# kalj/dealii-cuda

Hardware: AMD Instinct MI355X
Metric: DoFs/s on 1305x Laplace vmult (bmop), p=4 3D uniform (higher is better)
Workload: dtype f64; 1 GPU; bmop: DEGREE_FE=4, DIMENSION=3, MATRIX_FREE_UNIFORM_MESH, hyper_cube(-1,1), 54^3 cells, 10218313 DoFs, 1 z-slab(s); cells_per_dir=54, n_dofs=10218313, n_cells=157464, parallelism=slab1, dof_numbering=caller's (lexicographic), finite=True, clock_ramp_steps=2000

## Files before the change

dealii-cuda_amd/csrc/mfgpu_api.hip:

```cpp
#include <hip/hip_runtime.h>

#include <type_traits>

#include <algorithm>
#include <cmath>
#include <cstdlib>
#include <cstring>
#include <memory>
#include <string>
#include <vector>

#include "mfgpu_kernels.h"

using namespace mfgpu;

struct EventTimer {
  std::vector<Event> ev;
  size_t used = 0;
  double ms = 0.0;
  int begin(hipStream_t st) {
    if (used + 2 > ev.size()) {
      Event e0, e1;
      int rc;
      if ((rc = e0.create(hipEventDefault)) || (rc = e1.create(hipEventDefault))) return rc;
      ev.push_back(std::move(e0));
      ev.push_back(std::move(e1));
    }
    HIP_TRY(hipEventRecord(ev[used].get(), st));
    return 0;
  }
  int end(hipStream_t st) {
    HIP_TRY(hipEventRecord(ev[used + 1].get(), st));
    used += 2;
    return 0;
  }
  int drain(double *total) {
    for (size_t i = 0; i + 1 < used; i += 2) {
      float t = 0.f;
      HIP_TRY(hipEventElapsedTime(&t, ev[i].get(), ev[i + 1].get()));
      ms += t;
    }
    used = 0;
    *total = ms;
    return 0;
  }
  void reset() {
    used = 0;
    ms = 0.0;
  }
};

struct mfgpu_handle {
  Plan plan;
  int dim = 0, n = 0, nd = 0, number_type = MFGPU_F64;
  bool hn = false;
  std::vector<double> S, Dt;
  std::vector<double> sv, sg;
  DeviceArray<uint32_t> d_batch_cell_off, d_batch_dof_off, d_bdofs;
  DeviceArray<uint8_t> d_bflags;
  DeviceArray<uint16_t> d_lmap;
  DeviceArray<uint16_t> d_lmapx;
  DeviceArray<uint16_t> d_perm;
  DeviceArray<uint32_t> d_bdofsp, d_idxp;
  DeviceArray<uint32_t> d_hnrec;
  DeviceArray<uint32_t> d_hn_slot;
  DeviceArray<void> d_coefp;
  DeviceArray<void> d_coef;
  DeviceArray<uint32_t> d_cmask, d_orphans;
  DeviceArray<void> d_hnw;
  DeviceArray<uint32_t> d_constrained;
  uint32_t n_constrained = 0;
  DeviceArray<void> d_tabsd;
  DeviceArray<void> d_tab2;
  bool twopass = true;
  DeviceArray<uint32_t> d_batch_nint, d_halo_off;
  std::vector<uint32_t> seg_end;
  std::vector<DeviceArray<uint32_t>> d_p2arr, d_p2tiles;
  std::vector<uint32_t> n_p2tiles;
  Stream side;
  std::vector<Event> ev_seg;
  Event ev_side;
  bool side_pending = false;
  DeviceArray<void> d_halo;
  DeviceArray<unsigned long long> d_stamps;
  size_t lds = 0, device_bytes = 0;
  PlaneKernel planes = PlaneKernel::none;
  BatchKernel batches = BatchKernel::none;
  uint32_t max_grid = 0;
  uint32_t max_grid_p = 0;
  uint32_t max_grid_ph = 0;
  bool prof = false;
  EventTimer t_cells;
  EventTimer t_pass2;
  uint64_t prof_vmults = 0;
};

namespace {

template <typename T>
hipError_t family_configure(const mfgpu_handle *h, PlaneKernel k, bool hn, size_t *lds, int *blocks) {
  const Plan &P = h->plan;
  switch (k) {
    case PlaneKernel::planes3: return p_configure<T>(P.dim, P.n, hn, h->twopass, P.max_batch_dofs, lds, blocks);
    case PlaneKernel::planes4: return q_configure<T>(P.dim, P.n, hn, h->twopass, P.max_batch_dofs, lds, blocks);
    default: return hipErrorInvalidValue;
  }
}
template <typename T>
hipError_t family_configure(const mfgpu_handle *h, BatchKernel k, bool hn, size_t *lds, int *blocks) {
  const Plan &P = h->plan;
  switch (k) {
    case BatchKernel::batches: return apply_configure<T>(P.dim, P.n, hn, h->twopass, P.max_batch_dofs, lds, blocks);
    case BatchKernel::x: return x_configure<T>(P.dim, P.n, hn, h->twopass, P.max_batch_dofs, lds, blocks);
    case BatchKernel::g: return g_configure<T>(P.dim, P.n, hn, h->twopass, P.max_batch_dofs, lds, blocks);
    case BatchKernel::g2: return g2_configure<T>(P.dim, P.n, hn, h->twopass, P.max_batch_dofs, lds, blocks);
    default: return hipErrorInvalidValue;
  }
}
template <typename T>
hipError_t family_launch(const mfgpu_handle *h, PlaneKernel k, const ApplyArgs<T> &a, bool hn, uint32_t grid,
                         hipStream_t st) {
  const Plan &P = h->plan;
  const double *S = h->S.data(), *Dt = h->Dt.data();
  switch (k) {
    case PlaneKernel::planes3: return p_launch<T>(P.dim, P.n, hn, h->twopass, a, S, Dt, grid, st);
    case PlaneKernel::planes4: return q_launch<T>(P.dim, P.n, hn, h->twopass, a, S, Dt, grid, st);
    default: return hipErrorInvalidValue;
  }
}
template <typename T>
hipError_t family_launch(const mfgpu_handle *h, BatchKernel k, const ApplyArgs<T> &a, bool hn, uint32_t grid,
                         hipStream_t st) {
  const Plan &P = h->plan;
  const double *S = h->S.data(), *Dt = h->Dt.data();
  switch (k) {
    case BatchKernel::batches: return apply_launch<T>(P.dim, P.n, hn, h->twopass, a, S, Dt, grid, st);
    case BatchKernel::x: return x_launch<T>(P.dim, P.n, hn, h->twopass, a, S, Dt, grid, st);
    case BatchKernel::g: return g_launch<T>(P.dim, P.n, hn, h->twopass, a, S, Dt, grid, st);
    case BatchKernel::g2: return g2_launch<T>(P.dim, P.n, hn, h->twopass, a, S, Dt, grid, st);
    default: return hipErrorInvalidValue;
  }
}

int check_symmetrize(int n, std::vector<double> &S, std::vector<double> &Dt) {
  const int p = n - 1;
  double err = 0, mag = 0;
  for (int r = 0; r < n; ++r)
    for (int c = 0; c < n; ++c) {
      const double s1 = S[r * n + c], s2 = S[(p - r) * n + (p - c)];
      const double d1 = Dt[r * n + c], d2 = -Dt[(p - r) * n + (p - c)];
      err = std::fmax(err, std::fmax(std::fabs(s1 - s2), std::fabs(d1 - d2)));
      mag = std::fmax(mag, std::fmax(std::fabs(s1), std::fabs(d1)));
    }
  if (err > 1e-10 * mag) {
    set_error("shape tables are not symmetric about the cell midpoint (unsupported)");
    return MFGPU_EUNSUPPORTED;
  }
  for (int r = 0; r < n; ++r)
    for (int c = 0; c < n; ++c) {
      const int r2 = p - r, c2 = p - c;
      if (r * n + c < r2 * n + c2) {
        const double s = 0.5 * (S[r * n + c] + S[r2 * n + c2]);
        S[r * n + c] = S[r2 * n + c2] = s;
        const double d = 0.5 * (Dt[r * n + c] - Dt[r2 * n + c2]);
        Dt[r * n + c] = d;
        Dt[r2 * n + c2] = -d;
      } else if (r == r2 && c == c2) {
        Dt[r * n + c] = 0.0;
      }
    }
  return 0;
}

int upload_pass2(mfgpu_handle *h, const uint32_t *priority, uint32_t n_priority) {
  const Plan &P = h->plan;
  std::vector<uint8_t> prio(P.n_dofs, 0);
  for (uint32_t i = 0; i < n_priority; ++i) {
    if (priority[i] >= P.n_dofs) {
      set_error("priority dof out of range");
      return MFGPU_EINVAL;
    }
    prio[priority[i]] = 1;
  }
  const size_t ng = 1 + h->seg_end.size();
  std::vector<std::vector<uint32_t>> sd(ng), so(ng, std::vector<uint32_t>(1, 0u)), si(ng);
  auto add = [&](uint32_t dof, const uint32_t *slots, uint32_t k, size_t seg) {
    const size_t g = prio[dof & 0x7fffffffu] ? 0 : 1 + seg;
    sd[g].push_back(dof);
    si[g].insert(si[g].end(), slots, slots + k);
    so[g].push_back((uint32_t)si[g].size());
  };
  for (size_t i = 0; i < P.sdofs.size(); ++i) {
    size_t seg = 0;
    if (P.s_off[i + 1] > P.s_off[i]) {
      const uint32_t slot = P.s_idx[P.s_off[i + 1] - 1];
      const uint32_t batch = (uint32_t)(std::upper_bound(P.halo_off.begin(), P.halo_off.end(), slot) - P.halo_off.begin()) - 1;
      seg = (size_t)(std::upper_bound(h->seg_end.begin(), h->seg_end.end(), batch) - h->seg_end.begin());
      if (seg >= h->seg_end.size()) seg = h->seg_end.size() - 1;
    }
    add(P.sdofs[i], P.s_idx.data() + P.s_off[i], P.s_off[i + 1] - P.s_off[i], seg);
  }
  const uint32_t zero_slot = P.halo_off.empty() ? 0u : P.halo_off.back();
  for (uint32_t orph : P.orphans) add(orph, &zero_slot, 1, 0);
  std::vector<DeviceArray<uint32_t>> d_arr(ng), d_tiles(ng);
  std::vector<uint32_t> n_tiles(ng, 0u);
  for (size_t g = 0; g < ng; ++g) {
    std::vector<uint32_t> arr, tiles;
    build_pass2_classes(sd[g], so[g], si[g], arr, tiles);
    n_tiles[g] = (uint32_t)(tiles.size() / 4);
    if ((size_t)P.halo_off.back() * esize(h->number_type) <= ((size_t)256 << 20)) {
      const size_t nt = tiles.size() / 4;
      for (size_t a = 0, b = nt ? nt - 1 : 0; a < b; ++a, --b)
        for (int w = 0; w < 4; ++w) std::swap(tiles[4 * a + w], tiles[4 * b + w]);
    }
    int rc;
    if ((rc = d_arr[g].upload(arr.data(), arr.size()))) return rc;
    if ((rc = d_tiles[g].upload(tiles.data(), tiles.size()))) return rc;
  }
  h->d_p2arr = std::move(d_arr);
  h->d_p2tiles = std::move(d_tiles);
  h->n_p2tiles = std::move(n_tiles);
  return 0;
}

template <typename T>
int create_arrays(mfgpu_handle *h, const mfgpu_desc &d) {
  const Plan &P = h->plan;
  const size_t ncell = P.n_cells, nd = (size_t)P.nd;
  size_t &acct = h->device_bytes;
  auto up = [&](auto &arr, const void *src, size_t n) {
    const int rc = arr.upload(src, n);
    acct += arr.bytes();
    return rc;
  };
  int rc;
  if ((rc = up(h->d_batch_cell_off, P.batch_cell_off.data(), P.batch_cell_off.size()))) return rc;
  if ((rc = up(h->d_batch_dof_off, P.batch_dof_off.data(), P.batch_dof_off.size()))) return rc;
  if ((rc = up(h->d_bdofs, P.bdofs.data(), P.bdofs.size()))) return rc;
  if ((rc = up(h->d_bflags, P.bflags.data(), P.bflags.size()))) return rc;
  if ((rc = up(h->d_lmap, P.lmap.data(), P.lmap.size()))) return rc;
  const bool general = h->batches == BatchKernel::g || h->batches == BatchKernel::g2;
  if (h->batches == BatchKernel::x && !h->hn) {
    const int n = P.n, n2 = n * n, PP = n2, CH = 256 / PP, ndl = n2 * n;
    std::vector<uint16_t> perm(512, 0xffff);
    for (int layout = 0; layout < 2; ++layout) {
      uint16_t *lanes = perm.data() + 256 * layout;
      std::vector<int> fill(32, 0), overflow;
      for (int q = 0; q < CH * PP; ++q) {
        const int cell = q / PP, pen = q % PP, a = pen % n, b = pen / n;
        const int base = cell * ndl + (layout == 0 ? a + n2 * b : a + n * b);
        const int r = base & 31;
        if (fill[r] < 8) lanes[32 * fill[r]++ + r] = (uint16_t)q;
        else overflow.push_back(q);
      }
      for (int l = 255; l >= 0 && !overflow.empty(); --l)
        if (lanes[l] == 0xffff) {
          lanes[l] = (uint16_t)overflow.back();
          overflow.pop_back();
        }
    }
    if ((rc = up(h->d_perm, perm.data(), perm.size()))) return rc;
  }
  if (h->batches == BatchKernel::x || general) {
    const size_t n = (size_t)P.n, np = (n + 1) & ~(size_t)1, runs = P.lmap.size() / n;
    std::vector<uint16_t> lx(runs * np, 0);
    for (size_t r = 0; r < runs; ++r)
      for (size_t i = 0; i < n; ++i) lx[r * np + i] = P.lmap[r * n + i];
    if ((rc = up(h->d_lmapx, lx.data(), lx.size()))) return rc;
  }
  if (h->batches == BatchKernel::g2) {
    std::vector<T> sd(2 * (size_t)P.n * P.n);
    for (int i = 0; i < P.n * P.n; ++i) {
      sd[i] = (T)h->S[i];
      sd[P.n * P.n + i] = (T)h->Dt[i];
    }
    if ((rc = up(h->d_tabsd, sd.data(), sd.size() * sizeof(T)))) return rc;
  }
  if (h->planes != PlaneKernel::none) {
    if ((rc = build_plane_records(h->plan, d.constraint_mask))) return rc;
    if (!P.pr_hn.empty()) {
      if ((rc = up(h->d_hnrec, P.pr_hn.data(), P.pr_hn.size()))) return rc;
      if ((rc = up(h->d_hn_slot, P.pr_hn_slot.data(), P.pr_hn_slot.size()))) return rc;
    }
    if ((rc = up(h->d_bdofsp, P.pr_dofs.data(), P.pr_dofs.size()))) return rc;
    if ((rc = up(h->d_idxp, P.pr_idx.data(), P.pr_idx.size()))) return rc;
  }
  if ((rc = up(h->d_orphans, P.orphans.data(), P.orphans.size()))) return rc;
  if (h->twopass) {
    if ((rc = up(h->d_batch_nint, P.batch_nint.data(), P.batch_nint.size()))) return rc;
    if ((rc = up(h->d_halo_off, P.halo_off.data(), P.halo_off.size()))) return rc;
    if (h->planes != PlaneKernel::none && (uint64_t)P.halo_off.back() >= (1ull << 29)) {
      set_error("halo buffer too large for 32-bit byte offsets");
      return MFGPU_EUNSUPPORTED;
    }
    const size_t hb = ((size_t)P.halo_off.back() + 1) * sizeof(T);
    if ((rc = h->d_halo.alloc(hb, true))) return rc;
    acct += hb;
  }
  if (h->hn) {
    std::vector<uint32_t> cm(ncell);
    for (size_t i = 0; i < ncell; ++i) cm[i] = d.constraint_mask[P.cell_order[i]];
    if ((rc = up(h->d_cmask, cm.data(), ncell))) return rc;
    std::vector<T> w((size_t)h->n * h->n);
    for (size_t i = 0; i < w.size(); ++i) w[i] = (T)d.constraint_weights[i];
    if ((rc = up(h->d_hnw, w.data(), w.size() * sizeof(T)))) return rc;
  }
  DeviceArray<T> metric;
  if ((rc = fold_coefficient<T>(metric, d.coefficient, d.quadrature_points, d.JxW, d.inv_jac, P.cell_order.data(), P.dim,
                                (uint32_t)ncell, (uint32_t)nd, general)))
    return rc;
  h->d_coef = std::move(metric);
  acct += h->d_coef.bytes();
  if (h->planes != PlaneKernel::none) {
    const int n = P.n, NT = p_cells_per_wave(n) * n;
    const size_t nbat = P.n_plane_batches, total = nbat * (size_t)(n * n) * NT;
    const size_t ncell_p = P.batch_cell_off[nbat];
    std::vector<uint32_t> cb(ncell_p), cp(ncell_p);
    for (size_t b = 0; b < nbat; ++b)
      for (uint32_t c = P.batch_cell_off[b]; c < P.batch_cell_off[b + 1]; ++c) {
        cb[c] = (uint32_t)b;
        cp[c] = c - P.batch_cell_off[b];
      }
    DeviceArray<uint32_t> t_cb, t_cp;
    if ((rc = t_cb.upload(cb.data(), ncell_p))) return rc;
    if ((rc = t_cp.upload(cp.data(), ncell_p))) return rc;
    if ((rc = h->d_coefp.alloc(total * sizeof(T), true))) return rc;
    acct += h->d_coefp.bytes();
    HIP_TRY(relayout_coef_launch<T>(h->d_coefp.as<T>(), h->d_coef.as<const T>(), t_cb.get(), t_cp.get(), ncell_p * nd, n,
                                    nullptr));
    HIP_TRY(hipDeviceSynchronize());
  }
  int dev = 0, per_cu = 0;
  hipDeviceProp_t prop;
  HIP_TRY(hipGetDevice(&dev));
  HIP_TRY(hipGetDeviceProperties(&prop, dev));
  auto resident_grid = [&](int blocks_per_cu) {
    const uint32_t g = (uint32_t)(blocks_per_cu < 1 ? 1 : blocks_per_cu) * (uint32_t)prop.multiProcessorCount;
    return d.max_workgroups && d.max_workgroups < g ? d.max_workgroups : g;
  };
  if (h->planes != PlaneKernel::none) {
    HIP_TRY(family_configure<T>(h, h->planes, false, &h->lds, &per_cu));
    h->max_grid_p = resident_grid(per_cu);
    if (P.n_plain_plane_batches < P.n_plane_batches) {
      size_t lds_h = 0;
      HIP_TRY(family_configure<T>(h, h->planes, true, &lds_h, &per_cu));
      h->max_grid_ph = resident_grid(per_cu);
      h->lds = std::max(h->lds, lds_h);
    }
  }
  if (h->batches == BatchKernel::none) return 0;
  const hipError_t configure_batch_family = family_configure<T>(h, h->batches, h->hn, &h->lds, &per_cu);
  if (h->lds > 160 * 1024) {
    set_error("batch needs more than 160 KiB of LDS; lower max_dofs_per_batch");
    return MFGPU_EINVAL;
  }
  HIP_TRY(configure_batch_family);
  h->max_grid = resident_grid(per_cu);
  return 0;
}

void choose_segments(mfgpu_handle *h, uint32_t request) {
  const Plan &P = h->plan;
  const uint32_t nb = (uint32_t)(P.batch_cell_off.size() - 1);
  h->seg_end.assign(1, nb);
  if (!h->twopass || nb < 2 || request == 1) return;
  const uint32_t npl = P.n_plane_batches, nplain = P.n_plain_plane_batches;
  std::vector<uint32_t> cuts;
  if (npl > 0 && npl < nb) cuts.push_back(npl);
  if (nplain > 0 && nplain < npl) cuts.push_back(nplain);
  if (request > 1) {
    for (uint32_t i = 1; i < request; ++i) cuts.push_back((uint32_t)((uint64_t)nb * i / request));
  }
  if (request == 0 && !P.pr_hn.empty() && nplain == 0 && P.n == 5) cuts.push_back(nb / 2);
  std::sort(cuts.begin(), cuts.end());
  h->seg_end.clear();
  for (uint32_t c : cuts)
    if (c > 0 && c < nb && (h->seg_end.empty() || h->seg_end.back() != c)) h->seg_end.push_back(c);
  h->seg_end.push_back(nb);
}

template <typename T>
int create_typed(mfgpu_handle *h, const mfgpu_desc &d) {
  int rc = create_arrays<T>(h, d);
  if (rc) return rc;
  choose_segments(h, d.cell_loop_segments);
  if (!h->twopass) return 0;
  if (h->seg_end.size() > 1) {
    int prio_least = 0, prio_greatest = 0;
    HIP_TRY(hipDeviceGetStreamPriorityRange(&prio_least, &prio_greatest));
    if ((rc = h->side.create(hipStreamNonBlocking, prio_least))) return rc;
    if ((rc = h->ev_side.create(hipEventDisableTiming))) return rc;
    h->ev_seg.resize(h->seg_end.size() - 1);
    for (Event &e : h->ev_seg)
      if ((rc = e.create(hipEventDisableTiming))) return rc;
  }
  return upload_pass2(h, nullptr, 0);
}

template <typename T>
int launch_pass2_group(mfgpu_handle *h, size_t group, void *dst, const void *src, hipStream_t st, int add) {
  HIP_TRY(reduce_classes_launch<T>((T *)dst, (const T *)src, h->d_halo.as<const T>(), h->d_p2arr[group].get(),
                                   h->d_p2tiles[group].get(), h->n_p2tiles[group], add, st));
  return 0;
}

template <typename T>
int vmult_pass2(mfgpu_handle *h, int phase, void *dst, const void *src, hipStream_t st, int add) {
  if (!h->twopass) return 0;
  if (phase == 0) return launch_pass2_group<T>(h, 0, dst, src, st, add);
  int rc = launch_pass2_group<T>(h, h->seg_end.size(), dst, src, st, add);
  if (!rc && h->side_pending) {
    HIP_TRY(hipStreamWaitEvent(st, h->ev_side.get(), 0));
    h->side_pending = false;
  }
  return rc;
}

template <typename T>
int launch_cells(mfgpu_handle *h, ApplyArgs<T> a, uint32_t b0, uint32_t b1, hipStream_t st) {
  const Plan &P = h->plan;
  const uint32_t npl = P.n_plane_batches, nplain = P.n_plain_plane_batches;
  if (b0 < nplain) {
    a.batch0 = b0;
    a.batch_end = b1 < nplain ? b1 : nplain;
    const uint32_t nbat = a.batch_end - a.batch0;
    HIP_TRY(family_launch<T>(h, h->planes, a, false, nbat < h->max_grid_p ? nbat : h->max_grid_p, st));
    b0 = a.batch_end;
  }
  if (b0 < npl && b0 < b1) {
    a.batch0 = b0;
    a.batch_end = b1 < npl ? b1 : npl;
    const uint32_t nbat = a.batch_end - a.batch0;
    HIP_TRY(family_launch<T>(h, h->planes, a, true, nbat < h->max_grid_ph ? nbat : h->max_grid_ph, st));
    b0 = a.batch_end;
  }
  if (b0 >= b1) return 0;
  a.batch0 = b0;
  a.batch_end = b1;
  const uint32_t nrest = b1 - b0, grid = nrest < h->max_grid ? nrest : h->max_grid;
  HIP_TRY(family_launch<T>(h, h->batches, a, h->hn, grid, st));
  return 0;
}

template <typename T>
ApplyArgs<T> make_args(mfgpu_handle *h, void *dst, const void *src, int add) {
  const Plan &P = h->plan;
  ApplyArgs<T> a;
  a.batch_cell_off = h->d_batch_cell_off.get();
  a.batch_dof_off = h->d_batch_dof_off.get();
  a.bdofs = h->d_bdofs.get();
  a.bflags = h->d_bflags.get();
  a.lmap = h->d_lmap.get();
  a.lmapx = h->d_lmapx.get();
  a.perm = h->d_perm.get();
  a.bdofsp = h->d_bdofsp.get();
  a.idxp = h->d_idxp.get();
  a.hnrec = h->d_hnrec.get();
  a.hn_slot = h->d_hn_slot.get();
  a.coefp = h->d_coefp.as<const T>();
  a.coef = h->d_coef.as<const T>();
  a.cmask = h->d_cmask.get();
  a.hn_weights = h->d_hnw.as<const T>();
  a.tabS = h->d_tabsd.as<const T>();
  a.tabDt = a.tabS ? a.tabS + (size_t)P.n * P.n : nullptr;
  a.batch_nint = h->d_batch_nint.get();
  a.halo_off = h->d_halo_off.get();
  a.halo = h->d_halo.as<T>();
  a.dst = (T *)dst;
  a.src = (const T *)src;
  a.nb_max = P.max_batch_dofs;
  a.add = add;
  a.stamps = h->d_stamps.get();
  a.dbg = 0;
  return a;
}

template <typename T>
int vmult_main(mfgpu_handle *h, void *dst, const void *src, hipStream_t st, int add) {
  const Plan &P = h->plan;
  ApplyArgs<T> a = make_args<T>(h, dst, src, add);
  int rc;
  if (h->prof && (rc = h->t_cells.begin(st))) return rc;
  if (h->twopass) {
    const size_t nseg = h->seg_end.size();
    if (h->side_pending) {
      HIP_TRY(hipStreamWaitEvent(st, h->ev_side.get(), 0));
      h->side_pending = false;
    }
    for (size_t s = 0; s < nseg; ++s) {
      if ((rc = launch_cells<T>(h, a, s ? h->seg_end[s - 1] : 0u, h->seg_end[s], st))) return rc;
      if (s + 1 < nseg) {
        HIP_TRY(hipEventRecord(h->ev_seg[s].get(), st));
        HIP_TRY(hipStreamWaitEvent(h->side.get(), h->ev_seg[s].get(), 0));
        if ((rc = launch_pass2_group<T>(h, 1 + s, dst, src, h->side.get(), add))) return rc;
      }
    }
    if (nseg > 1) {
      HIP_TRY(hipEventRecord(h->ev_side.get(), h->side.get()));
      h->side_pending = true;
    }
  } else {
    for (size_t c = 0; c + 1 < P.color_batch_off.size(); ++c) {
      if (P.color_batch_off[c + 1] == P.color_batch_off[c]) continue;
      if ((rc = launch_cells<T>(h, a, P.color_batch_off[c], P.color_batch_off[c + 1], st))) return rc;
    }
  }
  if (h->prof && (rc = h->t_cells.end(st))) return rc;
  if (!h->twopass)
    HIP_TRY(orphan_launch<T>((T *)dst, (const T *)src, h->d_orphans.get(), (uint32_t)P.orphans.size(), add, st));
  if (h->prof) h->prof_vmults++;
  return 0;
}

template <typename T>
int vmult_typed(mfgpu_handle *h, void *dst, const void *src, hipStream_t st, int add) {
  int rc = vmult_main<T>(h, dst, src, st, add);
  if (rc) return rc;
  const bool timed = h->prof && h->twopass;
  if (timed && (rc = h->t_pass2.begin(st))) return rc;
  rc = vmult_pass2<T>(h, 0, dst, src, st, add);
  if (!rc) rc = vmult_pass2<T>(h, 1, dst, src, st, add);
  if (!rc && timed) rc = h->t_pass2.end(st);
  return rc;
}

}

namespace {
template <typename T>
int inverse_diagonal_typed(mfgpu_handle *h, void *diag, hipStream_t st) {
  const Plan &P = h->plan;
  const bool general = h->batches == BatchKernel::g || h->batches == BatchKernel::g2;
  if (!h->d_tab2.get()) {
    const int nn = h->n * h->n;
    std::vector<T> t2(2 * (size_t)nn);
    for (int i = 0; i < nn; ++i) {
      t2[i] = (T)(general ? h->sv[i] : h->sv[i] * h->sv[i]);
      t2[nn + i] = (T)(general ? h->sg[i] : h->sg[i] * h->sg[i]);
    }
    if (const int rc = h->d_tab2.upload(t2.data(), t2.size() * sizeof(T))) return rc;
    h->device_bytes += h->d_tab2.bytes();
  }
  HIP_TRY(fill_launch<T>((T *)diag, P.n_dofs, T(0), st));
  const uint32_t nb = (uint32_t)(P.batch_cell_off.size() - 1), *cell_off = h->d_batch_cell_off.get();
  const uint32_t *dof_off = h->d_batch_dof_off.get(), *bdofs = h->d_bdofs.get(), *cmask = h->d_cmask.get();
  const uint16_t *lmap = h->d_lmap.get();
  const T *coef = h->d_coef.as<const T>(), *hnw = h->d_hnw.as<const T>(), *tab2 = h->d_tab2.as<const T>();
  if (h->batches == BatchKernel::g2)
    HIP_TRY(diag_general2_launch<T>(P.n, (T *)diag, nb, cell_off, dof_off, bdofs, lmap, coef, cmask, hnw, tab2, st));
  else if (h->batches == BatchKernel::g)
    HIP_TRY(diag_general_launch<T>(P.n, (T *)diag, nb, cell_off, dof_off, bdofs, lmap, coef, cmask, hnw, tab2, st));
  else
    HIP_TRY(diag_launch<T>(P.dim, P.n, (T *)diag, nb, cell_off, dof_off, bdofs, lmap, coef, cmask, hnw, tab2, st));
  HIP_TRY(set_values_launch<T>((T *)diag, h->d_constrained.get(), h->n_constrained, T(1), st));
  HIP_TRY(vec_map_launch<T>(4, (T *)diag, nullptr, T(0), T(0), P.n_dofs, st));
  return 0;
}
}


namespace {
int vec_map(int op, void *v, const void *w, double s, double a, size_t n, int nt, void *stream) {
  if ((!v && n) || (!w && n && op <= 3)) {
    set_error("null vector");
    return MFGPU_EINVAL;
  }
  if (nt == MFGPU_F32)
    HIP_TRY(vec_map_launch<float>(op, (float *)v, (const float *)w, (float)s, (float)a, n, (hipStream_t)stream));
  else if (nt == MFGPU_F64)
    HIP_TRY(vec_map_launch<double>(op, (double *)v, (const double *)w, s, a, n, (hipStream_t)stream));
  else
    return MFGPU_EINVAL;
  return 0;
}
int vec_reduce(int op, void *v, const void *x, const void *w, double a, size_t n, int nt, void *stream, double *out) {
  if (!out || (n && (!v || (op != 2 && !w) || (op == 1 && !x)))) {
    set_error("null argument");
    return MFGPU_EINVAL;
  }
  if (nt == MFGPU_F32)
    HIP_TRY(vec_reduce_launch<float>(op, (float *)v, (const float *)x, (const float *)w, (float)a, n, (hipStream_t)stream, out));
  else if (nt == MFGPU_F64)
    HIP_TRY(vec_reduce_launch<double>(op, (double *)v, (const double *)x, (const double *)w, a, n, (hipStream_t)stream, out));
  else
    return MFGPU_EINVAL;
  return 0;
}
}


namespace mfgpu {
int handle_number_type(const mfgpu_handle *h) { return h->number_type; }
int handle_set_priority_dofs(mfgpu_handle *h, const uint32_t *ids, uint32_t n) {
  return h->twopass ? upload_pass2(h, ids, n) : 0;
}
int handle_n_batches(const mfgpu_handle *h) { return (int)h->plan.batch_cell_off.size() - 1; }
bool handle_ranged_ok(const mfgpu_handle *h) { return h->twopass && h->seg_end.size() == 1; }
int handle_batches_touching(const mfgpu_handle *h, const uint32_t *ids, uint32_t n, std::vector<uint8_t> &flags) {
  const Plan &P = h->plan;
  std::vector<uint8_t> mark(P.n_dofs, 0);
  for (uint32_t i = 0; i < n; ++i) {
    if (ids[i] >= P.n_dofs) {
      set_error("interface dof out of range");
      return MFGPU_EINVAL;
    }
    mark[ids[i]] = 1;
  }
  const size_t nb = P.batch_cell_off.size() - 1;
  flags.assign(nb, 0);
  for (size_t b = 0; b < nb; ++b)
    for (uint32_t t = P.batch_dof_off[b]; t < P.batch_dof_off[b + 1]; ++t)
      if (mark[P.bdofs[t] & 0x7fffffffu]) {
        flags[b] = 1;
        break;
      }
  return 0;
}
int handle_cells_range(mfgpu_handle *h, uint32_t b0, uint32_t b1, void *dst, const void *src, void *stream, int add) {
  if (b0 >= b1) return 0;
  hipStream_t st = (hipStream_t)stream;
  if (h->number_type == MFGPU_F64) return launch_cells<double>(h, make_args<double>(h, dst, src, add), b0, b1, st);
  return launch_cells<float>(h, make_args<float>(h, dst, src, add), b0, b1, st);
}
int handle_cells_two_ranges(mfgpu_handle *h, uint32_t b0, uint32_t b1, uint32_t c0, uint32_t c1, void *dst,
                            const void *src, void *stream, int add) {
  const uint32_t nplain = h->plan.n_plain_plane_batches, npl = h->plan.n_plane_batches;
  const bool plain = c1 <= nplain, masked = b0 >= nplain && c1 <= npl;
  if (b0 >= b1 || c0 >= c1 || b1 > c0 || !(plain || masked)) {
    const int rc = handle_cells_range(h, b0, b1, dst, src, stream, add);
    return rc ? rc : handle_cells_range(h, c0, c1, dst, src, stream, add);
  }
  hipStream_t st = (hipStream_t)stream;
  auto run = [&](auto a) -> int {
    a.batch0 = b0;
    a.batch_end = c1;
    a.hole0 = b1;
    a.hole_len = c0 - b1;
    const uint32_t nbat = (b1 - b0) + (c1 - c0);
    using T = typename std::remove_const<typename std::remove_pointer<decltype(a.src)>::type>::type;
    const uint32_t cap = plain ? h->max_grid_p : h->max_grid_ph;
    HIP_TRY(family_launch<T>(h, h->planes, a, !plain, nbat < cap ? nbat : cap, st));
    return 0;
  };
  return h->number_type == MFGPU_F64 ? run(make_args<double>(h, dst, src, add)) : run(make_args<float>(h, dst, src, add));
}
int handle_pass2_group(mfgpu_handle *h, int group, void *dst, const void *src, void *stream, int add) {
  if (!h->twopass) return 0;
  hipStream_t st = (hipStream_t)stream;
  return h->number_type == MFGPU_F64 ? launch_pass2_group<double>(h, (size_t)group, dst, src, st, add)
                                     : launch_pass2_group<float>(h, (size_t)group, dst, src, st, add);
}
int handle_vmult_phase(mfgpu_handle *h, int phase, void *dst, const void *src, void *stream, int add) {
  hipStream_t st = (hipStream_t)stream;
  if (h->number_type == MFGPU_F64)
    return phase == 0 ? vmult_main<double>(h, dst, src, st, add) : vmult_pass2<double>(h, phase - 1, dst, src, st, add);
  return phase == 0 ? vmult_main<float>(h, dst, src, st, add) : vmult_pass2<float>(h, phase - 1, dst, src, st, add);
}
}

extern "C" {

int mfgpu_create(const mfgpu_desc *desc, mfgpu_handle **out) {
  if (!desc || !out) {
    set_error("null argument");
    return MFGPU_EINVAL;
  }
  const mfgpu_desc &d = *desc;
  if (!valid_number_type(d.number_type)) {
    set_error("number_type must be MFGPU_F64 or MFGPU_F32");
    return MFGPU_EINVAL;
  }
  const bool general = !(d.flags & MFGPU_UNIFORM_J0);
  if (general && (d.flags & MFGPU_COLORED_SCATTER)) {
    set_error("the general-Jacobian path (no MFGPU_UNIFORM_J0) is implemented in two-pass scatter mode only");
    return MFGPU_EUNSUPPORTED;
  }
  if (!d.JxW || !d.inv_jac || !d.shape_values || !d.shape_gradients ||
      (!d.coefficient && !d.quadrature_points)) {
    set_error("JxW, inv_jac, shape tables and coefficient (or quadrature_points) are required");
    return MFGPU_EINVAL;
  }
  const bool hn = (d.flags & MFGPU_HANGING_NODES) != 0;
  if (hn && (!d.constraint_mask || !d.constraint_weights)) {
    set_error("MFGPU_HANGING_NODES needs constraint_mask and constraint_weights");
    return MFGPU_EINVAL;
  }
  std::unique_ptr<mfgpu_handle, decltype(&mfgpu_destroy)> h(new mfgpu_handle(), mfgpu_destroy);
  int rc = choose_kernel_and_plan(d, h->planes, h->batches, h->plan);
  if (rc) return rc;
  h->dim = d.dim;
  h->n = d.degree + 1;
  h->nd = h->plan.nd;
  h->number_type = d.number_type;
  h->hn = hn;
  h->twopass = !(d.flags & MFGPU_COLORED_SCATTER);
  const int nn = h->n * h->n;
  std::vector<double> sv(nn), sg(nn);
  for (int i = 0; i < nn; ++i) {
    sv[i] = d.number_type == MFGPU_F64 ? ((const double *)d.shape_values)[i] : ((const float *)d.shape_values)[i];
    sg[i] = d.number_type == MFGPU_F64 ? ((const double *)d.shape_gradients)[i] : ((const float *)d.shape_gradients)[i];
  }
  h->sv = sv;
  h->sg = sg;
  rc = derive_tables(h->n, sv.data(), sg.data(), h->S, h->Dt);
  if (!rc) rc = check_symmetrize(h->n, h->S, h->Dt);
  if (!rc) rc = d.number_type == MFGPU_F64 ? create_typed<double>(h.get(), d) : create_typed<float>(h.get(), d);
  if (!rc && d.n_constrained) {
    h->n_constrained = d.n_constrained;
    rc = h->d_constrained.upload(d.constrained_dofs, d.n_constrained);
    h->device_bytes += h->d_constrained.bytes();
  }
  if (rc) return rc;
  *out = h.release();
  return 0;
}

void mfgpu_destroy(mfgpu_handle *h) {
  if (!h) return;
  if (h->side.get()) hipStreamSynchronize(h->side.get());
  delete h;
}

int mfgpu_vmult(mfgpu_handle *h, void *dst, const void *src, void *stream) {
  if (!h || !dst || !src) {
    set_error("null argument");
    return MFGPU_EINVAL;
  }
  if (dst == src) {
    set_error("vmult: dst and src must not alias");
    return MFGPU_EINVAL;
  }
  return h->number_type == MFGPU_F64 ? vmult_typed<double>(h, dst, src, (hipStream_t)stream, 0)
                                     : vmult_typed<float>(h, dst, src, (hipStream_t)stream, 0);
}

int mfgpu_vmult_add(mfgpu_handle *h, void *dst, const void *src, void *stream) {
  if (!h || !dst || !src) {
    set_error("null argument");
    return MFGPU_EINVAL;
  }
  if (dst == src) {
    set_error("vmult_add: dst and src must not alias");
    return MFGPU_EINVAL;
  }
  return h->number_type == MFGPU_F64 ? vmult_typed<double>(h, dst, src, (hipStream_t)stream, 1)
                                     : vmult_typed<float>(h, dst, src, (hipStream_t)stream, 1);
}

uint32_t mfgpu_n_dofs(const mfgpu_handle *h) { return h ? h->plan.n_dofs : 0; }

size_t mfgpu_memory_consumption(const mfgpu_handle *h) { return h ? h->device_bytes : 0; }

int mfgpu_plan_stats(const mfgpu_handle *h, uint64_t s[8]) {
  if (!h || !s) return MFGPU_EINVAL;
  const Plan &P = h->plan;
  s[0] = P.batch_cell_off.size() - 1;
  s[1] = P.color_batch_off.size() - 1;
  s[2] = P.bdofs.size();
  s[3] = P.max_batch_dofs;
  s[4] = P.max_batch_cells;
  s[5] = P.orphans.size();
  s[6] = P.n_first;
  s[7] = P.n_add;
  if (h->twopass) {
    const uint32_t nb = (uint32_t)s[0], npl = P.n_plane_batches, nplain = P.n_plain_plane_batches;
    const uint32_t edge[4] = {0u, nplain, npl, nb};
    s[1] = 0;
    for (size_t g = 0; g < h->seg_end.size(); ++g) {
      const uint32_t s0 = g ? h->seg_end[g - 1] : 0u, s1 = h->seg_end[g];
      for (int f = 0; f < 3; ++f)
        if (std::max(s0, edge[f]) < std::min(s1, edge[f + 1])) ++s[1];
    }
    s[6] = P.sdofs.size();
    s[7] = P.halo_off.back();
  }
  return 0;
}

const char *mfgpu_kernel_name(const mfgpu_handle *h) {
  if (!h) return "";
  const bool x = h->batches == BatchKernel::x;
  switch (h->planes) {
    case PlaneKernel::planes3: return x ? "apply_planes3+apply_batches_x" : "apply_planes3";
    case PlaneKernel::planes4: return x ? "apply_planes4+apply_batches_x" : "apply_planes4";
    default: break;
  }
  switch (h->batches) {
    case BatchKernel::x: return "apply_batches_x";
    case BatchKernel::g: return "apply_batches_g";
    case BatchKernel::g2: return "apply_batches_g2";
    default: return "apply_batches";
  }
}

int mfgpu_profile_enable(mfgpu_handle *h, int on) {
  if (!h) return MFGPU_EINVAL;
  h->prof = on != 0;
  h->t_cells.reset();
  h->t_pass2.reset();
  h->prof_vmults = 0;
  return 0;
}

int mfgpu_profile_read_pass2(mfgpu_handle *h, double *ms) {
  if (!h || !ms) return MFGPU_EINVAL;
  HIP_TRY(hipDeviceSynchronize());
  return h->t_pass2.drain(ms);
}

int mfgpu_profile_read(mfgpu_handle *h, double *ms, uint64_t *nv) {
  if (!h || !ms || !nv) return MFGPU_EINVAL;
  HIP_TRY(hipDeviceSynchronize());
  if (const int rc = h->t_cells.drain(ms)) return rc;
  *nv = h->prof_vmults;
  return 0;
}

#ifdef MFGPU_STAMPS
int mfgpu_debug_stamps(mfgpu_handle *h, unsigned long long *out, size_t n_batches) {
  if (!h) return MFGPU_EINVAL;
  const size_t nbt = h->plan.batch_cell_off.size() - 1;
  if (!h->d_stamps.get()) return h->d_stamps.alloc(2 * nbt * 16, true);
  if (out && n_batches == nbt) {
    HIP_TRY(hipDeviceSynchronize());
    HIP_TRY(hipMemcpy(out, h->d_stamps.get(), 2 * nbt * 16 * sizeof(unsigned long long), hipMemcpyDeviceToHost));
  }
  return 0;
}
#endif


int mfgpu_compute_inverse_diagonal(mfgpu_handle *h, void *inv_diag, void *stream) {
  if (!h || !inv_diag) {
    set_error("null argument");
    return MFGPU_EINVAL;
  }
  return h->number_type == MFGPU_F64 ? inverse_diagonal_typed<double>(h, inv_diag, (hipStream_t)stream)
                                     : inverse_diagonal_typed<float>(h, inv_diag, (hipStream_t)stream);
}

int mfgpu_set_constrained_values(mfgpu_handle *h, void *vec, double value, void *stream) {
  if (!h || !vec) {
    set_error("null argument");
    return MFGPU_EINVAL;
  }
  if (h->number_type == MFGPU_F64)
    HIP_TRY(set_values_launch<double>((double *)vec, h->d_constrained.get(), h->n_constrained, value, (hipStream_t)stream));
  else
    HIP_TRY(set_values_launch<float>((float *)vec, h->d_constrained.get(), h->n_constrained, (float)value,
                                     (hipStream_t)stream));
  return 0;
}

int mfgpu_vec_sadd(void *v, double s, double a, const void *w, size_t n, int nt, void *stream) {
  return vec_map(0, v, w, s, a, n, nt, stream);
}
int mfgpu_vec_equ(void *v, double a, const void *w, size_t n, int nt, void *stream) {
  return vec_map(1, v, w, 0.0, a, n, nt, stream);
}
int mfgpu_vec_scale(void *v, const void *w, size_t n, int nt, void *stream) {
  return vec_map(2, v, w, 0.0, 0.0, n, nt, stream);
}
int mfgpu_vec_divide(void *v, const void *w, size_t n, int nt, void *stream) {
  return vec_map(3, v, w, 0.0, 0.0, n, nt, stream);
}
int mfgpu_vec_invert(void *v, size_t n, int nt, void *stream) { return vec_map(4, v, nullptr, 0.0, 0.0, n, nt, stream); }
int mfgpu_vec_mul(void *v, double a, size_t n, int nt, void *stream) {
  return vec_map(5, v, nullptr, 0.0, a, n, nt, stream);
}
int mfgpu_vec_dot(const void *v, const void *w, size_t n, int nt, void *stream, double *result) {
  return vec_reduce(0, const_cast<void *>(v), nullptr, w, 0.0, n, nt, stream, result);
}
int mfgpu_vec_l2_norm(const void *v, size_t n, int nt, void *stream, double *result) {
  int rc = vec_reduce(0, const_cast<void *>(v), nullptr, v, 0.0, n, nt, stream, result);
  if (!rc) *result = std::sqrt(*result);
  return rc;
}
int mfgpu_vec_add_and_dot(void *v, double a, const void *x, const void *w, size_t n, int nt, void *stream,
                          double *result) {
  return vec_reduce(1, v, x, w, a, n, nt, stream, result);
}
int mfgpu_vec_all_zero(const void *v, size_t n, int nt, void *stream, int *result) {
  if (!result) return MFGPU_EINVAL;
  double cnt = 0.0;
  int rc = vec_reduce(2, const_cast<void *>(v), nullptr, nullptr, 0.0, n, nt, stream, &cnt);
  if (!rc) *result = cnt == 0.0;
  return rc;
}

int mfgpu_vec_alloc(void **dev, size_t n, int nt) {
  if (!dev) return MFGPU_EINVAL;
  *dev = nullptr;
  if (n == 0) return 0;
  HIP_TRY(hipMalloc(dev, n * esize(nt)));
  HIP_TRY(hipMemset(*dev, 0, n * esize(nt)));
  return 0;
}
int mfgpu_vec_free(void *dev) {
  if (dev) HIP_TRY(hipFree(dev));
  return 0;
}
int mfgpu_vec_fill(void *dev, size_t n, int nt, double value, void *stream) {
  if (!dev && n) return MFGPU_EINVAL;
  if (nt == MFGPU_F32)
    HIP_TRY(fill_launch<float>((float *)dev, n, (float)value, (hipStream_t)stream));
  else
    HIP_TRY(fill_launch<double>((double *)dev, n, value, (hipStream_t)stream));
  return 0;
}
int mfgpu_vec_from_host(void *dev, const void *host, size_t n, int nt) {
  if (n) HIP_TRY(hipMemcpy(dev, host, n * esize(nt), hipMemcpyHostToDevice));
  return 0;
}
int mfgpu_vec_to_host(void *host, const void *dev, size_t n, int nt) {
  if (n) HIP_TRY(hipMemcpy(host, dev, n * esize(nt), hipMemcpyDeviceToHost));
  return 0;
}
int mfgpu_device_synchronize(void) {
  HIP_TRY(hipDeviceSynchronize());
  return 0;
}
int mfgpu_device_memory_info(size_t *free_bytes, size_t *total_bytes) {
  if (!free_bytes || !total_bytes) return MFGPU_EINVAL;
  HIP_TRY(hipMemGetInfo(free_bytes, total_bytes));
  return 0;
}

}
```

dealii-cuda_amd/csrc/mfgpu_internal.h:

```cpp
#ifndef MFGPU_INTERNAL_H
#define MFGPU_INTERNAL_H

#include <cstdint>
#include <string>
#include <vector>

#include "../../include/mfgpu.h"

namespace mfgpu {

void set_error(const std::string &msg);

inline int ipow(int a, int e) {
  int r = 1;
  for (int i = 0; i < e; ++i) r *= a;
  return r;
}

constexpr int p_cells_per_wave(int n) { return 64 / n; }
constexpr int p_ji(int n) { return n == 3 ? 2 : n == 4 ? 5 : n == 5 ? 9 : n == 6 ? 14 : 23; }
constexpr int p_hs(int n) { return n == 3 ? 3 : n == 4 ? 6 : n == 5 ? 9 : n == 6 ? 14 : 18; }
constexpr int p_kgu(int n) { return p_ji(n) + p_hs(n); }
constexpr int p_cell_stride(int n) {
  int s = n * n * n;
  while ((s & 31) != (n & 31)) ++s;
  return s;
}

constexpr int q_plane_stride(int n) { return n >= 6 ? 65 : n == 5 ? 33 : n == 4 ? 17 : 33; }
constexpr int q_cell_stride(int n) { return n * q_plane_stride(n); }
constexpr int p_priv_max(int n) { return n >= 5 ? 384 : n == 4 ? 256 : 192; }
constexpr int kHnOpRounds = 2;
constexpr int p_hn_rows(int n) { return p_priv_max(n) / 64 + 3 * kHnOpRounds * 3 + 2; }

template <typename T>
constexpr size_t q_region_doubles(int n) {
  const size_t t = ((size_t)(p_cells_per_wave(n) + 1) * q_cell_stride(n) * sizeof(T) + 7) / 8;
  const size_t u = (size_t)p_kgu(n) * 64 + p_priv_max(n);
  return t > u ? t : u;
}
template <typename T>
constexpr size_t q_lds_bytes(int n, bool hn) {
  return (q_region_doubles<T>(n) + (hn ? (size_t)n * n : 0)) * 8;
}

constexpr uint8_t kFlagConstrained = 1;
constexpr uint8_t kFlagAdd = 2;

struct Plan {
  int dim = 0, degree = 0, n = 0, nd = 0;
  uint32_t n_dofs = 0, n_cells = 0;
  std::vector<uint32_t> cell_order;
  std::vector<uint32_t> batch_cell_off;
  std::vector<uint32_t> batch_dof_off;
  std::vector<uint32_t> color_batch_off;
  std::vector<uint32_t> bdofs;
  std::vector<uint8_t> bflags;
  std::vector<uint16_t> lmap;
  std::vector<uint32_t> orphans;
  std::vector<uint32_t> batch_nint;
  std::vector<uint32_t> halo_off;
  std::vector<uint32_t> sdofs;
  std::vector<uint32_t> s_off;
  std::vector<uint32_t> s_idx;
  std::vector<uint32_t> chunks;
  std::vector<uint32_t> gstarts;
  uint32_t max_batch_dofs = 0, max_batch_cells = 0;
  uint32_t n_plane_batches = 0;
  uint32_t n_plain_plane_batches = 0;
  std::vector<uint32_t> pr_dofs, pr_idx, pr_hn, pr_hn_slot;
  uint64_t n_first = 0, n_add = 0;
};

struct PlanLimits {
  uint32_t max_cells = 0, max_dofs = 0;
  uint32_t interior_max = 0, shared_max = 0, halo_stride = 0;
  bool segregate_masked = false;
  bool masked_planes = false;
  uint32_t private_max = 0;
};

int build_plan(const mfgpu_desc &d, Plan &plan, uint32_t max_chunks = 3, const PlanLimits *limits = nullptr);

struct HnLine {
  uint16_t node[8];
};
void hn_cell_lines(unsigned mask, int n, std::vector<HnLine> (&lines)[3], std::vector<uint16_t> &nodes);

enum class PlaneKernel : uint8_t { none, planes3, planes4 };
enum class BatchKernel : uint8_t { none, batches, x, g, g2 };
int choose_kernel_and_plan(const mfgpu_desc &d, PlaneKernel &pk, BatchKernel &bk, Plan &plan);
int build_plane_records(Plan &plan, const uint32_t *constraint_mask);

int derive_tables(int n, const double *shape_values, const double *shape_gradients,
                  std::vector<double> &S, std::vector<double> &Dt);

int handle_number_type(const mfgpu_handle *h);
int handle_set_priority_dofs(mfgpu_handle *h, const uint32_t *ids, uint32_t n);
int handle_vmult_phase(mfgpu_handle *h, int phase, void *dst, const void *src, void *stream, int add);
int handle_n_batches(const mfgpu_handle *h);
bool handle_ranged_ok(const mfgpu_handle *h);
int handle_batches_touching(const mfgpu_handle *h, const uint32_t *ids, uint32_t n, std::vector<uint8_t> &flags);
int handle_cells_range(mfgpu_handle *h, uint32_t b0, uint32_t b1, void *dst, const void *src, void *stream, int add);
int handle_cells_two_ranges(mfgpu_handle *h, uint32_t b0, uint32_t b1, uint32_t c0, uint32_t c1, void *dst,
                            const void *src, void *stream, int add);
int handle_pass2_group(mfgpu_handle *h, int group, void *dst, const void *src, void *stream, int add);

}

struct mfgpu_plan {
  mfgpu::Plan plan;
};

#endif
```

dealii-cuda_amd/csrc/mfgpu_kernels.h:

```cpp
#ifndef MFGPU_KERNELS_H
#define MFGPU_KERNELS_H

#include <hip/hip_runtime.h>

#include "mfgpu_device.h"
#include "mfgpu_internal.h"

namespace mfgpu {

template <typename T>
struct ApplyArgs {
  const uint32_t *batch_cell_off;
  const uint32_t *batch_dof_off;
  const uint32_t *bdofs;
  const uint8_t *bflags;
  const uint16_t *lmap;
  const uint16_t *lmapx;
  const uint16_t *perm;
  const uint32_t *bdofsp;
  const uint32_t *idxp;
  const T *coefp;
  const uint32_t *hnrec;
  const uint32_t *hn_slot;
  const T *coef;
  const uint32_t *cmask;
  const T *hn_weights;
  const T *tabS, *tabDt;
  const uint32_t *batch_nint;
  const uint32_t *halo_off;
  T *halo;
  T *dst;
  const T *src;
  uint32_t batch0;
  uint32_t batch_end;
  uint32_t hole0 = 0xffffffffu, hole_len = 0;
  uint32_t nb_max;
  int add;
  unsigned long long *stamps;
  int dbg;
};

template <typename T, int n>
struct Tables {
  T S[((n + 1) / 2) * n];
  T Dt[((n + 1) / 2) * n];
};

template <typename T, int n>
inline Tables<T, n> make_tables(const double *S, const double *Dt) {
  Tables<T, n> tab;
  for (int i = 0; i < ((n + 1) / 2) * n; ++i) {
    tab.S[i] = (T)S[i];
    tab.Dt[i] = (T)Dt[i];
  }
  return tab;
}

inline hipError_t configure_kernel(const void *kernel, size_t lds, int block, int *blocks) {
  const hipError_t e = hipFuncSetAttribute(kernel, hipFuncAttributeMaxDynamicSharedMemorySize, (int)lds);
  return e == hipSuccess ? hipOccupancyMaxActiveBlocksPerMultiprocessor(blocks, kernel, block, lds) : e;
}

#define MFGPU_CELL_LOOP_LAUNCHERS(F)                                                                               \
  template <typename T>                                                                                            \
  hipError_t F##_configure(int dim, int n, bool hn, bool twopass, uint32_t nb_max, size_t *lds, int *blocks);     \
  template <typename T>                                                                                            \
  hipError_t F##_launch(int dim, int n, bool hn, bool twopass, const ApplyArgs<T> &a, const double *S,            \
                        const double *Dt, uint32_t grid, hipStream_t st);
MFGPU_CELL_LOOP_LAUNCHERS(apply)
MFGPU_CELL_LOOP_LAUNCHERS(x)
MFGPU_CELL_LOOP_LAUNCHERS(g)
MFGPU_CELL_LOOP_LAUNCHERS(g2)
MFGPU_CELL_LOOP_LAUNCHERS(p)
MFGPU_CELL_LOOP_LAUNCHERS(q)
#undef MFGPU_CELL_LOOP_LAUNCHERS
#define MFGPU_SWITCH_N_HN(FN, ...)                                                                \
  switch (n) {                                                                                    \
    case 2: return hn ? FN<2, T, true>(__VA_ARGS__) : FN<2, T, false>(__VA_ARGS__);               \
    case 3: return hn ? FN<3, T, true>(__VA_ARGS__) : FN<3, T, false>(__VA_ARGS__);               \
    case 4: return hn ? FN<4, T, true>(__VA_ARGS__) : FN<4, T, false>(__VA_ARGS__);               \
    case 5: return hn ? FN<5, T, true>(__VA_ARGS__) : FN<5, T, false>(__VA_ARGS__);               \
    case 6: return hn ? FN<6, T, true>(__VA_ARGS__) : FN<6, T, false>(__VA_ARGS__);               \
    case 7: return hn ? FN<7, T, true>(__VA_ARGS__) : FN<7, T, false>(__VA_ARGS__);               \
    default: return hipErrorInvalidValue;                                                         \
  }

void build_pass2_classes(const std::vector<uint32_t> &sdofs, const std::vector<uint32_t> &s_off,
                         const std::vector<uint32_t> &s_idx, std::vector<uint32_t> &arr, std::vector<uint32_t> &tiles);
template <typename T>
hipError_t reduce_classes_launch(T *dst, const T *src, const T *halo, const uint32_t *arr, const uint32_t *tiles,
                                 uint32_t n_tiles, int add, hipStream_t st);
template <typename T>
hipError_t relayout_coef_launch(T *out, const T *in, const uint32_t *cell_batch, const uint32_t *cell_pos,
                                size_t total, int n, hipStream_t st);
template <typename T>
hipError_t fold_general_launch(T *M, const T *coef, const T *jxw, const T *jinv, const uint32_t *order,
                               uint32_t n_cells, uint32_t nd, hipStream_t st);
template <typename T>
hipError_t fold_general2_launch(T *M, const T *coef, const T *jxw, const T *jinv, const uint32_t *order,
                                uint32_t n_cells, uint32_t nd, hipStream_t st);
template <typename T>
hipError_t orphan_launch(T *dst, const T *src, const uint32_t *orph, uint32_t n, int add, hipStream_t st);
template <typename T>
hipError_t coefficient_launch(T *coef, const T *qpts, size_t nq, int dim, hipStream_t st);
template <typename T>
hipError_t fold_launch(T *c, const T *coef, const T *jxw, const T *j0, const uint32_t *order,
                       uint32_t n_cells, uint32_t nd, hipStream_t st);
template <typename T>
hipError_t fill_launch(T *v, size_t n, T a, hipStream_t st);
template <typename T>
int fold_coefficient(DeviceArray<T> &out, const void *coefficient, const void *quadrature_points, const void *JxW,
                     const void *inv_jac, const uint32_t *cell_order, int dim, uint32_t n_cells, uint32_t nd,
                     bool general);

template <typename T>
hipError_t diag_launch(int dim, int n, T *diag, uint32_t n_batches, const uint32_t *batch_cell_off,
                       const uint32_t *batch_dof_off, const uint32_t *bdofs, const uint16_t *lmap, const T *coef,
                       const uint32_t *cmask, const T *hn_weights, const T *tab2, hipStream_t st);
template <typename T>
hipError_t diag_general_launch(int n, T *diag, uint32_t n_batches, const uint32_t *batch_cell_off,
                               const uint32_t *batch_dof_off, const uint32_t *bdofs, const uint16_t *lmap,
                               const T *metric, const uint32_t *cmask, const T *hn_weights, const T *tab,
                               hipStream_t st);
template <typename T>
hipError_t diag_general2_launch(int n, T *diag, uint32_t n_batches, const uint32_t *batch_cell_off,
                                const uint32_t *batch_dof_off, const uint32_t *bdofs, const uint16_t *lmap,
                                const T *metric, const uint32_t *cmask, const T *hn_weights, const T *tab,
                                hipStream_t st);
template <typename T>
hipError_t set_values_launch(T *v, const uint32_t *idx, uint32_t n, T value, hipStream_t st);
template <typename T>
hipError_t vec_map_launch(int op, T *v, const T *w, T s, T a, size_t n, hipStream_t st);
template <typename T>
hipError_t vec_reduce_launch(int op, T *v, const T *x, const T *w, T a, size_t n, hipStream_t st, double *out);

}
#endif
```

dealii-cuda_amd/csrc/mfgpu_kernels_p.hip:

```cpp
#include <hip/hip_runtime.h>

#include "mfgpu_cell.h"
#include "mfgpu_kernels.h"
#include "mfgpu_planes.h"

namespace mfgpu {

#define MFGPU_PIN_VMEM() __builtin_amdgcn_sched_barrier(0x380)

template <int n, typename T, bool ADD, bool HN>
__global__ void __launch_bounds__(64) __attribute__((amdgpu_waves_per_eu(1, 1)))
apply_planes3(const ApplyArgs<T> A, const TablesEO<T, n> tab) {
  constexpr int n2 = n * n;
  constexpr int CW = p_cells_per_wave(n);
  constexpr int NT = CW * n;
  constexpr int KGU = p_kgu(n);
  constexpr int JI = p_ji(n);
  constexpr int HS = KGU - JI;
  constexpr int SA = p_cell_stride(n);
  constexpr int NIW = (n2 + 1) / 2;
  extern __shared__ __attribute__((aligned(16))) unsigned char smem_raw[];
  constexpr int PRIV = HN ? p_priv_max(n) : 0;
  double *ua = reinterpret_cast<double *>(smem_raw);
  T *Aw = reinterpret_cast<T *>(ua + KGU * 64 + PRIV + (HN ? n2 : 0));
  T *Bw = Aw + (CW + 1) * SA;
  double *Wl = ua + KGU * 64 + PRIV;

  const int lane = threadIdx.x;
  if (HN) {
    if (lane < n2) Wl[lane] = (double)A.hn_weights[lane];
  }
  const int lc = lane / n, k = lane - lc * n;
  const bool lane_on = lane < NT;
  const int tk = lane_on ? lane : NT - 1;

  uint32_t b, bstride, bend;
  {
    const uint32_t nbt = A.batch_end - A.batch0 - A.hole_len, G = gridDim.x;
    if (G >= 8 && nbt >= G) {
      const uint32_t xcd = blockIdx.x & 7u, slot = blockIdx.x >> 3;
      const uint32_t q = G >> 3, rem = G & 7u;
      const uint32_t wlo = xcd * q + (xcd < rem ? xcd : rem);
      const uint32_t w = q + (xcd < rem ? 1u : 0u);
      b = A.batch0 + (uint32_t)((uint64_t)nbt * wlo / G) + slot;
      bend = A.batch0 + (uint32_t)((uint64_t)nbt * (wlo + w) / G);
      bstride = w;
    } else {
      b = A.batch0 + blockIdx.x;
      bend = A.batch_end - A.hole_len;
      bstride = G;
    }
  }
  if (b >= bend) return;
  const uint32_t hole0 = A.hole0, hole_len = A.hole_len;
  auto next_of = [&](uint32_t x) {
    const uint32_t l = (x >= hole0 ? x - hole_len : x) + bstride;
    return l < bend ? (l >= hole0 ? l + hole_len : l) : x;
  };
  if (b >= hole0) b += hole_len;

  auto load_dofs = [&](uint32_t bb, uint32_t (&g)[KGU]) {
    const uint32_t *p = A.bdofsp + (size_t)bb * (KGU * 64) + lane;
#pragma unroll
    for (int j = 0; j < KGU; ++j) g[j] = nt_load(p + j * 64);
  };
  auto src_at = [&](uint32_t g) -> T {
    return *reinterpret_cast<const T *>(reinterpret_cast<const char *>(A.src) + (uint32_t)(g * (uint32_t)sizeof(T)));
  };
  auto dst_at = [&](uint32_t g) -> T * {
    return reinterpret_cast<T *>(reinterpret_cast<char *>(A.dst) + (uint32_t)(g * (uint32_t)sizeof(T)));
  };
  auto load_ix = [&](uint32_t bb, uint32_t (&ix)[NIW]) {
    const uint32_t *p = A.idxp + (size_t)bb * (NIW * NT) + tk;
#pragma unroll
    for (int w = 0; w < NIW; ++w) ix[w] = nt_load(p + w * NT);
  };
  auto stage_src = [&](const uint32_t (&g)[KGU], const T (&sv)[KGU]) {
#pragma unroll
    for (int j = 0; j < KGU; ++j) {
      double v = (double)sv[j];
      if (j >= JI) {
        const unsigned long long keep = (unsigned long long)(long long)~((int)g[j] >> 31);
        v = __longlong_as_double((long long)((unsigned long long)__double_as_longlong(v) & keep));
      }
      ua[lane + j * 64] = v;
    }
  };
  auto ixb = [&](const uint32_t (&ix)[NIW], int i) -> uint32_t {
    return (i & 1) ? (ix[i >> 1] >> 16) : (ix[i >> 1] & 0xffffu);
  };
  auto scatter_slot = [&](int j, uint32_t bb, uint32_t g, T r, T oldv) {
    if (j < JI) {
      *dst_at(g) = ADD ? oldv + r : r;
    } else {
      T *const hp = A.halo + (size_t)bb * (HS * 64) + lane;
      hp[(j - JI) * 64] = r;
    }
  };

  uint32_t b1 = next_of(b), b2 = next_of(b1);
  uint32_t Gp[KGU], Gc[KGU], Gn[KGU], Gnn[KGU];
  uint32_t IXc[NIW], IXn[NIW];
  constexpr int CR = PRIV / 64, HROWS = HN ? p_hn_rows(n) : 1;
  uint32_t Hc[HROWS], Hn[HROWS];
  auto load_hn = [&](uint32_t bb, uint32_t (&H)[HROWS]) {
    const uint32_t slot = A.hn_slot[bb];
    if (slot != 0xffffffffu) {
      const uint32_t *p = A.hnrec + (size_t)slot * (HROWS * 64) + lane;
#pragma unroll
      for (int w = 0; w < HROWS; ++w) H[w] = nt_load(p + w * 64);
    } else {
#pragma unroll
      for (int w = 0; w < HROWS; ++w) H[w] = 0u;
    }
  };
  T Cc[n2];
  T SVn[KGU], R[KGU], old[KGU];
  load_dofs(b, Gc);
  load_dofs(b1, Gn);
  load_ix(b, IXc);
  if (HN) load_hn(b, Hc);
  constexpr uint32_t kDummyIx = 8u * (uint32_t)(KGU * 64 - 1) * 0x10001u;
#pragma unroll
  for (int w = 0; w < NIW; ++w) IXc[w] = lane_on ? IXc[w] : kDummyIx;
  {
    const T *p = A.coefp + (size_t)b * (n2 * NT) + tk;
#pragma unroll
    for (int r = 0; r < n2; ++r) Cc[r] = nt_load(p + r * NT);
  }
#pragma unroll
  for (int j = 0; j < KGU; ++j) {
    SVn[j] = src_at(Gc[j]);
    Gp[j] = Gc[j];
    R[j] = T(0);
    old[j] = T(0);
  }
  stage_src(Gc, SVn);
  WaveSync::sync();

  const int pxy = lc * SA + n2 * k;
  const int pyz = lc * SA + k;
  uint32_t bp = b;

  while (true) {
    const bool has_next = b1 != b;
    constexpr int kH2 = HN ? HROWS - 2 : 0, kH1 = HN ? HROWS - 1 : 0;
    const uint32_t hn_ncopy = HN ? (uint32_t)__builtin_amdgcn_readfirstlane(Hc[kH2] & 0xffffu) : 0u;
    auto hn_count = [&](int dir) -> uint32_t {
      const uint32_t w = dir == 0 ? Hc[kH2] >> 16 : dir == 1 ? Hc[kH1] & 0xffffu : Hc[kH1] >> 16;
      return (uint32_t)__builtin_amdgcn_readfirstlane(w);
    };
    auto hn_pass = [&](int dir, bool transposed, const double (&Wr)[n2]) {
      const uint32_t count = hn_count(dir);
#pragma unroll
      for (int r = 0; r < kHnOpRounds; ++r) {
        if ((uint32_t)(r * 64) >= count) break;
        const bool on = (uint32_t)(r * 64 + lane) < count;
        const uint32_t *ww = &Hc[CR + (dir * kHnOpRounds + r) * 3];
        double v[n], o[n];
        uint32_t pos[n];
#pragma unroll
        for (int t = 0; t < n; ++t) {
          pos[t] = on ? (ww[t >> 1] >> (16 * (t & 1))) & 0xffffu : (uint32_t)(KGU * 64 + PRIV - 1);
          v[t] = ua[pos[t]];
        }
#pragma unroll
        for (int i = 0; i < n; ++i) {
          double acc = 0.0;
#pragma unroll
          for (int k2 = 0; k2 < n; ++k2) acc = fma(transposed ? Wr[k2 * n + i] : Wr[i * n + k2], v[k2], acc);
          o[i] = acc;
        }
        if (on) {
#pragma unroll
          for (int i = 0; i < n; ++i) ua[pos[i]] = o[i];
        }
      }
    };
    if (HN && hn_ncopy) {
      double Wr[n2];
#pragma unroll
      for (int i = 0; i < n2; ++i) Wr[i] = Wl[i];
      double cv[CR > 0 ? CR : 1];
#pragma unroll
      for (int r = 0; r < CR; ++r) cv[r] = (uint32_t)(r * 64 + lane) < hn_ncopy ? ua[Hc[r] & 0xffffu] : 0.0;
#pragma unroll
      for (int r = 0; r < CR; ++r)
        if ((uint32_t)(r * 64 + lane) < hn_ncopy) ua[Hc[r] >> 16] = cv[r];
      WaveSync::sync();
      hn_pass(0, false, Wr);
      WaveSync::sync();
      hn_pass(1, false, Wr);
      WaveSync::sync();
      hn_pass(2, false, Wr);
      WaveSync::sync();
    }
    STAMP(0);
    RSTAMP(8);
    WGSTAMP(10);
    load_dofs(b2, Gnn);
    load_ix(b1, IXn);
    if (HN) load_hn(b1, Hn);
    if (ADD) {
#pragma unroll
      for (int j = 0; j < JI; ++j) old[j] = *dst_at(Gp[j]);
    }
    STAMP(1);
    auto hookA = [&](int) {};
    auto hookB = [&](int s) {
      MFGPU_PIN_VMEM();
#pragma unroll
      for (int j = (KGU * s) / (5 * n); j < (KGU * (s + 1)) / (5 * n); ++j)
        scatter_slot(j, bp, Gp[j], R[j], old[j]);
#pragma unroll
      for (int j = (KGU * s) / (5 * n); j < (KGU * (s + 1)) / (5 * n); ++j)
        SVn[j] = src_at(Gn[j]);
      MFGPU_PIN_VMEM();
    };
    const T *const cnext = A.coefp + (size_t)b1 * (n2 * NT) + tk;
    auto hookC = [&](int s) {
      MFGPU_PIN_VMEM();
#pragma unroll
      for (int r = (n2 * s) / (2 * n); r < (n2 * (s + 1)) / (2 * n); ++r)
        Cc[r] = nt_load(cnext + r * NT);
      MFGPU_PIN_VMEM();
    };

    {
      T u[n2];
#pragma unroll
      for (int x = 0; x < n; ++x)
#pragma unroll
        for (int y = 0; y < n; ++y)
          u[x + n * y] = (T) * reinterpret_cast<const double *>(reinterpret_cast<const char *>(ua) + ixb(IXc, x + n * y));
#pragma unroll
      for (int x = 0; x < n; ++x) {
        T in[n], out[n];
        get_line<n, 1>(u, x, in);
        eo_apply<n, 0>(tab, in, out);
        set_line<n, 1>(u, x, out);
        hookA(x);
      }
#pragma unroll
      for (int y = 0; y < n; ++y) {
        T in[n], a[n], bb[n];
        get_line<n, 0>(u, y, in);
        eo_apply<n, 0>(tab, in, a);
        eo_apply<n, 2>(tab, a, bb);
#pragma unroll
        for (int x = 0; x < n; ++x) {
          Aw[pxy + x + n * y] = a[x];
          Bw[pxy + x + n * y] = bb[x];
        }
        hookA(n + y);
      }
    }
    WaveSync::sync();
    STAMP(2);
#pragma unroll
    for (int j = 0; j < KGU + PRIV / 64; ++j) ua[lane + j * 64] = 0.0;

    {
      T nx[n];
#pragma unroll
      for (int z = 0; z < n; ++z) nx[z] = Bw[pyz + n2 * z];
#pragma unroll
      for (int y = 0; y < n; ++y) {
        T in[n], g[n], o[n];
#pragma unroll
        for (int z = 0; z < n; ++z) in[z] = nx[z];
#pragma unroll
        for (int z = 0; z < n; ++z) nx[z] = y + 1 < n ? Bw[pyz + n * (y + 1) + n2 * z] : Aw[pyz + n2 * z];
        eo_apply<n, 0>(tab, in, g);
#pragma unroll
        for (int z = 0; z < n; ++z) g[z] *= Cc[y + n * z];
        eo_apply<n, 1>(tab, g, o);
#pragma unroll
        for (int z = 0; z < n; ++z) Bw[pyz + n * y + n2 * z] = o[z];
        hookB(y);
      }
      T v[n2], r[n2];
#pragma unroll
      for (int y = 0; y < n; ++y) {
        T in[n], o[n];
#pragma unroll
        for (int z = 0; z < n; ++z) in[z] = nx[z];
        if (y + 1 < n) {
#pragma unroll
          for (int z = 0; z < n; ++z) nx[z] = Aw[pyz + n * (y + 1) + n2 * z];
        }
        eo_apply<n, 0>(tab, in, o);
        set_line<n, 1>(v, y, o);
        hookB(n + y);
      }
#pragma unroll
      for (int y = 0; y < n; ++y) {
        T in[n], g[n], o[n];
        get_line<n, 1>(v, y, in);
        eo_apply<n, 2>(tab, in, g);
#pragma unroll
        for (int z = 0; z < n; ++z) g[z] *= Cc[y + n * z];
        eo_apply<n, 3>(tab, g, o);
        set_line<n, 1>(r, y, o);
        hookB(2 * n + y);
      }
#pragma unroll
      for (int z = 0; z < n; ++z) {
        T in[n], g[n], o[n];
        get_line<n, 0>(v, z, in);
        eo_apply<n, 2>(tab, in, g);
#pragma unroll
        for (int y = 0; y < n; ++y) g[y] *= Cc[y + n * z];
        eo_apply<n, 3>(tab, g, o);
#pragma unroll
        for (int y = 0; y < n; ++y) r[y + n * z] += o[y];
        hookB(3 * n + z);
      }
#pragma unroll
      for (int y = 0; y < n; ++y) {
        T in[n], o[n];
        get_line<n, 1>(r, y, in);
        eo_apply<n, 1>(tab, in, o);
#pragma unroll
        for (int z = 0; z < n; ++z) Aw[pyz + n * y + n2 * z] = o[z];
        hookB(4 * n + y);
      }
    }
    WaveSync::sync();
    STAMP(3);

    {
      T o[n2];
      T nr[n], nt[n];
#pragma unroll
      for (int x = 0; x < n; ++x) {
        nr[x] = Aw[pxy + x];
        nt[x] = Bw[pxy + x];
      }
#pragma unroll
      for (int y = 0; y < n; ++y) {
        T rp[n], tp[n], w[n], ol[n];
#pragma unroll
        for (int x = 0; x < n; ++x) {
          rp[x] = nr[x];
          tp[x] = nt[x];
        }
        if (y + 1 < n) {
#pragma unroll
          for (int x = 0; x < n; ++x) {
            nr[x] = Aw[pxy + x + n * (y + 1)];
            nt[x] = Bw[pxy + x + n * (y + 1)];
          }
        }
        eo_apply<n, 3>(tab, tp, w);
#pragma unroll
        for (int x = 0; x < n; ++x) w[x] += rp[x];
        eo_apply<n, 1>(tab, w, ol);
        set_line<n, 0>(o, y, ol);
        hookC(y);
      }
#pragma unroll
      for (int x = 0; x < n; ++x) {
        T in[n], out[n];
        get_line<n, 1>(o, x, in);
        eo_apply<n, 1>(tab, in, out);
#pragma unroll
        for (int y = 0; y < n; ++y)
          lds_add(reinterpret_cast<double *>(reinterpret_cast<char *>(ua) + ixb(IXc, x + n * y)), (double)out[y]);
        hookC(n + x);
      }
    }
    WaveSync::sync();
    STAMP(4);

    if (HN && hn_ncopy) {
      double Wr[n2];
#pragma unroll
      for (int i = 0; i < n2; ++i) Wr[i] = Wl[i];
      hn_pass(2, true, Wr);
      WaveSync::sync();
      hn_pass(1, true, Wr);
      WaveSync::sync();
      hn_pass(0, true, Wr);
      WaveSync::sync();
      double cv[CR > 0 ? CR : 1];
#pragma unroll
      for (int r = 0; r < CR; ++r) cv[r] = (uint32_t)(r * 64 + lane) < hn_ncopy ? ua[Hc[r] >> 16] : 0.0;
#pragma unroll
      for (int r = 0; r < CR; ++r)
        if ((uint32_t)(r * 64 + lane) < hn_ncopy) lds_add(ua + (Hc[r] & 0xffffu), cv[r]);
      WaveSync::sync();
    }
#pragma unroll
    for (int j = 0; j < KGU; ++j) R[j] = (T)ua[lane + j * 64];
    WaveSync::sync();
    STAMP(5);
    stage_src(Gn, SVn);
    STAMP(6);
    bp = b;
#pragma unroll
    for (int j = 0; j < KGU; ++j) Gp[j] = Gc[j];
    STAMP(7);
    RSTAMP(9);
    if (!has_next) break;
    WaveSync::sync();
    b = b1;
    b1 = b2;
    b2 = next_of(b2);
#pragma unroll
    for (int j = 0; j < KGU; ++j) {
      Gc[j] = Gn[j];
      Gn[j] = Gnn[j];
    }
#pragma unroll
    for (int w = 0; w < NIW; ++w) IXc[w] = lane_on ? IXn[w] : kDummyIx;
    if (HN) {
#pragma unroll
      for (int w = 0; w < HROWS; ++w) Hc[w] = Hn[w];
    }
  }
  if (ADD) {
#pragma unroll
    for (int j = 0; j < JI; ++j) old[j] = *dst_at(Gp[j]);
  }
#pragma unroll
  for (int j = 0; j < KGU; ++j) scatter_slot(j, bp, Gp[j], R[j], old[j]);
}

template <int n, typename T>
static size_t p_lds_bytes(bool hn) {
  return ((size_t)p_kgu(n) * 64 + (hn ? (size_t)p_priv_max(n) + n * n : 0)) * sizeof(double) +
         (size_t)2 * (p_cells_per_wave(n) + 1) * p_cell_stride(n) * sizeof(T);
}

template <int n, typename T>
static hipError_t p_configure_t(bool hn, size_t *lds, int *blocks) {
  *lds = p_lds_bytes<n, T>(hn);
  const void *f0 = hn ? (const void *)apply_planes3<n, T, false, true> : (const void *)apply_planes3<n, T, false, false>;
  const void *f1 = hn ? (const void *)apply_planes3<n, T, true, true> : (const void *)apply_planes3<n, T, true, false>;
  const hipError_t e = hipFuncSetAttribute(f1, hipFuncAttributeMaxDynamicSharedMemorySize, (int)*lds);
  return e == hipSuccess ? configure_kernel(f0, *lds, 64, blocks) : e;
}

template <int n, typename T>
static hipError_t p_launch_t(const ApplyArgs<T> &a, const double *S, const double *Dt, bool hn, uint32_t grid,
                             hipStream_t st) {
  const size_t lds = p_lds_bytes<n, T>(hn);
  const TablesEO<T, n> tab = make_tables_eo<T, n>(S, Dt);
  if (hn) {
    if (a.add)
      hipLaunchKernelGGL((apply_planes3<n, T, true, true>), dim3(grid), dim3(64), lds, st, a, tab);
    else
      hipLaunchKernelGGL((apply_planes3<n, T, false, true>), dim3(grid), dim3(64), lds, st, a, tab);
  } else {
    if (a.add)
      hipLaunchKernelGGL((apply_planes3<n, T, true, false>), dim3(grid), dim3(64), lds, st, a, tab);
    else
      hipLaunchKernelGGL((apply_planes3<n, T, false, false>), dim3(grid), dim3(64), lds, st, a, tab);
  }
  return hipGetLastError();
}

#define P_SWITCH(FN, ...)                 \
  switch (n) {                            \
    case 3: return FN<3, T>(__VA_ARGS__); \
    case 4: return FN<4, T>(__VA_ARGS__); \
    case 5: return FN<5, T>(__VA_ARGS__); \
    default: return hipErrorInvalidValue; \
  }
template <typename T>
hipError_t p_configure(int, int n, bool hn, bool, uint32_t, size_t *lds, int *blocks) {
  P_SWITCH(p_configure_t, hn, lds, blocks)
}
template <typename T>
hipError_t p_launch(int, int n, bool hn, bool, const ApplyArgs<T> &a, const double *S, const double *Dt, uint32_t grid,
                    hipStream_t st) {
  P_SWITCH(p_launch_t, a, S, Dt, hn, grid, st)
}
#undef P_SWITCH

template hipError_t p_configure<double>(int, int, bool, bool, uint32_t, size_t *, int *);
template hipError_t p_configure<float>(int, int, bool, bool, uint32_t, size_t *, int *);
template hipError_t p_launch<double>(int, int, bool, bool, const ApplyArgs<double> &, const double *, const double *,
                                     uint32_t, hipStream_t);
template hipError_t p_launch<float>(int, int, bool, bool, const ApplyArgs<float> &, const double *, const double *,
                                    uint32_t, hipStream_t);

template <typename T>
__global__ void relayout_coef_kernel(T *out, const T *in, const uint32_t *cell_batch, const uint32_t *cell_pos,
                                     size_t total, int n) {
  const size_t i = (size_t)blockIdx.x * blockDim.x + threadIdx.x;
  if (i >= total) return;
  const int n2 = n * n, nd = n2 * n, NT = (64 / n) * n;
  const size_t cell = i / nd;
  const int q = (int)(i - cell * nd);
  const int x = q % n, r = q / n;
  out[((size_t)cell_batch[cell] * n2 + r) * NT + cell_pos[cell] * n + x] = in[i];
}

template <typename T>
hipError_t relayout_coef_launch(T *out, const T *in, const uint32_t *cell_batch, const uint32_t *cell_pos,
                                size_t total, int n, hipStream_t st) {
  if (total == 0) return hipSuccess;
  hipLaunchKernelGGL(relayout_coef_kernel<T>, dim3((unsigned)((total + 255) / 256)), dim3(256), 0, st, out, in,
                     cell_batch, cell_pos, total, n);
  return hipGetLastError();
}
template hipError_t relayout_coef_launch<double>(double *, const double *, const uint32_t *, const uint32_t *, size_t,
                                                 int, hipStream_t);
template hipError_t relayout_coef_launch<float>(float *, const float *, const uint32_t *, const uint32_t *, size_t, int,
                                                hipStream_t);

}
```

dealii-cuda_amd/csrc/mfgpu_pass2.hip:

```cpp
#include <hip/hip_runtime.h>

#include <algorithm>

#include "mfgpu_kernels.h"

namespace mfgpu {

namespace {

template <typename T, int K>
__device__ __forceinline__ void reduce_two(T *__restrict__ dst, const T *__restrict__ src, const T *__restrict__ halo,
                                           const uint32_t *__restrict__ p, uint32_t cnt, uint32_t i0, uint32_t k,
                                           int add) {
  const uint32_t i1 = i0 + 256u;
  const uint32_t d0 = p[i0], d1 = p[i1];
  constexpr int KU = K > 0 ? K : 1;
  uint32_t s0[KU], s1[KU];
#pragma unroll
  for (int t = 0; t < KU; ++t) {
    s0[t] = p[(size_t)(1 + t) * cnt + i0];
    s1[t] = p[(size_t)(1 + t) * cnt + i1];
  }
  const bool on0 = d0 != 0xffffffffu, on1 = d1 != 0xffffffffu;
  const uint32_t g0 = d0 & 0x7fffffffu, g1 = d1 & 0x7fffffffu;
  T v0 = T(0), v1 = T(0), o0 = T(0), o1 = T(0);
  if (on0) {
    if (d0 >> 31) {
      v0 = src[g0];
    } else {
      T q[KU];
#pragma unroll
      for (int t = 0; t < KU; ++t) q[t] = halo[s0[t]];
      v0 = q[0];
#pragma unroll
      for (int t = 1; t < KU; ++t) v0 += q[t];
      if (K == 0)
        for (uint32_t t = 1; t < k; ++t) v0 += halo[p[(size_t)(1 + t) * cnt + i0]];
    }
    if (add) o0 = dst[g0];
  }
  if (on1) {
    if (d1 >> 31) {
      v1 = src[g1];
    } else {
      T q[KU];
#pragma unroll
      for (int t = 0; t < KU; ++t) q[t] = halo[s1[t]];
      v1 = q[0];
#pragma unroll
      for (int t = 1; t < KU; ++t) v1 += q[t];
      if (K == 0)
        for (uint32_t t = 1; t < k; ++t) v1 += halo[p[(size_t)(1 + t) * cnt + i1]];
    }
    if (add) o1 = dst[g1];
  }
  if (on0) dst[g0] = add ? o0 + v0 : v0;
  if (on1) dst[g1] = add ? o1 + v1 : v1;
}

template <typename T>
__global__ void __launch_bounds__(256)
reduce_classes(T *__restrict__ dst, const T *__restrict__ src, const T *__restrict__ halo,
               const uint32_t *__restrict__ arr, const uint4 *__restrict__ tiles, int add) {
  const uint4 td = tiles[blockIdx.x];
  const uint32_t *p = arr + td.x;
  const uint32_t i0 = td.w + threadIdx.x;
  switch (td.y) {
    case 1: reduce_two<T, 1>(dst, src, halo, p, td.z, i0, 1, add); break;
    case 2: reduce_two<T, 2>(dst, src, halo, p, td.z, i0, 2, add); break;
    case 3: reduce_two<T, 3>(dst, src, halo, p, td.z, i0, 3, add); break;
    case 4: reduce_two<T, 4>(dst, src, halo, p, td.z, i0, 4, add); break;
    case 8: reduce_two<T, 8>(dst, src, halo, p, td.z, i0, 8, add); break;
    default: reduce_two<T, 0>(dst, src, halo, p, td.z, i0, td.y, add); break;
  }
}

}

void build_pass2_classes(const std::vector<uint32_t> &sdofs, const std::vector<uint32_t> &s_off,
                         const std::vector<uint32_t> &s_idx, std::vector<uint32_t> &arr, std::vector<uint32_t> &tiles) {
  arr.clear();
  tiles.clear();
  const size_t ns = sdofs.size();
  uint32_t kmax = 0;
  for (size_t i = 0; i < ns; ++i) kmax = std::max(kmax, s_off[i + 1] - s_off[i]);
  std::vector<std::vector<uint32_t>> members(kmax + 1);
  for (size_t i = 0; i < ns; ++i) {
    uint32_t k = s_off[i + 1] - s_off[i];
    if (k == 0) k = 1;
    members[k].push_back((uint32_t)i);
  }
  for (uint32_t k = 1; k <= kmax; ++k) {
    const std::vector<uint32_t> &m = members[k];
    if (m.empty()) continue;
    const uint32_t entries = (uint32_t)((m.size() + 511) / 512 * 512);
    const uint32_t base = (uint32_t)arr.size();
    arr.resize(arr.size() + (size_t)(1 + k) * entries, 0u);
    for (uint32_t e = 0; e < entries; ++e) arr[base + e] = e < m.size() ? sdofs[m[e]] : 0xffffffffu;
    for (size_t e = 0; e < m.size(); ++e) {
      const uint32_t i = m[e], cnt = s_off[i + 1] - s_off[i];
      for (uint32_t t = 0; t < k; ++t) arr[base + (size_t)(1 + t) * entries + e] = t < cnt ? s_idx[s_off[i] + t] : 0u;
    }
    for (uint32_t first = 0; first < entries; first += 512) {
      tiles.push_back(base);
      tiles.push_back(k);
      tiles.push_back(entries);
      tiles.push_back(first);
    }
  }
}

template <typename T>
hipError_t reduce_classes_launch(T *dst, const T *src, const T *halo, const uint32_t *arr, const uint32_t *tiles,
                                 uint32_t n_tiles, int add, hipStream_t st) {
  if (n_tiles == 0) return hipSuccess;
  hipLaunchKernelGGL(reduce_classes<T>, dim3(n_tiles), dim3(256), 0, st, dst, src, halo, arr,
                     reinterpret_cast<const uint4 *>(tiles), add);
  return hipGetLastError();
}
template hipError_t reduce_classes_launch<double>(double *, const double *, const double *, const uint32_t *,
                                                  const uint32_t *, uint32_t, int, hipStream_t);
template hipError_t reduce_classes_launch<float>(float *, const float *, const float *, const uint32_t *,
                                                 const uint32_t *, uint32_t, int, hipStream_t);

}
```

dealii-cuda_amd/csrc/mfgpu_plan.cpp:

```cpp
#include <algorithm>
#include <cassert>
#include <cmath>
#include <cstring>
#include <numeric>

#include "mfgpu_internal.h"

namespace mfgpu {

static thread_local std::string g_err;
void set_error(const std::string &msg) { g_err = msg; }
const char *last_error() { return g_err.c_str(); }

int derive_tables(int n, const double *sv, const double *sg, std::vector<double> &S,
                  std::vector<double> &Dt) {
  std::vector<long double> A(n * n), B(n * n);
  for (int i = 0; i < n * n; ++i) {
    A[i] = sv[i];
    B[i] = sg[i];
  }
  for (int c = 0; c < n; ++c) {
    int piv = c;
    for (int r = c + 1; r < n; ++r)
      if (fabsl(A[r * n + c]) > fabsl(A[piv * n + c])) piv = r;
    if (fabsl(A[piv * n + c]) < 1e-30L) {
      set_error("shape_values table is singular");
      return MFGPU_EINVAL;
    }
    if (piv != c)
      for (int k = 0; k < n; ++k) {
        std::swap(A[c * n + k], A[piv * n + k]);
        std::swap(B[c * n + k], B[piv * n + k]);
      }
    for (int r = 0; r < n; ++r) {
      if (r == c) continue;
      long double f = A[r * n + c] / A[c * n + c];
      for (int k = 0; k < n; ++k) {
        A[r * n + k] -= f * A[c * n + k];
        B[r * n + k] -= f * B[c * n + k];
      }
    }
  }
  S.assign(sv, sv + n * n);
  Dt.resize(n * n);
  for (int t = 0; t < n; ++t)
    for (int q = 0; q < n; ++q) Dt[q * n + t] = (double)(B[t * n + q] / A[t * n + t]);
  return 0;
}

static void default_batch_limits(const mfgpu_desc &d, uint32_t max_chunks, uint32_t &max_cells, uint32_t &max_dofs) {
  const int p = d.degree, dim = d.dim;
  max_dofs = d.max_dofs_per_batch ? d.max_dofs_per_batch : 2304u;
  if (max_dofs > 2304u) max_dofs = 2304u;
  const uint32_t nd = (uint32_t)ipow(p + 1, dim);
  if (max_dofs < nd) max_dofs = nd;
  if (d.max_cells_per_batch) {
    max_cells = d.max_cells_per_batch;
  } else {
    int m = 1;
    while ((uint64_t)ipow((m + 1) * p + 1, dim) <= max_dofs) ++m;
    uint64_t best = (uint64_t)ipow(m, dim);
    for (int k = 1; k < dim; ++k) {
      const uint64_t dofs = (uint64_t)ipow((m + 1) * p + 1, k) * (uint64_t)ipow(m * p + 1, dim - k);
      if (dofs <= max_dofs) best = (uint64_t)ipow(m + 1, k) * (uint64_t)ipow(m, dim - k);
    }
    max_cells = (uint32_t)best;
    const uint32_t cap = std::max<uint32_t>(1u, d.n_cells / 4096u);
    max_cells = std::min(max_cells, cap);
  }
  const uint32_t threads = d.max_dofs_per_batch && d.max_dofs_per_batch <= 768 ? 64u : 256u;
  const uint32_t ch = std::max<uint32_t>(1u, threads / (uint32_t)ipow(p + 1, dim - 1));
  max_cells = std::min(max_cells, max_chunks * ch);
  if (max_cells < 1) max_cells = 1;
}

void hn_cell_lines(unsigned mask, int n, std::vector<HnLine> (&lines)[3], std::vector<uint16_t> &nodes) {
  const int p = n - 1;
  const unsigned TYPE[3] = {1u << 0, 1u << 1, 1u << 2}, FACE[3] = {1u << 3, 1u << 4, 1u << 5};
  const unsigned EDGE[3] = {1u << 7, 1u << 8, 1u << 6};
  const int stride[3] = {1, n, n * n};
  std::vector<uint8_t> on(n * n * n, 0);
  for (int d = 0; d < 3; ++d) {
    lines[d].clear();
    const int d1 = (d + 1) % 3, d2 = (d + 2) % 3;
    if (!(mask & (FACE[d1] | FACE[d2] | EDGE[d]))) continue;
    const int i1 = (mask & TYPE[d1]) ? 0 : p, i2 = (mask & TYPE[d2]) ? 0 : p;
    const bool typ = (mask & TYPE[d]) != 0;
    for (int a = 0; a < n; ++a)
      for (int b = 0; b < n; ++b) {
        const bool flag = ((mask & FACE[d1]) && a == i1) || ((mask & FACE[d2]) && b == i2) ||
                          ((mask & EDGE[d]) && a == i1 && b == i2);
        if (!flag) continue;
        HnLine L{};
        for (int t = 0; t < n; ++t) {
          const int node = (typ ? t : p - t) * stride[d] + a * stride[d1] + b * stride[d2];
          L.node[t] = (uint16_t)node;
          on[node] = 1;
        }
        lines[d].push_back(L);
      }
  }
  nodes.clear();
  for (int i = 0; i < n * n * n; ++i)
    if (on[i]) nodes.push_back((uint16_t)i);
}

int build_plan(const mfgpu_desc &d, Plan &P, uint32_t max_chunks, const PlanLimits *limits) {
  if (d.dim != 2 && d.dim != 3) {
    set_error("dim must be 2 or 3");
    return MFGPU_EINVAL;
  }
  if (d.degree < 1 || d.degree > 6) {
    set_error("degree must be in 1..6");
    return MFGPU_EUNSUPPORTED;
  }
  if (!d.loc2glob || d.n_cells == 0 || d.n_dofs == 0) {
    set_error("empty description (n_cells, n_dofs and loc2glob are required)");
    return MFGPU_EINVAL;
  }
  if (d.n_constrained && !d.constrained_dofs) {
    set_error("n_constrained > 0 but constrained_dofs is NULL");
    return MFGPU_EINVAL;
  }
  P.dim = d.dim;
  P.degree = d.degree;
  P.n = d.degree + 1;
  P.nd = ipow(P.n, d.dim);
  P.n_dofs = d.n_dofs;
  P.n_cells = d.n_cells;
  const uint32_t nd = (uint32_t)P.nd, nc = d.n_cells, N = d.n_dofs;
  const uint32_t *l2g = d.loc2glob;

  for (uint64_t i = 0; i < (uint64_t)nc * nd; ++i)
    if (l2g[i] >= N) {
      set_error("loc2glob entry out of range");
      return MFGPU_EINVAL;
    }
  std::vector<uint8_t> constrained(N, 0);
  for (uint32_t i = 0; i < d.n_constrained; ++i) {
    if (d.constrained_dofs[i] >= N) {
      set_error("constrained_dofs entry out of range");
      return MFGPU_EINVAL;
    }
    constrained[d.constrained_dofs[i]] = 1;
  }

  if (N >= 0x80000000u) {
    set_error("n_dofs >= 2^31 is not supported (bit 31 of the dof lists carries the constrained flag)");
    return MFGPU_EUNSUPPORTED;
  }
  const bool segregate = limits && limits->segregate_masked && (d.flags & MFGPU_HANGING_NODES) && d.constraint_mask;
  uint32_t Bmax1 = 0, NBmax1 = 0;
  if (segregate) default_batch_limits(d, max_chunks, Bmax1, NBmax1);
  const bool masked_planes = segregate && limits->masked_planes && limits->max_cells && limits->max_dofs;
  std::vector<uint32_t> priv_of_mask;
  if (masked_planes) {
    priv_of_mask.assign(512, 0u);
    std::vector<HnLine> ln[3];
    std::vector<uint16_t> nodes;
    for (unsigned m = 1; m < 512; ++m) {
      hn_cell_lines(m, P.n, ln, nodes);
      priv_of_mask[m] = (uint32_t)nodes.size();
    }
    for (uint32_t c = 0; c < nc; ++c)
      if (d.constraint_mask[c] >= 512) {
        set_error("constraint_mask has bits beyond the nine of hanging_nodes.cuh:38-50");
        return MFGPU_EINVAL;
      }
  }
  auto priv_of = [&](uint32_t c) { return masked_planes ? priv_of_mask[d.constraint_mask[c]] : 0u; };
  uint32_t Bmax, NBmax;
  if (limits && limits->max_cells && limits->max_dofs) {
    Bmax = d.max_cells_per_batch ? std::min(d.max_cells_per_batch, limits->max_cells) : limits->max_cells;
    NBmax = d.max_dofs_per_batch ? std::min(d.max_dofs_per_batch, limits->max_dofs) : limits->max_dofs;
    if (NBmax < (uint32_t)P.nd) {
      set_error("max_dofs_per_batch is smaller than one cell");
      return MFGPU_EINVAL;
    }
  } else {
    default_batch_limits(d, max_chunks, Bmax, NBmax);
  }

  std::vector<uint32_t> dc_off(N + 1, 0);
  for (uint64_t i = 0; i < (uint64_t)nc * nd; ++i) dc_off[l2g[i] + 1]++;
  for (uint32_t g = 0; g < N; ++g) dc_off[g + 1] += dc_off[g];
  std::vector<uint32_t> dc(dc_off[N]);
  {
    std::vector<uint32_t> pos(dc_off.begin(), dc_off.end() - 1);
    for (uint32_t c = 0; c < nc; ++c)
      for (uint32_t i = 0; i < nd; ++i) dc[pos[l2g[(uint64_t)c * nd + i]]++] = c;
    uint32_t w = 0;
    for (uint32_t g = 0; g < N; ++g) {
      const uint32_t beg = dc_off[g], end = dc_off[g + 1];
      dc_off[g] = w;
      for (uint32_t k = beg; k < end; ++k)
        if (k == beg || dc[k] != dc[k - 1]) dc[w++] = dc[k];
    }
    dc_off[N] = w;
    dc.resize(w);
  }

  constexpr uint32_t NONE = 0xffffffffu;
  const bool bound_surface_any = limits && limits->interior_max;
  auto masked = [&](uint32_t c) { return segregate && d.constraint_mask[c] != 0; };

  std::vector<uint32_t> nbr;
  const bool use_boxes = bound_surface_any && !segregate && P.dim == 3 && P.n >= 3 && Bmax >= 4;
  if (use_boxes) {
    nbr.assign((size_t)nc * 6, NONE);
    const uint32_t n_ = (uint32_t)P.n, mid = 1;
    for (uint32_t c = 0; c < nc; ++c)
      for (uint32_t axis = 0; axis < 3; ++axis)
        for (uint32_t side = 0; side < 2; ++side) {
          uint32_t ijk[3] = {mid, mid, mid}, opp[3] = {mid, mid, mid};
          ijk[axis] = side ? n_ - 1 : 0;
          opp[axis] = side ? 0 : n_ - 1;
          const uint32_t li = ijk[0] + n_ * ijk[1] + n_ * n_ * ijk[2], lo = opp[0] + n_ * opp[1] + n_ * n_ * opp[2];
          const uint32_t g = l2g[(uint64_t)c * nd + li];
          if (dc_off[g + 1] - dc_off[g] != 2) continue;
          const uint32_t c2 = dc[dc_off[g]] == c ? dc[dc_off[g] + 1] : dc[dc_off[g]];
          if (c2 != c && l2g[(uint64_t)c2 * nd + lo] == g) nbr[(size_t)c * 6 + 2 * axis + side] = c2;
        }
  }
  struct Shape {
    uint32_t a, b, c;
  };
  std::vector<Shape> shapes;
  if (use_boxes) {
    for (uint32_t a = 1; a <= Bmax; ++a)
      for (uint32_t b2 = 1; a * b2 <= Bmax; ++b2)
        for (uint32_t c2 = 1; a * b2 * c2 <= Bmax; ++c2)
          if (a * b2 * c2 == Bmax) shapes.push_back({a, b2, c2});
    auto spread = [](const Shape &s2) { return std::max(s2.a, std::max(s2.b, s2.c)) * 4 + s2.a + s2.b + s2.c; };
    std::stable_sort(shapes.begin(), shapes.end(), [&](const Shape &x, const Shape &y) {
      const uint32_t vx = x.a * x.b * x.c, vy = y.a * y.b * y.c;
      if (vx != vy) return vx > vy;
      if (spread(x) != spread(y)) return spread(x) < spread(y);
      return x.a != y.a ? x.a > y.a : x.b > y.b;
    });
  }

  std::vector<uint8_t> batch_masked;
  std::vector<uint32_t> cell_batch(nc, NONE);
  std::vector<uint32_t> dof_stamp(N, NONE);
  std::vector<uint32_t> inc_cnt(bound_surface_any ? N : 0, 0);
  std::vector<uint32_t> gain(nc, 0), gain_stamp(nc, NONE);
  std::vector<uint32_t> cand, box;
  std::vector<std::vector<uint32_t>> batches;
  uint32_t stamp = 0;
  uint32_t seed = 0;
  while (true) {
    while (seed < nc && cell_batch[seed] != NONE) ++seed;
    if (seed >= nc) break;
    const uint32_t b = (uint32_t)batches.size();
    batches.emplace_back();
    std::vector<uint32_t> &cells = batches.back();
    const bool cls = masked(seed);
    batch_masked.push_back(cls);
    const bool bound_surface = bound_surface_any && (!cls || masked_planes);
    const uint32_t Bmax_b = cls && !masked_planes ? Bmax1 : Bmax, NBmax_b = cls && !masked_planes ? NBmax1 : NBmax;
    uint32_t ndofs = 0, n_enclosed = 0, npriv = 0;
    auto surface_ok = [&]() {
      return !bound_surface || ndofs - std::min(n_enclosed, limits->interior_max) <= limits->shared_max;
    };
    auto begin_build = [&]() {
      for (uint32_t c : cells) cell_batch[c] = NONE;
      cells.clear();
      cand.clear();
      ++stamp;
      ndofs = n_enclosed = npriv = 0;
    };
    auto add_cell = [&](uint32_t c) {
      cell_batch[c] = b;
      cells.push_back(c);
      npriv += priv_of(c);
      for (uint32_t i = 0; i < nd; ++i) {
        const uint32_t g = l2g[(uint64_t)c * nd + i];
        const bool first = dof_stamp[g] != stamp;
        if (bound_surface) {
          bool dup = false;
          for (uint32_t i2 = 0; i2 < i && !dup; ++i2) dup = l2g[(uint64_t)c * nd + i2] == g;
          if (!dup) {
            if (first) inc_cnt[g] = 0;
            if (++inc_cnt[g] == dc_off[g + 1] - dc_off[g] && !constrained[g]) ++n_enclosed;
          }
        }
        if (!first) continue;
        dof_stamp[g] = stamp;
        ++ndofs;
        if (Bmax_b == 1) continue;
        for (uint32_t k = dc_off[g]; k < dc_off[g + 1]; ++k) {
          const uint32_t c2 = dc[k];
          if (cell_batch[c2] != NONE || masked(c2) != cls) continue;
          if (gain_stamp[c2] != stamp) {
            gain_stamp[c2] = stamp;
            gain[c2] = 0;
            cand.push_back(c2);
          }
          gain[c2]++;
        }
      }
    };

    bool boxed = false;
    if (use_boxes && bound_surface && Bmax_b == Bmax) {
      for (const Shape &sh : shapes) {
        box.clear();
        bool ok = true;
        uint32_t cz = seed;
        for (uint32_t k = 0; k < sh.c && ok; ++k) {
          uint32_t cy = cz;
          for (uint32_t j = 0; j < sh.b && ok; ++j) {
            uint32_t cx = cy;
            for (uint32_t i = 0; i < sh.a && ok; ++i) {
              if (cx == NONE || cell_batch[cx] != NONE || masked(cx) != cls) {
                ok = false;
                break;
              }
              box.push_back(cx);
              cx = nbr[(size_t)cx * 6 + 1];
            }
            cy = cy == NONE ? NONE : nbr[(size_t)cy * 6 + 3];
            if (cy == NONE && j + 1 < sh.b) ok = false;
          }
          cz = cz == NONE ? NONE : nbr[(size_t)cz * 6 + 5];
          if (cz == NONE && k + 1 < sh.c) ok = false;
        }
        if (!ok) continue;
        begin_build();
        for (uint32_t c : box) add_cell(c);
        if (ndofs <= NBmax_b && surface_ok() && (!(cls && masked_planes) || npriv <= limits->private_max)) {
          boxed = true;
          break;
        }
      }
      if (!boxed) begin_build();
    } else {
      begin_build();
    }

    size_t last_ok = boxed ? cells.size() : 0;
    uint32_t next = boxed ? NONE : seed;
    while (true) {
      if (next != NONE) {
        add_cell(next);
        if (surface_ok()) last_ok = cells.size();
      }
      if (cells.size() >= Bmax_b) break;
      uint32_t best = NONE, best_gain = 0;
      size_t w = 0;
      for (size_t k = 0; k < cand.size(); ++k) {
        const uint32_t c2 = cand[k];
        if (cell_batch[c2] != NONE) continue;
        cand[w++] = c2;
        if (gain[c2] > best_gain) {
          best_gain = gain[c2];
          best = c2;
        }
      }
      cand.resize(w);
      if (best == NONE) break;
      if (ndofs + (nd - best_gain) > NBmax_b) break;
      if (cls && masked_planes && npriv + priv_of(best) > limits->private_max) break;
      next = best;
    }
    if (last_ok == 0) last_ok = 1;
    for (size_t k = last_ok; k < cells.size(); ++k) cell_batch[cells[k]] = NONE;
    cells.resize(last_ok);
    if (seed < nc && cell_batch[seed] != b) seed = 0;
  }
  if (segregate && !masked_planes) {
    std::vector<uint32_t> idx(batches.size());
    std::iota(idx.begin(), idx.end(), 0u);
    std::stable_sort(idx.begin(), idx.end(), [&](uint32_t a, uint32_t b2) { return batch_masked[a] < batch_masked[b2]; });
    std::vector<std::vector<uint32_t>> sorted_batches(batches.size());
    std::vector<uint8_t> sorted_masked(batches.size());
    for (size_t k = 0; k < idx.size(); ++k) {
      sorted_batches[k] = std::move(batches[idx[k]]);
      sorted_masked[k] = batch_masked[idx[k]];
    }
    batches.swap(sorted_batches);
    batch_masked.swap(sorted_masked);
  } else if (!segregate) {
    batch_masked.assign(batches.size(), 0);
  }
  uint32_t nb = (uint32_t)batches.size();
  if ((d.flags & MFGPU_HANGING_NODES) && d.constraint_mask)
    for (auto &cells : batches)
      std::stable_partition(cells.begin(), cells.end(), [&](uint32_t c) { return d.constraint_mask[c] != 0; });

  const uint32_t interior_max = limits ? limits->interior_max : 0u;
  std::vector<std::vector<uint32_t>> bd;
  std::vector<uint32_t> ntouch, nint;
  std::vector<uint8_t> shared_flag;
  for (;;) {
    nb = (uint32_t)batches.size();
    bd.assign(nb, {});
    ntouch.assign(N, 0);
    for (uint32_t b = 0; b < nb; ++b) {
      std::vector<uint32_t> &v = bd[b];
      v.reserve(batches[b].size() * nd);
      for (uint32_t c : batches[b])
        for (uint32_t i = 0; i < nd; ++i) v.push_back(l2g[(uint64_t)c * nd + i]);
      std::sort(v.begin(), v.end());
      v.erase(std::unique(v.begin(), v.end()), v.end());
      if (v.size() > (batch_masked[b] && !masked_planes ? NBmax1 : NBmax) || v.size() > 8191u) {
        set_error("internal: batch exceeds the kernel's dof slots (degenerate loc2glob?)");
        return MFGPU_EINVAL;
      }
      for (uint32_t g : v) ntouch[g]++;
    }
    shared_flag.assign(N, 0);
    for (uint32_t g = 0; g < N; ++g) shared_flag[g] = ntouch[g] >= 2;
    if (interior_max)
      for (uint32_t b = 0; b < nb; ++b)
        if (!batch_masked[b] || masked_planes)
          for (uint32_t g : bd[b])
            if (ntouch[g] == 1 && constrained[g]) shared_flag[g] = 1;
    nint.assign(nb, 0);
    std::vector<uint32_t> too_big;
    for (uint32_t b = 0; b < nb; ++b) {
      std::vector<uint32_t> &v = bd[b];
      std::stable_partition(v.begin(), v.end(), [&](uint32_t g) { return !shared_flag[g]; });
      uint32_t k = 0;
      while (k < v.size() && !shared_flag[v[k]]) ++k;
      if (interior_max && (!batch_masked[b] || masked_planes)) {
        uint32_t keep = std::min(k, interior_max);
        if (keep == v.size() && keep > 0) --keep;
        for (uint32_t t = keep; t < k; ++t) shared_flag[v[t]] = 1;
        k = keep;
        if (v.size() - k > limits->shared_max) too_big.push_back(b);
      }
      nint[b] = k;
    }
    if (too_big.empty()) break;
    for (size_t i = too_big.size(); i-- > 0;) {
      const uint32_t b = too_big[i];
      if (batches[b].size() < 2) {
        set_error("one cell has more pass-2 dofs than the plane kernel's dof-list slots hold");
        return MFGPU_EUNSUPPORTED;
      }
      const size_t half = batches[b].size() / 2;
      std::vector<uint32_t> second(batches[b].begin() + half, batches[b].end());
      batches[b].resize(half);
      batches.insert(batches.begin() + b + 1, std::move(second));
      batch_masked.insert(batch_masked.begin() + b + 1, batch_masked[b]);
    }
  }

  std::vector<uint64_t> dof_colors(N, 0);
  std::vector<uint32_t> bcolor(nb, 0);
  uint32_t ncolors = 0;
  for (uint32_t b = 0; b < nb; ++b) {
    uint64_t forbidden = 0;
    for (uint32_t g : bd[b]) forbidden |= dof_colors[g];
    uint32_t c = 0;
    while (c < 64 && (forbidden >> c) & 1) ++c;
    if (c >= 64) {
      set_error("more than 64 batch colours needed");
      return MFGPU_EUNSUPPORTED;
    }
    bcolor[b] = c;
    ncolors = std::max(ncolors, c + 1);
    for (uint32_t g : bd[b]) dof_colors[g] |= (1ull << c);
  }
  const bool colored = (d.flags & MFGPU_COLORED_SCATTER) != 0;
  std::vector<uint32_t> order(nb);
  std::iota(order.begin(), order.end(), 0u);
  if (colored) {
    std::stable_sort(order.begin(), order.end(),
                     [&](uint32_t a, uint32_t b2) { return bcolor[a] < bcolor[b2]; });
    P.color_batch_off.assign(ncolors + 1, 0);
    for (uint32_t b = 0; b < nb; ++b) P.color_batch_off[bcolor[b] + 1]++;
    for (uint32_t c = 0; c < ncolors; ++c) P.color_batch_off[c + 1] += P.color_batch_off[c];
  } else {
    P.color_batch_off.assign({0u, nb});
  }

  std::vector<uint32_t> rank_of(nb);
  for (uint32_t k = 0; k < nb; ++k) rank_of[order[k]] = k;
  std::vector<uint32_t> shared_ids;
  for (uint32_t g = 0; g < N; ++g)
    if (shared_flag[g]) shared_ids.push_back(g);
  const size_t ns = shared_ids.size();
  std::vector<uint32_t> sid(N, NONE), t_off(ns + 1, 0);
  for (size_t i = 0; i < ns; ++i) {
    sid[shared_ids[i]] = (uint32_t)i;
    t_off[i + 1] = t_off[i] + ntouch[shared_ids[i]];
  }
  std::vector<uint32_t> touchers(t_off[ns]);
  {
    std::vector<uint32_t> fill(t_off.begin(), t_off.end() - 1);
    for (uint32_t k = 0; k < nb; ++k)
      for (size_t t = nint[order[k]]; t < bd[order[k]].size(); ++t) touchers[fill[sid[bd[order[k]][t]]]++] = k;
  }
  auto seq_less = [&](uint32_t a, uint32_t b2) {
    const uint32_t la = t_off[a + 1] - t_off[a], lb = t_off[b2 + 1] - t_off[b2];
    const uint32_t *pa = &touchers[t_off[a]], *pb = &touchers[t_off[b2]];
    for (uint32_t i = 0; i < la && i < lb; ++i)
      if (pa[i] != pb[i]) return pa[i] < pb[i];
    if (la != lb) return la < lb;
    return a < b2;
  };
  auto same_group = [&](uint32_t a, uint32_t b2) {
    const uint32_t la = t_off[a + 1] - t_off[a], lb = t_off[b2 + 1] - t_off[b2];
    return la == lb && std::equal(&touchers[t_off[a]], &touchers[t_off[a]] + la, &touchers[t_off[b2]]);
  };
  std::vector<uint32_t> sorder(ns);
  std::iota(sorder.begin(), sorder.end(), 0u);
  std::sort(sorder.begin(), sorder.end(), seq_less);
  std::vector<uint32_t> spos(N, NONE);
  for (size_t i = 0; i < ns; ++i) spos[shared_ids[sorder[i]]] = (uint32_t)i;
  for (uint32_t b = 0; b < nb; ++b)
    std::sort(bd[b].begin() + nint[b], bd[b].end(), [&](uint32_t x, uint32_t y) { return spos[x] < spos[y]; });

  P.cell_order.clear();
  P.cell_order.reserve(nc);
  P.batch_cell_off.assign(1, 0);
  P.batch_dof_off.assign(1, 0);
  P.bdofs.clear();
  P.bflags.clear();
  P.lmap.assign((size_t)nc * nd, 0);
  std::vector<uint8_t> touched(N, 0);
  std::vector<uint16_t> pos_in_batch(N, 0);
  P.max_batch_dofs = P.max_batch_cells = 0;
  P.n_first = P.n_add = 0;
  P.batch_nint.clear();
  P.halo_off.assign(1, 0);
  for (uint32_t k = 0; k < nb; ++k) {
    const uint32_t b = order[k];
    const std::vector<uint32_t> &v = bd[b];
    P.batch_nint.push_back(nint[b]);
    P.halo_off.push_back(P.halo_off.back() +
                         (interior_max && (!batch_masked[b] || masked_planes) ? limits->halo_stride
                                                                              : (uint32_t)(v.size() - nint[b])));
    for (uint32_t g : v) {
      uint8_t f = 0;
      if (constrained[g]) f |= kFlagConstrained;
      if (touched[g]) {
        f |= kFlagAdd;
        ++P.n_add;
      } else {
        touched[g] = 1;
        ++P.n_first;
      }
      P.bdofs.push_back(g | (constrained[g] ? 0x80000000u : 0u));
      P.bflags.push_back(f);
    }
    for (size_t t = 0; t < v.size(); ++t) pos_in_batch[v[t]] = (uint16_t)t;
    for (uint32_t c : batches[b]) {
      const size_t pos = P.cell_order.size();
      P.cell_order.push_back(c);
      for (uint32_t i = 0; i < nd; ++i) P.lmap[pos * nd + i] = pos_in_batch[l2g[(uint64_t)c * nd + i]];
    }
    P.batch_cell_off.push_back((uint32_t)P.cell_order.size());
    P.batch_dof_off.push_back((uint32_t)P.bdofs.size());
    P.max_batch_dofs = std::max<uint32_t>(P.max_batch_dofs, (uint32_t)v.size());
    P.max_batch_cells = std::max<uint32_t>(P.max_batch_cells, (uint32_t)batches[b].size());
  }
  P.n_plane_batches = P.n_plain_plane_batches = 0;
  if (interior_max) {
    for (uint32_t k = 0; k < nb; ++k) {
      P.n_plain_plane_batches += batch_masked[order[k]] ? 0u : 1u;
      P.n_plane_batches += (batch_masked[order[k]] && !masked_planes) ? 0u : 1u;
    }
    if (masked_planes && P.n_plain_plane_batches < P.n_plane_batches) P.n_plain_plane_batches = 0;
  }
  P.orphans.clear();
  for (uint32_t g = 0; g < N; ++g)
    if (!touched[g]) P.orphans.push_back(g | (constrained[g] ? 0x80000000u : 0u));
  {
    P.sdofs.resize(ns);
    for (size_t i = 0; i < ns; ++i) {
      const uint32_t g = shared_ids[sorder[i]];
      P.sdofs[i] = g | (constrained[g] ? 0x80000000u : 0u);
    }
    P.s_off.assign(ns + 1, 0);
    for (size_t i = 0; i < ns; ++i) P.s_off[i + 1] = P.s_off[i] + ntouch[P.sdofs[i] & 0x7fffffffu];
    P.s_idx.assign(P.s_off[ns], 0);
    std::vector<uint32_t> fill(P.s_off.begin(), P.s_off.end() - 1);
    for (uint32_t k = 0; k < nb; ++k) {
      const uint32_t ni = P.batch_nint[k];
      const uint32_t d0 = P.batch_dof_off[k], d1 = P.batch_dof_off[k + 1];
      for (uint32_t t = d0 + ni; t < d1; ++t) {
        const uint32_t g = P.bdofs[t] & 0x7fffffffu;
        P.s_idx[fill[spos[g]]++] = P.halo_off[k] + (t - d0 - ni);
      }
    }
    P.chunks.clear();
    P.gstarts.clear();
    for (size_t i = 0; i < ns;) {
      size_t j = i + 1;
      while (j < ns && same_group(sorder[i], sorder[j])) ++j;
      const uint32_t k = P.s_off[i + 1] - P.s_off[i], tstart = (uint32_t)P.gstarts.size();
      for (uint32_t t = 0; t < k; ++t) P.gstarts.push_back(P.s_idx[P.s_off[i] + t]);
      for (size_t o = i; o < j; o += 64) {
        const uint32_t cnt = (uint32_t)std::min<size_t>(64, j - o);
        P.chunks.push_back((uint32_t)o);
        P.chunks.push_back(cnt | (k << 16));
        P.chunks.push_back(tstart);
        P.chunks.push_back((uint32_t)(o - i));
      }
      i = j;
    }
  }
  return 0;
}

int build_plane_records(Plan &P, const uint32_t *constraint_mask) {
  const int n = P.n, n2 = n * n, NT = p_cells_per_wave(n) * n, NIW = (n2 + 1) / 2;
  const int JI = p_ji(n) * 64, NB = p_kgu(n) * 64;
  const size_t nbat = P.n_plane_batches;
  const uint32_t dummy = 8u * (uint32_t)(NB - 1);
  std::vector<uint32_t> &bd = P.pr_dofs, &ix = P.pr_idx;
  bd.assign((size_t)NB * nbat, 0u);
  ix.assign((size_t)NIW * NT * nbat, dummy | (dummy << 16));
  std::vector<uint32_t> slot_of;
  const int HROWS = p_hn_rows(n), CR = p_priv_max(n) / 64;
  std::vector<uint32_t> &hnrec = P.pr_hn;
  hnrec.clear();
  P.pr_hn_slot.assign(nbat, 0xffffffffu);
  std::vector<HnLine> lines[3];
  std::vector<uint16_t> pnodes;
  std::vector<uint32_t> priv_pos((size_t)P.nd);
  for (size_t b = 0; b < nbat; ++b) {
    const uint32_t c0 = P.batch_cell_off[b], nc = P.batch_cell_off[b + 1] - c0;
    const uint32_t d0 = P.batch_dof_off[b], nbd = P.batch_dof_off[b + 1] - d0, ni = P.batch_nint[b];
    if ((int)nc * n > NT || (int)ni > JI || (int)(nbd - ni) >= NB - JI || nbd == ni) {
      set_error("internal: batch does not fit the plane kernel's dof-list slots");
      return MFGPU_EINVAL;
    }
    slot_of.assign(nbd, 0u);
    for (uint32_t t = 0; t < nbd; ++t) slot_of[t] = t < ni ? t : (uint32_t)JI + (t - ni);
    for (int t = 0; t < NB; ++t) {
      uint32_t src_t;
      if (t < JI) src_t = (uint32_t)t < ni ? (uint32_t)t : ni;
      else src_t = std::min<uint32_t>(ni + (uint32_t)(t - JI), nbd - 1);
      bd[b * NB + t] = P.bdofs[d0 + src_t];
    }
    bool hnb = false;
    if (constraint_mask && b >= P.n_plain_plane_batches)
      for (uint32_t c = 0; c < nc; ++c) hnb = hnb || constraint_mask[P.cell_order[c0 + c]] != 0;
    uint32_t next_priv = (uint32_t)NB;
    std::vector<uint32_t> copies, ops_d[3];
    for (uint32_t c = 0; c < nc; ++c) {
      const unsigned mask = hnb ? constraint_mask[P.cell_order[c0 + c]] : 0u;
      std::fill(priv_pos.begin(), priv_pos.end(), 0xffffffffu);
      if (mask) {
        hn_cell_lines(mask, n, lines, pnodes);
        for (uint16_t node : pnodes) {
          if (next_priv >= (uint32_t)NB + (uint32_t)p_priv_max(n)) {
            set_error("internal: batch exceeds the plane kernel's private hanging-node entries");
            return MFGPU_EINVAL;
          }
          priv_pos[node] = next_priv;
          copies.push_back((next_priv << 16) | slot_of[P.lmap[(size_t)(c0 + c) * P.nd + node]]);
          ++next_priv;
        }
        for (int dir = 0; dir < 3; ++dir)
          for (const HnLine &L : lines[dir]) {
            uint32_t w[3] = {0u, 0u, 0u};
            for (int t = 0; t < n; ++t) w[t >> 1] |= priv_pos[L.node[t]] << (16 * (t & 1));
            ops_d[dir].insert(ops_d[dir].end(), w, w + 3);
          }
      }
      for (int k = 0; k < n; ++k)
        for (int i = 0; i < n2; ++i) {
          const int node = i + n2 * k;
          const uint32_t pos = priv_pos[node] != 0xffffffffu ? priv_pos[node] : slot_of[P.lmap[(size_t)(c0 + c) * P.nd + node]];
          const uint32_t off = 8u * pos;
          uint32_t &w = ix[(b * NIW + i / 2) * NT + c * n + k];
          w = (i & 1) ? ((w & 0xffffu) | (off << 16)) : ((w & 0xffff0000u) | off);
        }
    }
    if (hnb) {
      P.pr_hn_slot[b] = (uint32_t)(hnrec.size() / ((size_t)HROWS * 64));
      hnrec.resize(hnrec.size() + (size_t)HROWS * 64, 0u);
      uint32_t *rec = hnrec.data() + (size_t)P.pr_hn_slot[b] * HROWS * 64;
      for (size_t e = 0; e < copies.size(); ++e) rec[e] = copies[e];
      for (int dir = 0; dir < 3; ++dir) {
        const size_t nops = ops_d[dir].size() / 3;
        if (nops > (size_t)kHnOpRounds * 64) {
          set_error("internal: more hanging-node lines in a batch than the plane kernel's record holds");
          return MFGPU_EINVAL;
        }
        for (size_t e = 0; e < nops; ++e)
          for (int w = 0; w < 3; ++w)
            rec[(size_t)(CR + (dir * kHnOpRounds + (int)(e / 64)) * 3 + w) * 64 + e % 64] = ops_d[dir][e * 3 + w];
      }
      const uint32_t h0 = (uint32_t)copies.size() | ((uint32_t)(ops_d[0].size() / 3) << 16);
      const uint32_t h1 = (uint32_t)(ops_d[1].size() / 3) | ((uint32_t)(ops_d[2].size() / 3) << 16);
      for (int l = 0; l < 64; ++l) {
        rec[(size_t)(HROWS - 2) * 64 + l] = h0;
        rec[(size_t)(HROWS - 1) * 64 + l] = h1;
      }
    }
  }
  return 0;
}

int choose_kernel_and_plan(const mfgpu_desc &d, PlaneKernel &pk, BatchKernel &bk, Plan &plan) {
  const bool general = !(d.flags & MFGPU_UNIFORM_J0), hn = (d.flags & MFGPU_HANGING_NODES) != 0;
  const bool colored = (d.flags & MFGPU_COLORED_SCATTER) != 0;
  if (d.kernel > MFGPU_KERNEL_PLANES_2W) {
    set_error("unknown mfgpu_desc.kernel");
    return MFGPU_EINVAL;
  }
  const bool pk_ok = d.dim == 3 && !general && !colored && d.degree >= 2 && d.degree <= 6 &&
                     d.n_dofs < (1u << 29);
  const bool xk_ok = d.dim == 3 && !general && !colored;
  const bool want_planes = d.kernel == MFGPU_KERNEL_PLANES || d.kernel == MFGPU_KERNEL_PLANES_2W;
  if ((want_planes && !pk_ok) || (d.kernel == MFGPU_KERNEL_PENCILS_X && !xk_ok) ||
      (d.kernel == MFGPU_KERNEL_PENCILS && general)) {
    set_error("mfgpu_desc.kernel: this kernel family does not cover the description (see include/mfgpu.h)");
    return MFGPU_EUNSUPPORTED;
  }
  bool planes = pk_ok && (want_planes || (d.kernel == MFGPU_KERNEL_AUTO &&
                                     (d.degree >= 4 || (d.degree == 3 && (hn || d.number_type == MFGPU_F64)))));
  bool pencils_x = xk_ok && !planes && d.kernel != MFGPU_KERNEL_PENCILS;
  PlanLimits lim;
  if (planes) {
    lim.max_cells = (uint32_t)p_cells_per_wave(d.degree + 1);
    lim.max_dofs = (uint32_t)p_kgu(d.degree + 1) * 64u - 1u;
    lim.interior_max = (uint32_t)p_ji(d.degree + 1) * 64u;
    lim.halo_stride = (uint32_t)p_hs(d.degree + 1) * 64u;
    lim.shared_max = lim.halo_stride - 1u;
    lim.segregate_masked = hn;
    lim.masked_planes = hn && d.degree <= 4;
    lim.private_max = (uint32_t)p_priv_max(d.degree + 1);
  }
  int rc = build_plan(d, plan, (pencils_x && d.degree == 3) ? 4u : 3u, planes ? &lim : nullptr);
  if (rc == MFGPU_EUNSUPPORTED && planes && d.kernel == MFGPU_KERNEL_AUTO && xk_ok) {
    planes = false;
    pencils_x = true;
    plan = Plan();
    rc = build_plan(d, plan, d.degree == 3 ? 4u : 3u, nullptr);
  }
  if (!rc && planes) {
    const uint32_t nbat = (uint32_t)plan.batch_cell_off.size() - 1;
    pencils_x = plan.n_plane_batches < nbat;
    if (plan.n_plane_batches == 0) planes = false;
  }
  const bool planes4 = d.kernel == MFGPU_KERNEL_PLANES_2W || d.degree >= 5 ||
                       (d.kernel == MFGPU_KERNEL_AUTO && d.degree == 3 && d.number_type == MFGPU_F64);
  pk = !planes ? PlaneKernel::none : planes4 ? PlaneKernel::planes4 : PlaneKernel::planes3;
  bk = pencils_x ? BatchKernel::x : general ? (d.dim == 2 ? BatchKernel::g2 : BatchKernel::g)
                                   : planes ? BatchKernel::none : BatchKernel::batches;
  assert(rc || (pk != PlaneKernel::none) == (plan.n_plane_batches > 0));
  return rc;
}

}

extern "C" {

const char *mfgpu_last_error(void) { return mfgpu::last_error(); }

int mfgpu_plan_create(const mfgpu_desc *desc, mfgpu_plan **out) {
  if (!desc || !out) {
    mfgpu::set_error("null argument");
    return MFGPU_EINVAL;
  }
  mfgpu_plan *p = new mfgpu_plan();
  mfgpu::PlaneKernel pk;
  mfgpu::BatchKernel bk;
  int rc = mfgpu::choose_kernel_and_plan(*desc, pk, bk, p->plan);
  if (!rc && pk != mfgpu::PlaneKernel::none) rc = mfgpu::build_plane_records(p->plan, desc->constraint_mask);
  if (rc) {
    delete p;
    return rc;
  }
  *out = p;
  return 0;
}

void mfgpu_plan_destroy(mfgpu_plan *p) { delete p; }

int mfgpu_suggest_renumbering(const mfgpu_desc *desc, uint32_t *new_index) {
  if (!desc || !new_index) {
    mfgpu::set_error("null argument");
    return MFGPU_EINVAL;
  }
  mfgpu::Plan P;
  mfgpu::PlaneKernel pk;
  mfgpu::BatchKernel bk;
  int rc = mfgpu::choose_kernel_and_plan(*desc, pk, bk, P);
  if (rc) return rc;
  const uint32_t NONE = 0xffffffffu;
  std::fill(new_index, new_index + desc->n_dofs, NONE);
  uint32_t next = 0;
  const size_t nb = P.batch_cell_off.size() - 1;
  for (size_t b = 0; b < nb; ++b) {
    const uint32_t d0 = P.batch_dof_off[b];
    const uint32_t ni = P.batch_nint.empty() ? P.batch_dof_off[b + 1] - d0 : P.batch_nint[b];
    for (uint32_t t = 0; t < ni; ++t) {
      const uint32_t g = P.bdofs[d0 + t] & 0x7fffffffu;
      if (new_index[g] == NONE) new_index[g] = next++;
    }
  }
  for (uint32_t e : P.sdofs) {
    const uint32_t g = e & 0x7fffffffu;
    if (new_index[g] == NONE) new_index[g] = next++;
  }
  for (uint32_t g = 0; g < desc->n_dofs; ++g)
    if (new_index[g] == NONE) new_index[g] = next++;
  if (next != desc->n_dofs) {
    mfgpu::set_error("internal: renumbering is not a permutation");
    return MFGPU_EINVAL;
  }
  return 0;
}

int64_t mfgpu_plan_array_u32(const mfgpu_plan *p, int what, const uint32_t **ptr) {
  if (!p || !ptr) return MFGPU_EINVAL;
  const std::vector<uint32_t> *v = nullptr;
  switch (what) {
    case 0: v = &p->plan.batch_cell_off; break;
    case 1: v = &p->plan.batch_dof_off; break;
    case 2: v = &p->plan.color_batch_off; break;
    case 3: v = &p->plan.cell_order; break;
    case 4: v = &p->plan.bdofs; break;
    case 5: v = &p->plan.orphans; break;
    case 6: v = &p->plan.batch_nint; break;
    case 7: v = &p->plan.halo_off; break;
    case 8: v = &p->plan.sdofs; break;
    case 9: v = &p->plan.s_off; break;
    case 10: v = &p->plan.s_idx; break;
    case 11: v = &p->plan.chunks; break;
    case 12: v = &p->plan.gstarts; break;
    case 13: v = &p->plan.pr_dofs; break;
    case 14: v = &p->plan.pr_idx; break;
    case 15: v = &p->plan.pr_hn; break;
    case 16: v = &p->plan.pr_hn_slot; break;
    default: mfgpu::set_error("bad array id"); return MFGPU_EINVAL;
  }
  *ptr = v->data();
  return (int64_t)v->size();
}

int64_t mfgpu_plan_lmap(const mfgpu_plan *p, const uint16_t **ptr) {
  if (!p || !ptr) return MFGPU_EINVAL;
  *ptr = p->plan.lmap.data();
  return (int64_t)p->plan.lmap.size();
}

int64_t mfgpu_plan_bflags(const mfgpu_plan *p, const uint8_t **ptr) {
  if (!p || !ptr) return MFGPU_EINVAL;
  *ptr = p->plan.bflags.data();
  return (int64_t)p->plan.bflags.size();
}

}
```

dealii-cuda_amd/pymfgpu/__init__.py:

```python
from __future__ import annotations

import ctypes as C
import os

import numpy as np

_HERE = os.path.dirname(os.path.abspath(__file__))
LIB_PATH = os.environ.get("MFGPU_LIB") or os.path.join(os.path.dirname(_HERE), "lib", "libmfgpu.so")

F64, F32 = 0, 1
OK, EINVAL = 0, -1
UNIFORM_J0, HANGING_NODES, COLORED_SCATTER = 1, 2, 1 << 8
KERNEL_AUTO, KERNEL_PENCILS, KERNEL_PENCILS_X, KERNEL_PLANES, KERNEL_PLANES_2W = 0, 1, 2, 3, 4


class MfgpuError(RuntimeError):
    pass


class Desc(C.Structure):
    _fields_ = [
        ("dim", C.c_int32), ("degree", C.c_int32), ("number_type", C.c_int32), ("flags", C.c_uint32),
        ("n_dofs", C.c_uint32), ("n_cells", C.c_uint32),
        ("loc2glob", C.c_void_p), ("constraint_mask", C.c_void_p),
        ("JxW", C.c_void_p), ("inv_jac", C.c_void_p), ("coefficient", C.c_void_p),
        ("quadrature_points", C.c_void_p), ("shape_values", C.c_void_p), ("shape_gradients", C.c_void_p),
        ("constraint_weights", C.c_void_p), ("constrained_dofs", C.c_void_p),
        ("n_constrained", C.c_uint32), ("max_cells_per_batch", C.c_uint32), ("max_dofs_per_batch", C.c_uint32),
        ("kernel", C.c_uint32), ("cell_loop_segments", C.c_uint32), ("max_workgroups", C.c_uint32),
    ]


SYMBOLS = [
    "mfgpu_create", "mfgpu_vmult", "mfgpu_vmult_add", "mfgpu_n_dofs", "mfgpu_memory_consumption",
    "mfgpu_destroy", "mfgpu_last_error", "mfgpu_plan_stats", "mfgpu_kernel_name", "mfgpu_compute_inverse_diagonal", "mfgpu_set_constrained_values",
    "mfgpu_vec_sadd", "mfgpu_vec_equ", "mfgpu_vec_scale", "mfgpu_vec_divide", "mfgpu_vec_invert", "mfgpu_vec_mul",
    "mfgpu_vec_dot", "mfgpu_vec_l2_norm", "mfgpu_vec_add_and_dot", "mfgpu_vec_all_zero", "mfgpu_profile_enable", "mfgpu_profile_read", "mfgpu_profile_read_pass2",
    "mfgpu_plan_create", "mfgpu_plan_destroy", "mfgpu_plan_array_u32", "mfgpu_plan_lmap", "mfgpu_plan_bflags",
    "mfgpu_vec_alloc", "mfgpu_vec_free", "mfgpu_vec_fill", "mfgpu_vec_from_host", "mfgpu_vec_to_host",
    "mfgpu_device_synchronize", "mfgpu_device_memory_info", "mfgpu_mesh_create_uniform", "mfgpu_mesh_create_adaptive", "mfgpu_mesh_create_ball", "mfgpu_mesh_create_from_leaves",
    "mfgpu_mesh_cell_levels", "mfgpu_mesh_destroy",
    "mfgpu_mesh_desc", "mfgpu_mesh_dof_coords", "mfgpu_mesh_interface_dofs",
    "mfgpu_dist_unique_id", "mfgpu_dist_create", "mfgpu_dist_connect_local", "mfgpu_dist_attach", "mfgpu_dist_schedule",
    "mfgpu_vmult_dist_begin", "mfgpu_vmult_dist_end", "mfgpu_vmult_dist", "mfgpu_dist_destroy",
    "mfgpu_transfer_create", "mfgpu_transfer_create_from_meshes", "mfgpu_transfer_prolongate",
    "mfgpu_transfer_restrict_and_add", "mfgpu_transfer_memory_consumption", "mfgpu_transfer_destroy",
    "mfgpu_mesh_transfer_patches", "mfgpu_suggest_renumbering", "mfgpu_mesh_renumber",
    "mfgpu_level_create", "mfgpu_level_operator", "mfgpu_level_vmult_interface_down", "mfgpu_level_vmult_interface_up",
    "mfgpu_level_destroy", "mfgpu_index_pairs_create", "mfgpu_vec_copy_pairs", "mfgpu_index_pairs_destroy",
    "mfgpu_mesh_create_adaptive_mg", "mfgpu_mg_hierarchy_create", "mfgpu_mg_n_levels", "mfgpu_mg_level_mesh",
    "mfgpu_mg_edge_dofs", "mfgpu_mg_copy_pairs", "mfgpu_mg_transfer_arrays", "mfgpu_mg_hierarchy_destroy",
    "mfgpu_integrator_create", "mfgpu_integrator_rhs", "mfgpu_integrator_l2_error", "mfgpu_integrator_error_points",
    "mfgpu_integrator_destroy",
    "mfgpu_vec_convert", "mfgpu_vec_copy_pairs_convert", "mfgpu_vec_chebyshev_start", "mfgpu_vec_chebyshev_update",
]

_lib = None


def lib():
    global _lib
    if _lib is None:
        if not os.path.exists(LIB_PATH):
            raise MfgpuError(f"{LIB_PATH} not found: build it with __graft_entry__.build() "
                             "(make -C dealii-cuda_amd); there is no fallback path")
        L = C.CDLL(LIB_PATH)
        L.mfgpu_last_error.restype = C.c_char_p
        L.mfgpu_create.argtypes = [C.POINTER(Desc), C.POINTER(C.c_void_p)]
        L.mfgpu_vmult.argtypes = [C.c_void_p, C.c_void_p, C.c_void_p, C.c_void_p]
        L.mfgpu_vmult_add.argtypes = [C.c_void_p, C.c_void_p, C.c_void_p, C.c_void_p]
        L.mfgpu_n_dofs.argtypes = [C.c_void_p]
        L.mfgpu_n_dofs.restype = C.c_uint32
        L.mfgpu_memory_consumption.argtypes = [C.c_void_p]
        L.mfgpu_memory_consumption.restype = C.c_size_t
        L.mfgpu_destroy.argtypes = [C.c_void_p]
        L.mfgpu_destroy.restype = None
        L.mfgpu_plan_stats.argtypes = [C.c_void_p, C.POINTER(C.c_uint64)]
        L.mfgpu_device_memory_info.argtypes = [C.POINTER(C.c_size_t), C.POINTER(C.c_size_t)]
        L.mfgpu_kernel_name.argtypes = [C.c_void_p]
        L.mfgpu_kernel_name.restype = C.c_char_p
        L.mfgpu_compute_inverse_diagonal.argtypes = [C.c_void_p, C.c_void_p, C.c_void_p]
        L.mfgpu_set_constrained_values.argtypes = [C.c_void_p, C.c_void_p, C.c_double, C.c_void_p]
        vp, d, z, i = C.c_void_p, C.c_double, C.c_size_t, C.c_int
        L.mfgpu_vec_sadd.argtypes = [vp, d, d, vp, z, i, vp]
        L.mfgpu_vec_equ.argtypes = [vp, d, vp, z, i, vp]
        L.mfgpu_vec_scale.argtypes = [vp, vp, z, i, vp]
        L.mfgpu_vec_divide.argtypes = [vp, vp, z, i, vp]
        L.mfgpu_vec_invert.argtypes = [vp, z, i, vp]
        L.mfgpu_vec_mul.argtypes = [vp, d, z, i, vp]
        L.mfgpu_vec_dot.argtypes = [vp, vp, z, i, vp, C.POINTER(d)]
        L.mfgpu_vec_l2_norm.argtypes = [vp, z, i, vp, C.POINTER(d)]
        L.mfgpu_vec_add_and_dot.argtypes = [vp, d, vp, vp, z, i, vp, C.POINTER(d)]
        L.mfgpu_vec_all_zero.argtypes = [vp, z, i, vp, C.POINTER(i)]
        L.mfgpu_profile_enable.argtypes = [C.c_void_p, C.c_int]
        L.mfgpu_profile_read.argtypes = [C.c_void_p, C.POINTER(C.c_double), C.POINTER(C.c_uint64)]
        L.mfgpu_profile_read_pass2.argtypes = [C.c_void_p, C.POINTER(C.c_double)]
        L.mfgpu_plan_create.argtypes = [C.POINTER(Desc), C.POINTER(C.c_void_p)]
        L.mfgpu_plan_destroy.argtypes = [C.c_void_p]
        L.mfgpu_plan_destroy.restype = None
        L.mfgpu_plan_array_u32.argtypes = [C.c_void_p, C.c_int, C.POINTER(C.c_void_p)]
        L.mfgpu_plan_array_u32.restype = C.c_int64
        L.mfgpu_plan_lmap.argtypes = [C.c_void_p, C.POINTER(C.c_void_p)]
        L.mfgpu_plan_lmap.restype = C.c_int64
        L.mfgpu_plan_bflags.argtypes = [C.c_void_p, C.POINTER(C.c_void_p)]
        L.mfgpu_plan_bflags.restype = C.c_int64
        L.mfgpu_vec_alloc.argtypes = [C.POINTER(C.c_void_p), C.c_size_t, C.c_int]
        L.mfgpu_vec_free.argtypes = [C.c_void_p]
        L.mfgpu_vec_fill.argtypes = [C.c_void_p, C.c_size_t, C.c_int, C.c_double, C.c_void_p]
        L.mfgpu_vec_from_host.argtypes = [C.c_void_p, C.c_void_p, C.c_size_t, C.c_int]
        L.mfgpu_vec_to_host.argtypes = [C.c_void_p, C.c_void_p, C.c_size_t, C.c_int]
        L.mfgpu_mesh_create_uniform.argtypes = [C.c_int, C.c_int, C.POINTER(C.c_uint32), C.c_double, C.c_double,
                                                C.c_uint32, C.c_uint32, C.c_int, C.POINTER(C.c_void_p)]
        L.mfgpu_mesh_create_adaptive.argtypes = [C.c_int, C.c_int, C.c_int, C.c_int, C.POINTER(C.c_void_p)]
        L.mfgpu_mesh_create_ball.argtypes = [C.c_int, C.c_int, C.c_int, C.c_int, C.POINTER(C.c_void_p)]
        L.mfgpu_mesh_create_from_leaves.argtypes = [C.c_int, C.c_int, C.c_void_p, C.c_uint32, C.c_int, C.POINTER(C.c_void_p)]
        L.mfgpu_mesh_cell_levels.argtypes = [C.c_void_p, C.POINTER(C.c_void_p)]
        L.mfgpu_mesh_cell_levels.restype = C.c_int64
        L.mfgpu_mesh_destroy.argtypes = [C.c_void_p]
        L.mfgpu_mesh_destroy.restype = None
        L.mfgpu_mesh_desc.argtypes = [C.c_void_p, C.POINTER(Desc)]
        L.mfgpu_mesh_dof_coords.argtypes = [C.c_void_p, C.POINTER(C.c_void_p)]
        L.mfgpu_mesh_dof_coords.restype = C.c_int64
        L.mfgpu_mesh_interface_dofs.argtypes = [C.c_void_p, C.c_int, C.POINTER(C.c_void_p)]
        L.mfgpu_mesh_interface_dofs.restype = C.c_int64
        L.mfgpu_transfer_create.argtypes = [C.c_int, C.c_int, C.c_int, C.c_uint32, C.c_void_p, C.c_void_p, C.c_uint32,
                                            C.c_uint32, C.c_void_p, C.c_uint32, C.c_void_p, C.POINTER(C.c_void_p)]
        L.mfgpu_transfer_create_from_meshes.argtypes = [C.c_void_p, C.c_void_p, C.POINTER(C.c_void_p)]
        L.mfgpu_transfer_prolongate.argtypes = [C.c_void_p, C.c_void_p, C.c_void_p, C.c_void_p]
        L.mfgpu_transfer_restrict_and_add.argtypes = [C.c_void_p, C.c_void_p, C.c_void_p, C.c_void_p]
        L.mfgpu_transfer_memory_consumption.argtypes = [C.c_void_p]
        L.mfgpu_transfer_memory_consumption.restype = C.c_size_t
        L.mfgpu_mesh_transfer_patches.argtypes = [C.c_void_p, C.c_void_p, C.c_void_p, C.c_void_p]
        L.mfgpu_mesh_transfer_patches.restype = C.c_int64
        L.mfgpu_suggest_renumbering.argtypes = [C.POINTER(Desc), C.c_void_p]
        L.mfgpu_mesh_renumber.argtypes = [C.c_void_p, C.c_void_p]
        L.mfgpu_level_create.argtypes = [C.POINTER(Desc), C.c_void_p, C.c_uint32, C.POINTER(C.c_void_p)]
        L.mfgpu_level_operator.argtypes = [C.c_void_p]
        L.mfgpu_level_operator.restype = C.c_void_p
        L.mfgpu_level_vmult_interface_down.argtypes = [C.c_void_p, C.c_void_p, C.c_void_p, C.c_void_p]
        L.mfgpu_level_vmult_interface_up.argtypes = [C.c_void_p, C.c_void_p, C.c_void_p, C.c_void_p]
        L.mfgpu_mesh_create_adaptive_mg.argtypes = [C.c_int, C.c_int, C.c_int, C.c_int, C.POINTER(C.c_void_p)]
        L.mfgpu_mg_hierarchy_create.argtypes = [C.c_void_p, C.POINTER(C.c_void_p)]
        L.mfgpu_mg_n_levels.argtypes = [C.c_void_p]
        L.mfgpu_mg_level_mesh.argtypes = [C.c_void_p, C.c_int]
        L.mfgpu_mg_level_mesh.restype = C.c_void_p
        L.mfgpu_mg_edge_dofs.argtypes = [C.c_void_p, C.c_int, C.POINTER(C.c_void_p)]
        L.mfgpu_mg_edge_dofs.restype = C.c_int64
        L.mfgpu_mg_copy_pairs.argtypes = [C.c_void_p, C.c_int, C.POINTER(C.c_void_p), C.POINTER(C.c_void_p)]
        L.mfgpu_mg_copy_pairs.restype = C.c_int64
        L.mfgpu_mg_transfer_arrays.argtypes = [C.c_void_p, C.c_int, C.POINTER(C.c_void_p), C.POINTER(C.c_void_p)]
        L.mfgpu_mg_transfer_arrays.restype = C.c_int64
        L.mfgpu_mg_hierarchy_destroy.argtypes = [C.c_void_p]
        L.mfgpu_mg_hierarchy_destroy.restype = None
        L.mfgpu_index_pairs_create.argtypes = [C.c_void_p, C.c_void_p, C.c_uint32, C.POINTER(C.c_void_p)]
        L.mfgpu_vec_copy_pairs.argtypes = [C.c_void_p, C.c_void_p, C.c_void_p, C.c_int, C.c_void_p]
        L.mfgpu_index_pairs_destroy.argtypes = [C.c_void_p]
        L.mfgpu_index_pairs_destroy.restype = None
        L.mfgpu_level_destroy.argtypes = [C.c_void_p]
        L.mfgpu_level_destroy.restype = None
        L.mfgpu_transfer_destroy.argtypes = [C.c_void_p]
        L.mfgpu_transfer_destroy.restype = None
        L.mfgpu_integrator_create.argtypes = [C.POINTER(Desc), C.POINTER(C.c_void_p)]
        L.mfgpu_integrator_rhs.argtypes = [C.c_void_p, C.c_void_p, C.c_void_p, C.c_void_p, C.c_void_p]
        L.mfgpu_integrator_l2_error.argtypes = [C.c_void_p, C.c_void_p, C.c_void_p, C.c_void_p, C.c_void_p,
                                                C.POINTER(C.c_double)]
        L.mfgpu_integrator_error_points.argtypes = [C.c_void_p, C.c_void_p, C.c_void_p]
        L.mfgpu_integrator_destroy.argtypes = [C.c_void_p]
        L.mfgpu_integrator_destroy.restype = None
        L.mfgpu_vec_convert.argtypes = [vp, i, vp, i, z, vp]
        L.mfgpu_vec_copy_pairs_convert.argtypes = [vp, vp, i, vp, i, vp]
        L.mfgpu_vec_chebyshev_start.argtypes = [vp, vp, vp, vp, vp, vp, d, i, z, i, vp]
        L.mfgpu_vec_chebyshev_update.argtypes = [vp, vp, vp, vp, vp, d, d, z, i, vp]
        _lib = L
    return _lib


def _check(rc):
    if rc != 0:
        raise MfgpuError(f"mfgpu error {rc}: {lib().mfgpu_last_error().decode()}")


def np_dtype(number_type):
    return np.float64 if number_type == F64 else np.float32


def _view(ptr, count, dtype):
    if count <= 0 or not ptr:
        return np.zeros(0, dtype=dtype)
    buf = (C.c_char * (count * np.dtype(dtype).itemsize)).from_address(ptr)
    return np.frombuffer(buf, dtype=dtype, count=count)


class Mesh:

    def __init__(self, handle, keep=None):
        self._h = handle
        self._keep = keep
        self.desc = Desc()
        _check(lib().mfgpu_mesh_desc(self._h, C.byref(self.desc)))

    @classmethod
    def uniform(cls, dim, degree, n_per_dir, lo=-1.0, hi=1.0, slab=(0, 0), number_type=F64):
        if np.isscalar(n_per_dir):
            n_per_dir = [int(n_per_dir)] * dim
        arr = (C.c_uint32 * 3)(*(list(n_per_dir) + [1] * (3 - len(n_per_dir))))
        h = C.c_void_p()
        _check(lib().mfgpu_mesh_create_uniform(dim, degree, arr, lo, hi, slab[0], slab[1], number_type, C.byref(h)))
        return cls(h)

    @classmethod
    def adaptive(cls, dim, degree, n_ref, number_type=F64):
        h = C.c_void_p()
        _check(lib().mfgpu_mesh_create_adaptive(dim, degree, n_ref, number_type, C.byref(h)))
        return cls(h)

    @classmethod
    def adaptive_mg(cls, dim, degree, n_ref, number_type=F64):
        h = C.c_void_p()
        _check(lib().mfgpu_mesh_create_adaptive_mg(dim, degree, n_ref, number_type, C.byref(h)))
        return cls(h)

    @classmethod
    def ball(cls, dim, degree, n_ref, number_type=F64):
        h = C.c_void_p()
        _check(lib().mfgpu_mesh_create_ball(dim, degree, n_ref, number_type, C.byref(h)))
        return cls(h)

    @classmethod
    def from_leaves(cls, dim, degree, leaves, number_type=F64):
        lv = np.ascontiguousarray(leaves, dtype=np.uint32).reshape(-1, 4)
        h = C.c_void_p()
        _check(lib().mfgpu_mesh_create_from_leaves(dim, degree, lv.ctypes.data, len(lv), number_type, C.byref(h)))
        return cls(h)

    def cell_levels(self):
        p = C.c_void_p()
        cnt = lib().mfgpu_mesh_cell_levels(self._h, C.byref(p))
        return _view(p.value, cnt, np.uint32).reshape(-1, 4).copy()

    def __del__(self):
        if getattr(self, "_h", None) and _lib is not None and getattr(self, "_owner", None) is None:
            _lib.mfgpu_mesh_destroy(self._h)
            self._h = None

    @property
    def n_dofs(self):
        return int(self.desc.n_dofs)

    @property
    def n_cells(self):
        return int(self.desc.n_cells)

    @property
    def nd(self):
        return (self.desc.degree + 1) ** self.desc.dim

    def arrays(self):
        d = self.desc
        dt = np_dtype(d.number_type)
        nd, nc, n = self.nd, d.n_cells, d.degree + 1
        out = dict(
            loc2glob=_view(d.loc2glob, nc * nd, np.uint32).reshape(nc, nd),
            JxW=_view(d.JxW, nc * nd, dt).reshape(nc, nd),
            inv_jac=(_view(d.inv_jac, nc, dt) if d.flags & UNIFORM_J0
                     else _view(d.inv_jac, nc * nd * d.dim * d.dim, dt).reshape(nc, nd, d.dim, d.dim)),
            quadrature_points=_view(d.quadrature_points, nc * nd * d.dim, dt).reshape(nc, nd, d.dim),
            shape_values=_view(d.shape_values, n * n, dt),
            shape_gradients=_view(d.shape_gradients, n * n, dt),
            constraint_weights=_view(d.constraint_weights, n * n, np.float64),
            constrained_dofs=_view(d.constrained_dofs, d.n_constrained, np.uint32),
            constraint_mask=_view(d.constraint_mask, nc, np.uint32) if d.constraint_mask else None,
        )
        return out

    def dof_coords(self):
        p = C.c_void_p()
        cnt = lib().mfgpu_mesh_dof_coords(self._h, C.byref(p))
        return _view(p.value, cnt, np.float64).reshape(-1, self.desc.dim)

    def suggest_renumbering(self):
        out = np.zeros(self.n_dofs, dtype=np.uint32)
        _check(lib().mfgpu_suggest_renumbering(C.byref(self.desc), out.ctypes.data))
        return out

    def renumber(self, new_index):
        ni = np.ascontiguousarray(new_index, dtype=np.uint32)
        assert ni.size == self.n_dofs
        _check(lib().mfgpu_mesh_renumber(self._h, ni.ctypes.data))
        _check(lib().mfgpu_mesh_desc(self._h, C.byref(self.desc)))

    def transfer_patches(self, fine: "Mesh"):
        p, dim = self.desc.degree, self.desc.dim
        cd = np.zeros((self.n_cells, (p + 1) ** dim), dtype=np.uint32)
        fd = np.zeros((self.n_cells, (2 * p + 1) ** dim), dtype=np.uint32)
        rc = lib().mfgpu_mesh_transfer_patches(self._h, fine._h, cd.ctypes.data, fd.ctypes.data)
        if rc < 0:
            _check(int(rc))
        return cd, fd

    def interface_dofs(self, which):
        p = C.c_void_p()
        cnt = lib().mfgpu_mesh_interface_dofs(self._h, which, C.byref(p))
        return _view(p.value, cnt, np.uint32).copy()


def make_desc(dim, degree, n_dofs, loc2glob, JxW, inv_jac, coefficient, constrained,
              shape_values, shape_gradients, number_type=F64, constraint_mask=None,
              constraint_weights=None, quadrature_points=None, max_cells_per_batch=0, max_dofs_per_batch=0,
              colored=False, kernel=0, cell_loop_segments=0, max_workgroups=0):
    dt = np_dtype(number_type)
    keep = []

    def ptr(a, dtype):
        if a is None:
            return None
        a = np.ascontiguousarray(a, dtype=dtype)
        keep.append(a)
        return a.ctypes.data

    d = Desc()
    d.dim, d.degree, d.number_type = dim, degree, number_type
    l2g = np.ascontiguousarray(loc2glob, dtype=np.uint32)
    d.n_dofs = int(n_dofs)
    d.n_cells = l2g.size // ((degree + 1) ** dim)
    uniform = np.asarray(inv_jac).size == d.n_cells
    assert uniform or np.asarray(inv_jac).size == l2g.size * dim * dim
    d.flags = ((UNIFORM_J0 if uniform else 0) | (HANGING_NODES if constraint_mask is not None else 0)
               | (COLORED_SCATTER if colored else 0))
    d.loc2glob = ptr(l2g, np.uint32)
    d.constraint_mask = ptr(constraint_mask, np.uint32)
    d.JxW = ptr(JxW, dt)
    d.inv_jac = ptr(inv_jac, dt)
    d.coefficient = ptr(coefficient, dt)
    d.quadrature_points = ptr(quadrature_points, dt)
    d.shape_values = ptr(shape_values, dt)
    d.shape_gradients = ptr(shape_gradients, dt)
    d.constraint_weights = ptr(constraint_weights, np.float64)
    c = np.ascontiguousarray(constrained, dtype=np.uint32)
    d.constrained_dofs = ptr(c, np.uint32)
    d.n_constrained = c.size
    d.max_cells_per_batch = max_cells_per_batch
    d.max_dofs_per_batch = max_dofs_per_batch
    d.kernel = kernel
    d.cell_loop_segments = cell_loop_segments
    d.max_workgroups = max_workgroups
    return d, keep


class Plan:

    def __init__(self, desc: Desc, keep=None):
        self._keep = keep
        self.nd = (desc.degree + 1) ** desc.dim
        h = C.c_void_p()
        _check(lib().mfgpu_plan_create(C.byref(desc), C.byref(h)))
        self._h = h

    def __del__(self):
        if getattr(self, "_h", None) and _lib is not None:
            _lib.mfgpu_plan_destroy(self._h)
            self._h = None

    def _u32(self, what):
        p = C.c_void_p()
        cnt = lib().mfgpu_plan_array_u32(self._h, what, C.byref(p))
        if cnt < 0:
            _check(int(cnt))
        return _view(p.value, cnt, np.uint32).copy()

    batch_cell_off = property(lambda s: s._u32(0))
    batch_dof_off = property(lambda s: s._u32(1))
    color_batch_off = property(lambda s: s._u32(2))
    cell_order = property(lambda s: s._u32(3))
    bdofs = property(lambda s: s._u32(4) & np.uint32(0x7fffffff))
    bdofs_constrained = property(lambda s: (s._u32(4) >> np.uint32(31)).astype(bool))
    orphans = property(lambda s: s._u32(5))
    batch_nint = property(lambda s: s._u32(6))
    halo_off = property(lambda s: s._u32(7))
    sdofs = property(lambda s: s._u32(8))
    s_off = property(lambda s: s._u32(9))
    s_idx = property(lambda s: s._u32(10))
    chunks = property(lambda s: s._u32(11).reshape(-1, 4))
    gstarts = property(lambda s: s._u32(12))
    pr_dofs = property(lambda s: s._u32(13))
    pr_idx = property(lambda s: s._u32(14))
    pr_hn = property(lambda s: s._u32(15))
    pr_hn_slot = property(lambda s: s._u32(16))

    @property
    def lmap(self):
        p = C.c_void_p()
        cnt = lib().mfgpu_plan_lmap(self._h, C.byref(p))
        return _view(p.value, cnt, np.uint16).reshape(-1, self.nd).copy()

    @property
    def bflags(self):
        p = C.c_void_p()
        cnt = lib().mfgpu_plan_bflags(self._h, C.byref(p))
        return _view(p.value, cnt, np.uint8).copy()


class DeviceVector:

    def __init__(self, n, number_type=F64):
        self.n, self.number_type = int(n), number_type
        p = C.c_void_p()
        _check(lib().mfgpu_vec_alloc(C.byref(p), self.n, number_type))
        self.ptr = p.value

    def __del__(self):
        if getattr(self, "ptr", None) and _lib is not None:
            _lib.mfgpu_vec_free(self.ptr)
            self.ptr = None

    def fill(self, value, stream=None):
        _check(lib().mfgpu_vec_fill(self.ptr, self.n, self.number_type, float(value), stream))

    def from_host(self, a):
        a = np.ascontiguousarray(a, dtype=np_dtype(self.number_type))
        assert a.size == self.n
        _check(lib().mfgpu_vec_from_host(self.ptr, a.ctypes.data, self.n, self.number_type))

    def to_host(self):
        a = np.empty(self.n, dtype=np_dtype(self.number_type))
        _check(lib().mfgpu_vec_to_host(a.ctypes.data, self.ptr, self.n, self.number_type))
        return a

    def swap(self, other):
        self.ptr, other.ptr = other.ptr, self.ptr
        self.n, other.n = other.n, self.n

    def _a(self, other=None):
        if other is not None:
            assert other.n == self.n and other.number_type == self.number_type
        return self.n, self.number_type

    def sadd(self, s, a, w, stream=None):
        _check(lib().mfgpu_vec_sadd(self.ptr, float(s), float(a), w.ptr, *self._a(w), stream))

    def add(self, a, w, stream=None):
        self.sadd(1.0, a, w, stream)

    def equ(self, a, w, stream=None):
        _check(lib().mfgpu_vec_equ(self.ptr, float(a), w.ptr, *self._a(w), stream))

    def scale(self, w, stream=None):
        _check(lib().mfgpu_vec_scale(self.ptr, w.ptr, *self._a(w), stream))

    def divide(self, w, stream=None):
        _check(lib().mfgpu_vec_divide(self.ptr, w.ptr, *self._a(w), stream))

    def invert(self, stream=None):
        _check(lib().mfgpu_vec_invert(self.ptr, *self._a(), stream))

    def mul(self, a, stream=None):
        _check(lib().mfgpu_vec_mul(self.ptr, float(a), *self._a(), stream))

    def dot(self, w, stream=None):
        r = C.c_double()
        _check(lib().mfgpu_vec_dot(self.ptr, w.ptr, *self._a(w), stream, C.byref(r)))
        return r.value

    def l2_norm(self, stream=None):
        r = C.c_double()
        _check(lib().mfgpu_vec_l2_norm(self.ptr, *self._a(), stream, C.byref(r)))
        return r.value

    def add_and_dot(self, a, x, w, stream=None):
        r = C.c_double()
        self._a(x)
        _check(lib().mfgpu_vec_add_and_dot(self.ptr, float(a), x.ptr, w.ptr, *self._a(w), stream, C.byref(r)))
        return r.value

    def all_zero(self, stream=None):
        r = C.c_int()
        _check(lib().mfgpu_vec_all_zero(self.ptr, *self._a(), stream, C.byref(r)))
        return bool(r.value)


class Operator:

    def __init__(self, desc: Desc, keep=None):
        self._keep = keep
        self.number_type = desc.number_type
        h = C.c_void_p()
        _check(lib().mfgpu_create(C.byref(desc), C.byref(h)))
        self._h = h

    def __del__(self):
        self.clear()

    def clear(self):
        if getattr(self, "_h", None) and _lib is not None:
            _lib.mfgpu_destroy(self._h)
            self._h = None

    def n(self):
        return int(lib().mfgpu_n_dofs(self._h))

    m = n

    def vmult(self, dst, src, stream=None):
        _check(lib().mfgpu_vmult(self._h, _ptr(dst), _ptr(src), stream))

    def vmult_add(self, dst, src, stream=None):
        _check(lib().mfgpu_vmult_add(self._h, _ptr(dst), _ptr(src), stream))

    def memory_consumption(self):
        return int(lib().mfgpu_memory_consumption(self._h))

    def plan_stats(self):
        s = (C.c_uint64 * 8)()
        _check(lib().mfgpu_plan_stats(self._h, s))
        keys = ["n_batches", "n_launches", "batch_dofs", "max_batch_dofs", "max_batch_cells", "n_orphans",
                "first_touch_or_shared_dofs", "rmw_adds_or_halo_slots"]
        return dict(zip(keys, [int(v) for v in s]))

    def kernel_name(self):
        return lib().mfgpu_kernel_name(self._h).decode()

    def compute_inverse_diagonal(self, inv_diag, stream=None):
        _check(lib().mfgpu_compute_inverse_diagonal(self._h, _ptr(inv_diag), stream))

    def set_constrained_values(self, vec, value, stream=None):
        _check(lib().mfgpu_set_constrained_values(self._h, _ptr(vec), float(value), stream))

    def profile_enable(self, on=True):
        _check(lib().mfgpu_profile_enable(self._h, int(on)))

    def profile_read(self):
        ms, nv = C.c_double(), C.c_uint64()
        _check(lib().mfgpu_profile_read(self._h, C.byref(ms), C.byref(nv)))
        return ms.value, int(nv.value)

    def profile_read_pass2(self):
        ms = C.c_double()
        _check(lib().mfgpu_profile_read_pass2(self._h, C.byref(ms)))
        return ms.value


class Integrator:

    def __init__(self, desc: Desc, keep=None):
        self._keep = keep
        self.dim, self.degree, self.n_cells = int(desc.dim), int(desc.degree), int(desc.n_cells)
        h = C.c_void_p()
        _check(lib().mfgpu_integrator_create(C.byref(desc), C.byref(h)))
        self._h = h

    def __del__(self):
        if getattr(self, "_h", None) and _lib is not None:
            _lib.mfgpu_integrator_destroy(self._h)
            self._h = None

    @property
    def n_error_points(self):
        return (self.degree + 2) ** self.dim

    def rhs(self, dst, f=None, u_b=None, stream=None):
        _check(lib().mfgpu_integrator_rhs(self._h, _ptr(dst), None if f is None else _ptr(f),
                                          None if u_b is None else _ptr(u_b), stream))

    def l2_error(self, u, exact=None, per_cell=None, stream=None):
        r = C.c_double()
        _check(lib().mfgpu_integrator_l2_error(self._h, _ptr(u), None if exact is None else _ptr(exact),
                                               None if per_cell is None else _ptr(per_cell), stream, C.byref(r)))
        return r.value

    def error_points(self):
        v = DeviceVector(self.n_cells * self.n_error_points * self.dim)
        _check(lib().mfgpu_integrator_error_points(self._h, v.ptr, None))
        return v.to_host().reshape(self.n_cells, self.n_error_points, self.dim)


class MgHierarchy:

    def __init__(self, mesh: "Mesh"):
        h = C.c_void_p()
        _check(lib().mfgpu_mg_hierarchy_create(mesh._h, C.byref(h)))
        self._h = h
        self.n_levels = int(lib().mfgpu_mg_n_levels(h))

    def level_mesh(self, level):
        m = Mesh.__new__(Mesh)
        m._owner = self
        m._h = C.c_void_p(lib().mfgpu_mg_level_mesh(self._h, level))
        m.desc = Desc()
        _check(lib().mfgpu_mesh_desc(m._h, C.byref(m.desc)))
        return m

    def edge_dofs(self, level):
        p = C.c_void_p()
        n = lib().mfgpu_mg_edge_dofs(self._h, level, C.byref(p))
        return _view(p.value, n, np.uint32).copy()

    def copy_pairs(self, level):
        a, b = C.c_void_p(), C.c_void_p()
        n = lib().mfgpu_mg_copy_pairs(self._h, level, C.byref(a), C.byref(b))
        return _view(a.value, n, np.uint32).copy(), _view(b.value, n, np.uint32).copy()

    def transfer_arrays(self, level, nd, nfd):
        a, b = C.c_void_p(), C.c_void_p()
        n = lib().mfgpu_mg_transfer_arrays(self._h, level, C.byref(a), C.byref(b))
        return _view(a.value, n * nd, np.uint32).reshape(n, nd).copy(), _view(b.value, n * nfd, np.uint32).reshape(n, nfd).copy()

    def __del__(self):
        if getattr(self, "_h", None) and _lib is not None:
            _lib.mfgpu_mg_hierarchy_destroy(self._h)
            self._h = None


class Level:

    def __init__(self, desc: Desc, edge_dofs, keep=None):
        self._keep = keep
        e = np.ascontiguousarray(edge_dofs, dtype=np.uint32)
        h = C.c_void_p()
        _check(lib().mfgpu_level_create(C.byref(desc), e.ctypes.data if e.size else None, e.size, C.byref(h)))
        self._h = h
        self.number_type = desc.number_type

    def vmult(self, dst, src, stream=None):
        _check(lib().mfgpu_vmult(lib().mfgpu_level_operator(self._h), _ptr(dst), _ptr(src), stream))

    def compute_inverse_diagonal(self, inv_diag, stream=None):
        _check(lib().mfgpu_compute_inverse_diagonal(lib().mfgpu_level_operator(self._h), _ptr(inv_diag), stream))

    def vmult_interface_down(self, dst, src, stream=None):
        _check(lib().mfgpu_level_vmult_interface_down(self._h, _ptr(dst), _ptr(src), stream))

    def vmult_interface_up(self, dst, src, stream=None):
        _check(lib().mfgpu_level_vmult_interface_up(self._h, _ptr(dst), _ptr(src), stream))

    def __del__(self):
        if getattr(self, "_h", None) and _lib is not None:
            _lib.mfgpu_level_destroy(self._h)
            self._h = None


class Transfer:

    def __init__(self, handle):
        self._h = handle

    @classmethod
    def from_arrays(cls, dim, degree, coarse_cell_dofs, fine_patch_dofs, n_coarse_dofs, n_fine_dofs, coarse_dirichlet,
                    number_type=F64, prolongation_1d=None):
        cd = np.ascontiguousarray(coarse_cell_dofs, dtype=np.uint32)
        fd = np.ascontiguousarray(fine_patch_dofs, dtype=np.uint32)
        di = np.ascontiguousarray(coarse_dirichlet, dtype=np.uint32)
        p1 = None if prolongation_1d is None else np.ascontiguousarray(prolongation_1d, dtype=np.float64)
        n_cells = cd.size // ((degree + 1) ** dim)
        assert fd.size == n_cells * (2 * degree + 1) ** dim
        h = C.c_void_p()
        _check(lib().mfgpu_transfer_create(dim, degree, number_type, n_cells, cd.ctypes.data, fd.ctypes.data, n_coarse_dofs,
                                           n_fine_dofs, di.ctypes.data if di.size else None, di.size,
                                           None if p1 is None else p1.ctypes.data, C.byref(h)))
        return cls(h)

    @classmethod
    def from_meshes(cls, coarse: "Mesh", fine: "Mesh"):
        h = C.c_void_p()
        _check(lib().mfgpu_transfer_create_from_meshes(coarse._h, fine._h, C.byref(h)))
        return cls(h)

    def prolongate(self, dst_fine, src_coarse, stream=None):
        _check(lib().mfgpu_transfer_prolongate(self._h, _ptr(dst_fine), _ptr(src_coarse), stream))

    def restrict_and_add(self, dst_coarse, src_fine, stream=None):
        _check(lib().mfgpu_transfer_restrict_and_add(self._h, _ptr(dst_coarse), _ptr(src_fine), stream))

    def memory_consumption(self):
        return int(lib().mfgpu_transfer_memory_consumption(self._h))

    def __del__(self):
        if getattr(self, "_h", None) and _lib is not None:
            _lib.mfgpu_transfer_destroy(self._h)
            self._h = None


def _ptr(v):
    if isinstance(v, DeviceVector):
        return v.ptr
    if hasattr(v, "data_ptr"):
        return v.data_ptr()
    return int(v)


class IndexPairs:

    def __init__(self, dst_idx, src_idx):
        a = np.ascontiguousarray(dst_idx, dtype=np.uint32)
        b = np.ascontiguousarray(src_idx, dtype=np.uint32)
        assert a.size == b.size
        h = C.c_void_p()
        _check(lib().mfgpu_index_pairs_create(a.ctypes.data if a.size else None, b.ctypes.data if b.size else None,
                                              a.size, C.byref(h)))
        self._h = h

    def copy(self, dst, src, number_type=F64, stream=None):
        _check(lib().mfgpu_vec_copy_pairs(self._h, _ptr(dst), _ptr(src), number_type, stream))

    def __del__(self):
        if getattr(self, "_h", None) and _lib is not None:
            _lib.mfgpu_index_pairs_destroy(self._h)
            self._h = None


def vec_convert(dst, dst_type, src, src_type, n, stream=None, check=True):
    rc = lib().mfgpu_vec_convert(_ptr(dst), dst_type, _ptr(src), src_type, n, stream)
    return _check(rc) if check else rc


def copy_pairs_convert(pairs: "IndexPairs", dst, dst_type, src, src_type, stream=None, check=True):
    rc = lib().mfgpu_vec_copy_pairs_convert(pairs._h, _ptr(dst), dst_type, _ptr(src), src_type, stream)
    return _check(rc) if check else rc


def chebyshev_start(x, upd, r, b, t, dinv, f, zero_start, n, number_type, stream=None, check=True):
    rc = lib().mfgpu_vec_chebyshev_start(_ptr(x), _ptr(upd), _ptr(r), _ptr(b), None if t is None else _ptr(t),
                                         _ptr(dinv), float(f), 1 if zero_start else 0, n, number_type, stream)
    return _check(rc) if check else rc


def chebyshev_update(x, upd, r, t, dinv, f1, f2, n, number_type, stream=None, check=True):
    rc = lib().mfgpu_vec_chebyshev_update(_ptr(x), _ptr(upd), _ptr(r), _ptr(t), _ptr(dinv), float(f1), float(f2), n,
                                          number_type, stream)
    return _check(rc) if check else rc


def synchronize():
    _check(lib().mfgpu_device_synchronize())


def device_memory_info():
    f, t = C.c_size_t(), C.c_size_t()
    _check(lib().mfgpu_device_memory_info(C.byref(f), C.byref(t)))
    return f.value, t.value


def dist_unique_id() -> bytes:
    buf = C.create_string_buffer(128)
    _check(lib().mfgpu_dist_unique_id(buf))
    return buf.raw


class Dist:

    def __init__(self, mesh: "Mesh", rank: int, world: int, unique_id=None):
        lo = np.ascontiguousarray(mesh.interface_dofs(0), dtype=np.uint32)
        up = np.ascontiguousarray(mesh.interface_dofs(1), dtype=np.uint32)
        con = np.ascontiguousarray(mesh.arrays()["constrained_dofs"], dtype=np.uint32)
        self._keep = (lo, up, con)
        self.number_type = mesh.desc.number_type
        d = C.c_void_p()
        L = lib()
        L.mfgpu_dist_create.argtypes = [C.c_char_p, C.c_int, C.c_int, C.c_void_p, C.c_uint32, C.c_void_p, C.c_uint32,
                                        C.c_void_p, C.c_uint32, C.c_uint32, C.c_int, C.c_void_p]
        _check(L.mfgpu_dist_create(unique_id, rank, world, lo.ctypes.data if lo.size else None, lo.size,
                                   up.ctypes.data if up.size else None, up.size, con.ctypes.data if con.size else None,
                                   con.size, mesh.n_dofs, self.number_type, C.byref(d)))
        self._d = d
        for f in ("mfgpu_dist_connect_local", "mfgpu_dist_attach"):
            getattr(L, f).argtypes = [C.c_void_p, C.c_void_p]
        L.mfgpu_vmult_dist_begin.argtypes = [C.c_void_p, C.c_void_p, C.c_void_p, C.c_void_p, C.c_void_p]
        L.mfgpu_vmult_dist.argtypes = [C.c_void_p, C.c_void_p, C.c_void_p, C.c_void_p, C.c_void_p]
        L.mfgpu_vmult_dist_end.argtypes = [C.c_void_p, C.c_void_p, C.c_void_p, C.c_void_p]
        L.mfgpu_dist_destroy.argtypes = [C.c_void_p]

    def __del__(self):
        if getattr(self, "_d", None) and _lib is not None:
            _lib.mfgpu_dist_destroy(self._d)
            self._d = None

    def connect_local(self, upper: "Dist"):
        _check(lib().mfgpu_dist_connect_local(self._d, upper._d))

    def attach(self, op: "Operator"):
        _check(lib().mfgpu_dist_attach(self._d, op._h))

    def schedule(self):
        info = (C.c_uint32 * 4)()
        lib().mfgpu_dist_schedule.argtypes = [C.c_void_p, C.c_void_p]
        _check(lib().mfgpu_dist_schedule(self._d, info))
        return bool(info[0]), int(info[1]), int(info[2]), int(info[3])

    def vmult_begin(self, op, dst, src, stream=None):
        _check(lib().mfgpu_vmult_dist_begin(op._h, self._d, _ptr(dst), _ptr(src), stream))

    def vmult_end(self, op, dst, stream=None):
        _check(lib().mfgpu_vmult_dist_end(op._h, self._d, _ptr(dst), stream))

    def vmult(self, op, dst, src, stream=None):
        _check(lib().mfgpu_vmult_dist(op._h, self._d, _ptr(dst), _ptr(src), stream))
```

include/mfgpu.h:

```cpp
#ifndef MFGPU_H
#define MFGPU_H

#include <stddef.h>
#include <stdint.h>

#ifdef __cplusplus
extern "C" {
#endif

#define MFGPU_OK 0
#define MFGPU_EINVAL (-1)
#define MFGPU_EHIP (-2)
#define MFGPU_ENOMEM (-3)
#define MFGPU_EUNSUPPORTED (-4)

#define MFGPU_F64 0
#define MFGPU_F32 1

#define MFGPU_UNIFORM_J0 (1u << 0)
#define MFGPU_HANGING_NODES (1u << 1)

#define MFGPU_COLORED_SCATTER (1u << 8)

typedef struct mfgpu_handle mfgpu_handle;

typedef struct mfgpu_desc {
  int32_t dim;
  int32_t degree;
  int32_t number_type;
  uint32_t flags;
  uint32_t n_dofs;
  uint32_t n_cells;
  const uint32_t *loc2glob;
  const uint32_t *constraint_mask;
  const void *JxW;
  const void *inv_jac;
  const void *coefficient;
  const void *quadrature_points;
  const void *shape_values;
  const void *shape_gradients;
  const double *constraint_weights;
  const uint32_t *constrained_dofs;
  uint32_t n_constrained;
  uint32_t max_cells_per_batch;
  uint32_t max_dofs_per_batch;
  uint32_t kernel;
  uint32_t cell_loop_segments;
  uint32_t max_workgroups;
} mfgpu_desc;

#define MFGPU_KERNEL_AUTO 0
#define MFGPU_KERNEL_PENCILS 1
#define MFGPU_KERNEL_PENCILS_X 2
#define MFGPU_KERNEL_PLANES 3
#define MFGPU_KERNEL_PLANES_2W 4


int mfgpu_create(const mfgpu_desc *desc, mfgpu_handle **out);

int mfgpu_vmult(mfgpu_handle *h, void *dst_dev, const void *src_dev, void *stream);

int mfgpu_vmult_add(mfgpu_handle *h, void *dst_dev, const void *src_dev, void *stream);

uint32_t mfgpu_n_dofs(const mfgpu_handle *h);

size_t mfgpu_memory_consumption(const mfgpu_handle *h);

void mfgpu_destroy(mfgpu_handle *h);

const char *mfgpu_last_error(void);

int mfgpu_plan_stats(const mfgpu_handle *h, uint64_t stats[8]);

const char *mfgpu_kernel_name(const mfgpu_handle *h);

int mfgpu_profile_enable(mfgpu_handle *h, int on);
int mfgpu_profile_read(mfgpu_handle *h, double *kernel_ms_total, uint64_t *n_vmults);
int mfgpu_profile_read_pass2(mfgpu_handle *h, double *pass2_ms_total);

typedef struct mfgpu_plan mfgpu_plan;
int mfgpu_plan_create(const mfgpu_desc *desc, mfgpu_plan **out);
void mfgpu_plan_destroy(mfgpu_plan *p);
int64_t mfgpu_plan_array_u32(const mfgpu_plan *p, int what, const uint32_t **ptr);
int64_t mfgpu_plan_lmap(const mfgpu_plan *p, const uint16_t **ptr);
int64_t mfgpu_plan_bflags(const mfgpu_plan *p, const uint8_t **ptr);

int mfgpu_suggest_renumbering(const mfgpu_desc *desc, uint32_t *new_index );

int mfgpu_compute_inverse_diagonal(mfgpu_handle *h, void *inv_diag, void *stream);
int mfgpu_set_constrained_values(mfgpu_handle *h, void *vec, double value, void *stream);

int mfgpu_vec_sadd(void *v, double s, double a, const void *w, size_t n, int number_type, void *stream);
int mfgpu_vec_equ(void *v, double a, const void *w, size_t n, int number_type, void *stream);
int mfgpu_vec_scale(void *v, const void *w, size_t n, int number_type, void *stream);
int mfgpu_vec_divide(void *v, const void *w, size_t n, int number_type, void *stream);
int mfgpu_vec_invert(void *v, size_t n, int number_type, void *stream);
int mfgpu_vec_mul(void *v, double a, size_t n, int number_type, void *stream);
int mfgpu_vec_dot(const void *v, const void *w, size_t n, int number_type, void *stream, double *result);
int mfgpu_vec_l2_norm(const void *v, size_t n, int number_type, void *stream, double *result);
int mfgpu_vec_add_and_dot(void *v, double a, const void *x, const void *w, size_t n, int number_type,
                          void *stream, double *result);
int mfgpu_vec_all_zero(const void *v, size_t n, int number_type, void *stream, int *result);

int mfgpu_vec_alloc(void **dev, size_t n, int number_type);
int mfgpu_vec_free(void *dev);
int mfgpu_vec_fill(void *dev, size_t n, int number_type, double value, void *stream);
int mfgpu_vec_from_host(void *dev, const void *host, size_t n, int number_type);
int mfgpu_vec_to_host(void *host, const void *dev, size_t n, int number_type);
int mfgpu_device_synchronize(void);
int mfgpu_device_memory_info(size_t *free_bytes, size_t *total_bytes);

typedef struct mfgpu_dist mfgpu_dist;
int mfgpu_dist_unique_id(void *id128);
int mfgpu_dist_create(const void *id128, int rank, int world, const uint32_t *lower_ids, uint32_t n_lower,
                      const uint32_t *upper_ids, uint32_t n_upper, const uint32_t *constrained_dofs,
                      uint32_t n_constrained, uint32_t n_dofs, int number_type, mfgpu_dist **out);
int mfgpu_dist_connect_local(mfgpu_dist *lower_rank, mfgpu_dist *upper_rank);
int mfgpu_dist_attach(mfgpu_dist *d, mfgpu_handle *h);
int mfgpu_dist_schedule(const mfgpu_dist *d, uint32_t info[4]);
int mfgpu_vmult_dist_begin(mfgpu_handle *h, mfgpu_dist *d, void *dst_dev, const void *src_dev, void *stream);
int mfgpu_vmult_dist_end(mfgpu_handle *h, mfgpu_dist *d, void *dst_dev, void *stream);
int mfgpu_vmult_dist(mfgpu_handle *h, mfgpu_dist *d, void *dst_dev, const void *src_dev, void *stream);
void mfgpu_dist_destroy(mfgpu_dist *d);

typedef struct mfgpu_transfer mfgpu_transfer;
int mfgpu_transfer_create(int dim, int degree, int number_type, uint32_t n_coarse_cells,
                          const uint32_t *coarse_cell_dofs ,
                          const uint32_t *fine_patch_dofs  , uint32_t n_coarse_dofs,
                          uint32_t n_fine_dofs, const uint32_t *coarse_dirichlet, uint32_t n_coarse_dirichlet,
                          const double *prolongation_1d ,
                          mfgpu_transfer **out);
int mfgpu_transfer_prolongate(mfgpu_transfer *t, void *dst_fine_dev, const void *src_coarse_dev, void *stream);
int mfgpu_transfer_restrict_and_add(mfgpu_transfer *t, void *dst_coarse_dev, const void *src_fine_dev, void *stream);
size_t mfgpu_transfer_memory_consumption(const mfgpu_transfer *t);
void mfgpu_transfer_destroy(mfgpu_transfer *t);

typedef struct mfgpu_level mfgpu_level;
int mfgpu_level_create(const mfgpu_desc *desc, const uint32_t *edge_dofs, uint32_t n_edge, mfgpu_level **out);
mfgpu_handle *mfgpu_level_operator(mfgpu_level *level);
int mfgpu_level_vmult_interface_down(mfgpu_level *level, void *dst_dev, const void *src_dev, void *stream);
int mfgpu_level_vmult_interface_up(mfgpu_level *level, void *dst_dev, const void *src_dev, void *stream);
void mfgpu_level_destroy(mfgpu_level *level);

typedef struct mfgpu_index_pairs mfgpu_index_pairs;
int mfgpu_index_pairs_create(const uint32_t *dst_idx, const uint32_t *src_idx, uint32_t n, mfgpu_index_pairs **out);
int mfgpu_vec_copy_pairs(const mfgpu_index_pairs *p, void *dst_dev, const void *src_dev, int number_type, void *stream);
void mfgpu_index_pairs_destroy(mfgpu_index_pairs *p);

int mfgpu_vec_convert(void *dst, int dst_type, const void *src, int src_type, size_t n, void *stream);
int mfgpu_vec_copy_pairs_convert(const mfgpu_index_pairs *p, void *dst, int dst_type, const void *src, int src_type,
                                 void *stream);
int mfgpu_vec_chebyshev_start(void *x, void *upd, void *r, const void *b, const void *t, const void *dinv, double f,
                              int zero_start, size_t n, int number_type, void *stream);
int mfgpu_vec_chebyshev_update(void *x, void *upd, void *r, const void *t, const void *dinv, double f1, double f2,
                               size_t n, int number_type, void *stream);

typedef struct mfgpu_integrator mfgpu_integrator;
int mfgpu_integrator_create(const mfgpu_desc *desc, mfgpu_integrator **out);
int mfgpu_integrator_rhs(mfgpu_integrator *it, void *rhs, const void *f_qp, const void *u_b, void *stream);
int mfgpu_integrator_l2_error(mfgpu_integrator *it, const void *u, const void *exact, void *per_cell, void *stream,
                              double *l2);
int mfgpu_integrator_error_points(mfgpu_integrator *it, void *points, void *stream);
void mfgpu_integrator_destroy(mfgpu_integrator *it);

typedef struct mfgpu_mesh mfgpu_mesh;

int mfgpu_mesh_create_uniform(int dim, int degree, const uint32_t *n_per_dir, double lo, double hi,
                              uint32_t slab_begin, uint32_t slab_end, int number_type,
                              mfgpu_mesh **out);
int mfgpu_mesh_create_adaptive(int dim, int degree, int n_ref, int number_type, mfgpu_mesh **out);
int mfgpu_mesh_create_ball(int dim, int degree, int n_ref, int number_type, mfgpu_mesh **out);
int mfgpu_transfer_create_from_meshes(const mfgpu_mesh *coarse, const mfgpu_mesh *fine, mfgpu_transfer **out);
int64_t mfgpu_mesh_transfer_patches(const mfgpu_mesh *coarse, const mfgpu_mesh *fine, uint32_t *coarse_cell_dofs,
                                    uint32_t *fine_patch_dofs);
int mfgpu_mesh_renumber(mfgpu_mesh *m, const uint32_t *new_index);
int mfgpu_mesh_create_adaptive_mg(int dim, int degree, int n_ref, int number_type, mfgpu_mesh **out);
typedef struct mfgpu_mg_hierarchy mfgpu_mg_hierarchy;
int mfgpu_mg_hierarchy_create(const mfgpu_mesh *adaptive, mfgpu_mg_hierarchy **out);
int mfgpu_mg_n_levels(const mfgpu_mg_hierarchy *h);
const mfgpu_mesh *mfgpu_mg_level_mesh(const mfgpu_mg_hierarchy *h, int level);
int64_t mfgpu_mg_edge_dofs(const mfgpu_mg_hierarchy *h, int level, const uint32_t **ptr);
int64_t mfgpu_mg_copy_pairs(const mfgpu_mg_hierarchy *h, int level, const uint32_t **active_dofs, const uint32_t **level_dofs);
int64_t mfgpu_mg_transfer_arrays(const mfgpu_mg_hierarchy *h, int level, const uint32_t **coarse_cell_dofs,
                                 const uint32_t **fine_patch_dofs);
void mfgpu_mg_hierarchy_destroy(mfgpu_mg_hierarchy *h);
int mfgpu_mesh_create_from_leaves(int dim, int degree, const uint32_t *leaves, uint32_t n_leaves,
                                  int number_type, mfgpu_mesh **out);
int64_t mfgpu_mesh_cell_levels(const mfgpu_mesh *m, const uint32_t **ptr);
void mfgpu_mesh_destroy(mfgpu_mesh *m);
int mfgpu_mesh_desc(const mfgpu_mesh *m, mfgpu_desc *desc);
int64_t mfgpu_mesh_dof_coords(const mfgpu_mesh *m, const double **ptr);
int64_t mfgpu_mesh_interface_dofs(const mfgpu_mesh *m, int which, const uint32_t **ptr);

#ifdef __cplusplus
}
#endif
#endif
```

Before: 73.07 billion DoFs/s.

## Deduplicate plane index records and pass-2 reduction records via shared per-batch tables

Per-batch dof and index records are stored relative to a per-batch base offset and deduplicated, so the plane kernel reads a small shared record set through a metadata table instead of streaming expanded per-batch index arrays. Pass 2 gets an owner-batch reduction kernel that uses shared records encoding halo slots relative to the owning batch. The aim is to cut index-stream DRAM traffic in this bandwidth-bound operator on a uniform mesh. In exchange the kernel does extra readlane metadata loads, drops nontemporal loads for the shared records, and adds a new pass-2 kernel launch path.

```diff
diff --git a/dealii-cuda_amd/csrc/mfgpu_api.hip b/dealii-cuda_amd/csrc/mfgpu_api.hip
--- a/dealii-cuda_amd/csrc/mfgpu_api.hip
+++ b/dealii-cuda_amd/csrc/mfgpu_api.hip
@@ -62,6 +62,9 @@
   DeviceArray<uint16_t> d_lmapx;
   DeviceArray<uint16_t> d_perm;
   DeviceArray<uint32_t> d_bdofsp, d_idxp;
+  DeviceArray<uint32_t> d_shtab;
+  bool shared_records = false;
+  size_t record_bytes = 0;
   DeviceArray<uint32_t> d_hnrec;
   DeviceArray<uint32_t> d_hn_slot;
   DeviceArray<void> d_coefp;
@@ -77,6 +80,8 @@
   std::vector<uint32_t> seg_end;
   std::vector<DeviceArray<uint32_t>> d_p2arr, d_p2tiles;
   std::vector<uint32_t> n_p2tiles;
+  DeviceArray<uint32_t> d_p2rec, d_p2tab;
+  bool p2_shared = false, p2_reverse = false, no_shared_records = false;
   Stream side;
   std::vector<Event> ev_seg;
   Event ev_side;
@@ -183,6 +188,7 @@
     prio[priority[i]] = 1;
   }
   const size_t ng = 1 + h->seg_end.size();
+  const bool shared = P.sh_p2_use && !h->no_shared_records && n_priority == 0 && ng == 2;
   std::vector<std::vector<uint32_t>> sd(ng), so(ng, std::vector<uint32_t>(1, 0u)), si(ng);
   auto add = [&](uint32_t dof, const uint32_t *slots, uint32_t k, size_t seg) {
     const size_t g = prio[dof & 0x7fffffffu] ? 0 : 1 + seg;
@@ -192,6 +198,7 @@
   };
   for (size_t i = 0; i < P.sdofs.size(); ++i) {
     size_t seg = 0;
+    if (shared && P.s_off[i + 1] > P.s_off[i]) continue;
     if (P.s_off[i + 1] > P.s_off[i]) {
       const uint32_t slot = P.s_idx[P.s_off[i + 1] - 1];
       const uint32_t batch = (uint32_t)(std::upper_bound(P.halo_off.begin(), P.halo_off.end(), slot) - P.halo_off.begin()) - 1;
@@ -204,11 +211,18 @@
   for (uint32_t orph : P.orphans) add(orph, &zero_slot, 1, 0);
   std::vector<DeviceArray<uint32_t>> d_arr(ng), d_tiles(ng);
   std::vector<uint32_t> n_tiles(ng, 0u);
+  const bool reverse = (size_t)P.halo_off.back() * esize(h->number_type) <= ((size_t)256 << 20);
+  DeviceArray<uint32_t> d_rec, d_tab;
+  if (shared) {
+    int rc;
+    if ((rc = d_rec.upload(P.sh_p2rec.data(), P.sh_p2rec.size()))) return rc;
+    if ((rc = d_tab.upload(P.sh_p2tab.data(), P.sh_p2tab.size()))) return rc;
+  }
   for (size_t g = 0; g < ng; ++g) {
     std::vector<uint32_t> arr, tiles;
     build_pass2_classes(sd[g], so[g], si[g], arr, tiles);
     n_tiles[g] = (uint32_t)(tiles.size() / 4);
-    if ((size_t)P.halo_off.back() * esize(h->number_type) <= ((size_t)256 << 20)) {
+    if (reverse) {
       const size_t nt = tiles.size() / 4;
       for (size_t a = 0, b = nt ? nt - 1 : 0; a < b; ++a, --b)
         for (int w = 0; w < 4; ++w) std::swap(tiles[4 * a + w], tiles[4 * b + w]);
@@ -220,6 +234,10 @@
   h->d_p2arr = std::move(d_arr);
   h->d_p2tiles = std::move(d_tiles);
   h->n_p2tiles = std::move(n_tiles);
+  h->d_p2rec = std::move(d_rec);
+  h->d_p2tab = std::move(d_tab);
+  h->p2_shared = shared;
+  h->p2_reverse = reverse;
   return 0;
 }
 
@@ -282,8 +300,13 @@
       if ((rc = up(h->d_hnrec, P.pr_hn.data(), P.pr_hn.size()))) return rc;
       if ((rc = up(h->d_hn_slot, P.pr_hn_slot.data(), P.pr_hn_slot.size()))) return rc;
     }
-    if ((rc = up(h->d_bdofsp, P.pr_dofs.data(), P.pr_dofs.size()))) return rc;
-    if ((rc = up(h->d_idxp, P.pr_idx.data(), P.pr_idx.size()))) return rc;
+    h->shared_records = P.sh_use && h->planes == PlaneKernel::planes3 && !(d.flags & MFGPU_NO_SHARED_RECORDS);
+    const std::vector<uint32_t> &rd = h->shared_records ? P.sh_dofs : P.pr_dofs;
+    const std::vector<uint32_t> &rx = h->shared_records ? P.sh_idx : P.pr_idx;
+    if ((rc = up(h->d_bdofsp, rd.data(), rd.size()))) return rc;
+    if ((rc = up(h->d_idxp, rx.data(), rx.size()))) return rc;
+    if (h->shared_records && (rc = up(h->d_shtab, P.sh_batch.data(), P.sh_batch.size()))) return rc;
+    h->record_bytes = h->d_bdofsp.bytes() + h->d_idxp.bytes() + h->d_shtab.bytes();
   }
   if ((rc = up(h->d_orphans, P.orphans.data(), P.orphans.size()))) return rc;
   if (h->twopass) {
@@ -399,6 +422,10 @@
 
 template <typename T>
 int launch_pass2_group(mfgpu_handle *h, size_t group, void *dst, const void *src, hipStream_t st, int add) {
+  if (h->p2_shared && group == 1)
+    HIP_TRY(reduce_owner_batches_launch<T>((T *)dst, (const T *)src, h->d_halo.as<const T>(), h->d_p2rec.get(),
+                                           h->d_p2tab.get(), (uint32_t)(h->plan.batch_cell_off.size() - 1),
+                                           (uint32_t)p_hs(h->plan.n) * 64u, h->p2_reverse ? 1 : 0, add, st));
   HIP_TRY(reduce_classes_launch<T>((T *)dst, (const T *)src, h->d_halo.as<const T>(), h->d_p2arr[group].get(),
                                    h->d_p2tiles[group].get(), h->n_p2tiles[group], add, st));
   return 0;
@@ -455,6 +482,7 @@
   a.perm = h->d_perm.get();
   a.bdofsp = h->d_bdofsp.get();
   a.idxp = h->d_idxp.get();
+  a.shtab = h->shared_records ? h->d_shtab.get() : nullptr;
   a.hnrec = h->d_hnrec.get();
   a.hn_slot = h->d_hn_slot.get();
   a.coefp = h->d_coefp.as<const T>();
@@ -694,6 +722,7 @@
   h->number_type = d.number_type;
   h->hn = hn;
   h->twopass = !(d.flags & MFGPU_COLORED_SCATTER);
+  h->no_shared_records = (d.flags & MFGPU_NO_SHARED_RECORDS) != 0;
   const int nn = h->n * h->n;
   std::vector<double> sv(nn), sg(nn);
   for (int i = 0; i < nn; ++i) {
@@ -777,6 +806,18 @@
   return 0;
 }
 
+int mfgpu_record_stats(const mfgpu_handle *h, uint64_t s[4]) {
+  if (!h || !s) return MFGPU_EINVAL;
+  const Plan &P = h->plan;
+  const size_t n = (size_t)P.n, nb = (size_t)p_kgu((int)n) * 64, nx = ((n * n + 1) / 2) * (p_cells_per_wave((int)n) * n);
+  const bool planes = h->planes != PlaneKernel::none;
+  s[0] = (h->shared_records ? 1 : 0) | (h->p2_shared ? 2 : 0);
+  s[1] = planes ? P.sh_dofs.size() / nb : 0;
+  s[2] = planes ? P.sh_idx.size() / nx : 0;
+  s[3] = h->record_bytes;
+  return 0;
+}
+
 const char *mfgpu_kernel_name(const mfgpu_handle *h) {
   if (!h) return "";
   const bool x = h->batches == BatchKernel::x;
diff --git a/dealii-cuda_amd/csrc/mfgpu_internal.h b/dealii-cuda_amd/csrc/mfgpu_internal.h
--- a/dealii-cuda_amd/csrc/mfgpu_internal.h
+++ b/dealii-cuda_amd/csrc/mfgpu_internal.h
@@ -69,6 +69,10 @@
   uint32_t n_plane_batches = 0;
   uint32_t n_plain_plane_batches = 0;
   std::vector<uint32_t> pr_dofs, pr_idx, pr_hn, pr_hn_slot;
+  std::vector<uint32_t> sh_dofs, sh_idx, sh_batch;
+  bool sh_use = false;
+  std::vector<uint32_t> sh_p2rec, sh_p2tab;
+  bool sh_p2_use = false;
   uint64_t n_first = 0, n_add = 0;
 };
 
@@ -91,6 +95,11 @@
 enum class BatchKernel : uint8_t { none, batches, x, g, g2 };
 int choose_kernel_and_plan(const mfgpu_desc &d, PlaneKernel &pk, BatchKernel &bk, Plan &plan);
 int build_plane_records(Plan &plan, const uint32_t *constraint_mask);
+constexpr int kShBatchWords = 4;
+constexpr double kShareMaxFraction = 0.5;
+void share_plane_records(Plan &plan);
+constexpr int kP2Header = 16, kP2MaxK = 12, kP2SlotBits = 12;
+void share_pass2_records(Plan &plan);
 
 int derive_tables(int n, const double *shape_values, const double *shape_gradients,
                   std::vector<double> &S, std::vector<double> &Dt);
diff --git a/dealii-cuda_amd/csrc/mfgpu_kernels.h b/dealii-cuda_amd/csrc/mfgpu_kernels.h
--- a/dealii-cuda_amd/csrc/mfgpu_kernels.h
+++ b/dealii-cuda_amd/csrc/mfgpu_kernels.h
@@ -38,6 +38,7 @@
   int add;
   unsigned long long *stamps;
   int dbg;
+  const uint32_t *shtab = nullptr;
 };
 
 template <typename T, int n>
@@ -91,6 +92,9 @@
 hipError_t reduce_classes_launch(T *dst, const T *src, const T *halo, const uint32_t *arr, const uint32_t *tiles,
                                  uint32_t n_tiles, int add, hipStream_t st);
 template <typename T>
+hipError_t reduce_owner_batches_launch(T *dst, const T *src, const T *halo, const uint32_t *rec, const uint32_t *tab,
+                                       uint32_t n_batches, uint32_t hstride, int reverse, int add, hipStream_t st);
+template <typename T>
 hipError_t relayout_coef_launch(T *out, const T *in, const uint32_t *cell_batch, const uint32_t *cell_pos,
                                 size_t total, int n, hipStream_t st);
 template <typename T>
diff --git a/dealii-cuda_amd/csrc/mfgpu_kernels_p.hip b/dealii-cuda_amd/csrc/mfgpu_kernels_p.hip
--- a/dealii-cuda_amd/csrc/mfgpu_kernels_p.hip
+++ b/dealii-cuda_amd/csrc/mfgpu_kernels_p.hip
@@ -8,7 +8,7 @@
 
 #define MFGPU_PIN_VMEM() __builtin_amdgcn_sched_barrier(0x380)
 
-template <int n, typename T, bool ADD, bool HN>
+template <int n, typename T, bool ADD, bool HN, bool SH = false>
 __global__ void __launch_bounds__(64) __attribute__((amdgpu_waves_per_eu(1, 1)))
 apply_planes3(const ApplyArgs<T> A, const TablesEO<T, n> tab) {
   constexpr int n2 = n * n;
@@ -58,22 +58,35 @@
     return l < bend ? (l >= hole0 ? l + hole_len : l) : x;
   };
   if (b >= hole0) b += hole_len;
-
-  auto load_dofs = [&](uint32_t bb, uint32_t (&g)[KGU]) {
-    const uint32_t *p = A.bdofsp + (size_t)bb * (KGU * 64) + lane;
-#pragma unroll
-    for (int j = 0; j < KGU; ++j) g[j] = nt_load(p + j * 64);
-  };
-  auto src_at = [&](uint32_t g) -> T {
-    return *reinterpret_cast<const T *>(reinterpret_cast<const char *>(A.src) + (uint32_t)(g * (uint32_t)sizeof(T)));
-  };
-  auto dst_at = [&](uint32_t g) -> T * {
-    return reinterpret_cast<T *>(reinterpret_cast<char *>(A.dst) + (uint32_t)(g * (uint32_t)sizeof(T)));
-  };
-  auto load_ix = [&](uint32_t bb, uint32_t (&ix)[NIW]) {
-    const uint32_t *p = A.idxp + (size_t)bb * (NIW * NT) + tk;
-#pragma unroll
-    for (int w = 0; w < NIW; ++w) ix[w] = nt_load(p + w * NT);
+  static_assert(!(SH && HN), "hanging-node batches keep the expanded records");
+  struct Meta {
+    uint32_t base, drec, irec;
+  };
+  auto meta_request = [&](uint32_t bb) -> uint32_t {
+    return A.shtab[(size_t)bb * kShBatchWords + (lane & (kShBatchWords - 1))];
+  };
+  auto meta_of = [&](uint32_t v) -> Meta {
+    return Meta{(uint32_t)__builtin_amdgcn_readlane((int)v, 0), (uint32_t)__builtin_amdgcn_readlane((int)v, 1),
+                (uint32_t)__builtin_amdgcn_readlane((int)v, 2)};
+  };
+
+  auto load_dofs = [&](uint32_t rec, uint32_t (&g)[KGU]) {
+    const uint32_t *p = A.bdofsp + (size_t)rec * (KGU * 64) + lane;
+#pragma unroll
+    for (int j = 0; j < KGU; ++j) g[j] = SH ? p[j * 64] : nt_load(p + j * 64);
+  };
+  auto src_at = [&](uint32_t base, uint32_t g) -> T {
+    const T *const sp = SH ? A.src + base : A.src;
+    return *reinterpret_cast<const T *>(reinterpret_cast<const char *>(sp) + (uint32_t)(g * (uint32_t)sizeof(T)));
+  };
+  auto dst_at = [&](uint32_t base, uint32_t g) -> T * {
+    T *const dp = SH ? A.dst + base : A.dst;
+    return reinterpret_cast<T *>(reinterpret_cast<char *>(dp) + (uint32_t)(g * (uint32_t)sizeof(T)));
+  };
+  auto load_ix = [&](uint32_t rec, uint32_t (&ix)[NIW]) {
+    const uint32_t *p = A.idxp + (size_t)rec * (NIW * NT) + tk;
+#pragma unroll
+    for (int w = 0; w < NIW; ++w) ix[w] = SH ? p[w * NT] : nt_load(p + w * NT);
   };
   auto stage_src = [&](const uint32_t (&g)[KGU], const T (&sv)[KGU]) {
 #pragma unroll
@@ -89,9 +102,9 @@
   auto ixb = [&](const uint32_t (&ix)[NIW], int i) -> uint32_t {
     return (i & 1) ? (ix[i >> 1] >> 16) : (ix[i >> 1] & 0xffffu);
   };
-  auto scatter_slot = [&](int j, uint32_t bb, uint32_t g, T r, T oldv) {
+  auto scatter_slot = [&](int j, uint32_t bb, uint32_t base, uint32_t g, T r, T oldv) {
     if (j < JI) {
-      *dst_at(g) = ADD ? oldv + r : r;
+      *dst_at(base, g) = ADD ? oldv + r : r;
     } else {
       T *const hp = A.halo + (size_t)bb * (HS * 64) + lane;
       hp[(j - JI) * 64] = r;
@@ -116,9 +129,17 @@
   };
   T Cc[n2];
   T SVn[KGU], R[KGU], old[KGU];
-  load_dofs(b, Gc);
-  load_dofs(b1, Gn);
-  load_ix(b, IXc);
+  Meta Mp{0u, 0u, 0u}, Mc = Mp, M1 = Mp, M2 = Mp;
+  uint32_t Mv = 0u;
+  if (SH) {
+    Mc = meta_of(meta_request(b));
+    M1 = meta_of(meta_request(b1));
+    M2 = meta_of(meta_request(b2));
+    Mp = Mc;
+  }
+  load_dofs(SH ? Mc.drec : b, Gc);
+  load_dofs(SH ? M1.drec : b1, Gn);
+  load_ix(SH ? Mc.irec : b, IXc);
   if (HN) load_hn(b, Hc);
   constexpr uint32_t kDummyIx = 8u * (uint32_t)(KGU * 64 - 1) * 0x10001u;
 #pragma unroll
@@ -130,7 +151,7 @@
   }
 #pragma unroll
   for (int j = 0; j < KGU; ++j) {
-    SVn[j] = src_at(Gc[j]);
+    SVn[j] = src_at(Mc.base, Gc[j]);
     Gp[j] = Gc[j];
     R[j] = T(0);
     old[j] = T(0);
@@ -198,12 +219,13 @@
     STAMP(0);
     RSTAMP(8);
     WGSTAMP(10);
-    load_dofs(b2, Gnn);
-    load_ix(b1, IXn);
+    load_dofs(SH ? M2.drec : b2, Gnn);
+    load_ix(SH ? M1.irec : b1, IXn);
+    if (SH) Mv = meta_request(next_of(b2));
     if (HN) load_hn(b1, Hn);
     if (ADD) {
 #pragma unroll
-      for (int j = 0; j < JI; ++j) old[j] = *dst_at(Gp[j]);
+      for (int j = 0; j < JI; ++j) old[j] = *dst_at(Mp.base, Gp[j]);
     }
     STAMP(1);
     auto hookA = [&](int) {};
@@ -211,10 +233,10 @@
       MFGPU_PIN_VMEM();
 #pragma unroll
       for (int j = (KGU * s) / (5 * n); j < (KGU * (s + 1)) / (5 * n); ++j)
-        scatter_slot(j, bp, Gp[j], R[j], old[j]);
+        scatter_slot(j, bp, Mp.base, Gp[j], R[j], old[j]);
 #pragma unroll
       for (int j = (KGU * s) / (5 * n); j < (KGU * (s + 1)) / (5 * n); ++j)
-        SVn[j] = src_at(Gn[j]);
+        SVn[j] = src_at(M1.base, Gn[j]);
       MFGPU_PIN_VMEM();
     };
     const T *const cnext = A.coefp + (size_t)b1 * (n2 * NT) + tk;
@@ -398,6 +420,7 @@
     stage_src(Gn, SVn);
     STAMP(6);
     bp = b;
+    if (SH) Mp = Mc;
 #pragma unroll
     for (int j = 0; j < KGU; ++j) Gp[j] = Gc[j];
     STAMP(7);
@@ -407,6 +430,11 @@
     b = b1;
     b1 = b2;
     b2 = next_of(b2);
+    if (SH) {
+      Mc = M1;
+      M1 = M2;
+      M2 = meta_of(Mv);
+    }
 #pragma unroll
     for (int j = 0; j < KGU; ++j) {
       Gc[j] = Gn[j];
@@ -421,10 +449,10 @@
   }
   if (ADD) {
 #pragma unroll
-    for (int j = 0; j < JI; ++j) old[j] = *dst_at(Gp[j]);
-  }
-#pragma unroll
-  for (int j = 0; j < KGU; ++j) scatter_slot(j, bp, Gp[j], R[j], old[j]);
+    for (int j = 0; j < JI; ++j) old[j] = *dst_at(Mp.base, Gp[j]);
+  }
+#pragma unroll
+  for (int j = 0; j < KGU; ++j) scatter_slot(j, bp, Mp.base, Gp[j], R[j], old[j]);
 }
 
 template <int n, typename T>
@@ -438,7 +466,14 @@
   *lds = p_lds_bytes<n, T>(hn);
   const void *f0 = hn ? (const void *)apply_planes3<n, T, false, true> : (const void *)apply_planes3<n, T, false, false>;
   const void *f1 = hn ? (const void *)apply_planes3<n, T, true, true> : (const void *)apply_planes3<n, T, true, false>;
-  const hipError_t e = hipFuncSetAttribute(f1, hipFuncAttributeMaxDynamicSharedMemorySize, (int)*lds);
+  hipError_t e = hipFuncSetAttribute(f1, hipFuncAttributeMaxDynamicSharedMemorySize, (int)*lds);
+  if (e == hipSuccess && !hn) {
+    e = hipFuncSetAttribute((const void *)apply_planes3<n, T, true, false, true>,
+                            hipFuncAttributeMaxDynamicSharedMemorySize, (int)*lds);
+    if (e == hipSuccess)
+      e = hipFuncSetAttribute((const void *)apply_planes3<n, T, false, false, true>,
+                              hipFuncAttributeMaxDynamicSharedMemorySize, (int)*lds);
+  }
   return e == hipSuccess ? configure_kernel(f0, *lds, 64, blocks) : e;
 }
 
@@ -452,6 +487,11 @@
       hipLaunchKernelGGL((apply_planes3<n, T, true, true>), dim3(grid), dim3(64), lds, st, a, tab);
     else
       hipLaunchKernelGGL((apply_planes3<n, T, false, true>), dim3(grid), dim3(64), lds, st, a, tab);
+  } else if (a.shtab) {
+    if (a.add)
+      hipLaunchKernelGGL((apply_planes3<n, T, true, false, true>), dim3(grid), dim3(64), lds, st, a, tab);
+    else
+      hipLaunchKernelGGL((apply_planes3<n, T, false, false, true>), dim3(grid), dim3(64), lds, st, a, tab);
   } else {
     if (a.add)
       hipLaunchKernelGGL((apply_planes3<n, T, true, false>), dim3(grid), dim3(64), lds, st, a, tab);
diff --git a/dealii-cuda_amd/csrc/mfgpu_pass2.hip b/dealii-cuda_amd/csrc/mfgpu_pass2.hip
--- a/dealii-cuda_amd/csrc/mfgpu_pass2.hip
+++ b/dealii-cuda_amd/csrc/mfgpu_pass2.hip
@@ -75,6 +75,67 @@
   }
 }
 
+template <typename T, int K>
+__device__ __forceinline__ void reduce_owned(T *__restrict__ dst, const T *__restrict__ src,
+                                             const T *__restrict__ halo, const uint32_t *__restrict__ r, uint32_t e,
+                                             uint32_t d, uint32_t kk, uint32_t kw, uint32_t hslot0, uint32_t hstride,
+                                             int add) {
+  const T *const hb = halo + hslot0;
+  auto partial = [&](uint32_t w) -> T {
+    return hb[(w >> kP2SlotBits) * hstride + (w & ((1u << kP2SlotBits) - 1u))];
+  };
+  constexpr int KU = K > 0 ? K : 1;
+  uint32_t w[KU];
+#pragma unroll
+  for (int t = 0; t < KU; ++t) w[t] = (uint32_t)t < kk ? r[r[3 + t] + e] : 0u;
+  if (d == 0xffffffffu) return;
+  T v;
+  if (d >> 31) {
+    v = src[d & 0x7fffffffu];
+  } else {
+    T q[KU];
+#pragma unroll
+    for (int t = 0; t < KU; ++t) q[t] = (uint32_t)t < kk ? partial(w[t]) : T(0);
+    v = q[0];
+#pragma unroll
+    for (int t = 1; t < KU; ++t)
+      if ((uint32_t)t < kk) v += q[t];
+    if (K == 0)
+      for (uint32_t t = 1; t < kw; ++t)
+        if (t < kk) v += partial(r[r[3 + t] + e]);
+  }
+  T *const out = dst + (d & 0x7fffffffu);
+  *out = add ? *out + v : v;
+}
+
+template <typename T>
+__global__ void __launch_bounds__(256)
+reduce_owner_batches(T *__restrict__ dst, const T *__restrict__ src, const T *__restrict__ halo,
+                     const uint32_t *__restrict__ rec, const uint2 *__restrict__ tab, uint32_t n_batches,
+                     uint32_t hstride, int reverse, int add) {
+  const uint32_t ob = reverse ? n_batches - 1u - blockIdx.x : blockIdx.x;
+  const uint2 t = tab[ob];
+  const uint32_t *const r = rec + t.y;
+  const uint32_t e0 = r[1];
+  dst += t.x;
+  src += t.x;
+  for (uint32_t e = threadIdx.x; e < e0; e += 256u) {
+    const uint32_t d = r[kP2Header + e], kk = r[kP2Header + e0 + e];
+    const uint32_t kw = (uint32_t)__builtin_amdgcn_readfirstlane((int)kk);
+    const uint32_t h0 = ob * hstride;
+    switch (kw) {
+      case 0: break;
+      case 1: reduce_owned<T, 1>(dst, src, halo, r, e, d, kk, kw, h0, hstride, add); break;
+      case 2: reduce_owned<T, 2>(dst, src, halo, r, e, d, kk, kw, h0, hstride, add); break;
+      case 3: reduce_owned<T, 3>(dst, src, halo, r, e, d, kk, kw, h0, hstride, add); break;
+      case 4: reduce_owned<T, 4>(dst, src, halo, r, e, d, kk, kw, h0, hstride, add); break;
+      case 5: case 6: case 7:
+      case 8: reduce_owned<T, 8>(dst, src, halo, r, e, d, kk, kw, h0, hstride, add); break;
+      default: reduce_owned<T, 0>(dst, src, halo, r, e, d, kk, kw, h0, hstride, add); break;
+    }
+  }
+}
+
 }
 
 void build_pass2_classes(const std::vector<uint32_t> &sdofs, const std::vector<uint32_t> &s_off,
@@ -118,6 +179,18 @@
                      reinterpret_cast<const uint4 *>(tiles), add);
   return hipGetLastError();
 }
+template <typename T>
+hipError_t reduce_owner_batches_launch(T *dst, const T *src, const T *halo, const uint32_t *rec, const uint32_t *tab,
+                                       uint32_t n_batches, uint32_t hstride, int reverse, int add, hipStream_t st) {
+  if (n_batches == 0) return hipSuccess;
+  hipLaunchKernelGGL(reduce_owner_batches<T>, dim3(n_batches), dim3(256), 0, st, dst, src, halo, rec,
+                     reinterpret_cast<const uint2 *>(tab), n_batches, hstride, reverse, add);
+  return hipGetLastError();
+}
+template hipError_t reduce_owner_batches_launch<double>(double *, const double *, const double *, const uint32_t *,
+                                                        const uint32_t *, uint32_t, uint32_t, int, int, hipStream_t);
+template hipError_t reduce_owner_batches_launch<float>(float *, const float *, const float *, const uint32_t *,
+                                                       const uint32_t *, uint32_t, uint32_t, int, int, hipStream_t);
 template hipError_t reduce_classes_launch<double>(double *, const double *, const double *, const uint32_t *,
                                                   const uint32_t *, uint32_t, int, hipStream_t);
 template hipError_t reduce_classes_launch<float>(float *, const float *, const float *, const uint32_t *,
diff --git a/dealii-cuda_amd/csrc/mfgpu_plan.cpp b/dealii-cuda_amd/csrc/mfgpu_plan.cpp
--- a/dealii-cuda_amd/csrc/mfgpu_plan.cpp
+++ b/dealii-cuda_amd/csrc/mfgpu_plan.cpp
@@ -3,6 +3,7 @@
 #include <cmath>
 #include <cstring>
 #include <numeric>
+#include <unordered_map>
 
 #include "mfgpu_internal.h"
 
@@ -696,7 +697,121 @@
       }
     }
   }
+  share_plane_records(P);
+  share_pass2_records(P);
   return 0;
+}
+
+namespace {
+uint64_t hash_words(const uint32_t *w, size_t n) {
+  uint64_t h = 1469598103934665603ull;
+  for (size_t i = 0; i < n; ++i) h = (h ^ w[i]) * 1099511628211ull;
+  return h;
+}
+
+uint32_t intern_record(std::vector<uint32_t> &table, std::unordered_multimap<uint64_t, uint32_t> &seen,
+                       const uint32_t *rec, size_t len) {
+  const uint64_t h = hash_words(rec, len);
+  const auto range = seen.equal_range(h);
+  for (auto it = range.first; it != range.second; ++it)
+    if (!std::memcmp(table.data() + (size_t)it->second * len, rec, len * sizeof(uint32_t))) return it->second;
+  const uint32_t id = (uint32_t)(table.size() / len);
+  table.insert(table.end(), rec, rec + len);
+  seen.emplace(h, id);
+  return id;
+}
+}
+
+void share_plane_records(Plan &P) {
+  const int n = P.n, NT = p_cells_per_wave(n) * n, NIW = (n * n + 1) / 2;
+  const size_t NB = (size_t)p_kgu(n) * 64, NX = (size_t)NIW * NT, nbat = P.n_plane_batches;
+  P.sh_dofs.clear();
+  P.sh_idx.clear();
+  P.sh_batch.assign(nbat * kShBatchWords, 0u);
+  std::unordered_multimap<uint64_t, uint32_t> seen_d, seen_x;
+  std::vector<uint32_t> rel(NB);
+  for (size_t b = 0; b < nbat; ++b) {
+    const uint32_t *g = P.pr_dofs.data() + b * NB;
+    uint32_t base = 0x7fffffffu;
+    for (size_t t = 0; t < NB; ++t) base = std::min(base, g[t] & 0x7fffffffu);
+    for (size_t t = 0; t < NB; ++t) rel[t] = g[t] - base;
+    uint32_t *e = P.sh_batch.data() + b * kShBatchWords;
+    e[0] = base;
+    e[1] = intern_record(P.sh_dofs, seen_d, rel.data(), NB);
+    e[2] = intern_record(P.sh_idx, seen_x, P.pr_idx.data() + b * NX, NX);
+  }
+  const size_t shared = P.sh_dofs.size() + P.sh_idx.size() + P.sh_batch.size();
+  const size_t expanded = P.pr_dofs.size() + P.pr_idx.size();
+  P.sh_use = nbat > 0 && P.pr_hn.empty() && (double)shared <= kShareMaxFraction * (double)expanded;
+}
+
+void share_pass2_records(Plan &P) {
+  P.sh_p2rec.clear();
+  P.sh_p2tab.clear();
+  P.sh_p2_use = false;
+  const size_t nb = P.batch_cell_off.size() - 1;
+  const uint32_t hs = (uint32_t)p_hs(P.n) * 64u;
+  if (nb == 0 || P.n_plane_batches != nb || P.halo_off.size() != nb + 1 || hs > (1u << kP2SlotBits)) return;
+  for (size_t b = 0; b <= nb; ++b)
+    if (P.halo_off[b] != (uint64_t)b * hs) return;
+  std::vector<std::vector<uint32_t>> owned(nb);
+  size_t expanded = 0;
+  for (size_t i = 0; i < P.sdofs.size(); ++i) {
+    const uint32_t k = P.s_off[i + 1] - P.s_off[i];
+    expanded += 1 + (k ? k : 1);
+    if (k == 0) continue;
+    if (k > (uint32_t)kP2MaxK) return;
+    const uint32_t owner = P.s_idx[P.s_off[i]] / hs;
+    for (uint32_t t = 0; t < k; ++t) {
+      const uint32_t tb = P.s_idx[P.s_off[i] + t] / hs;
+      if (tb >= nb || tb < owner || tb - owner >= (1u << (32 - kP2SlotBits))) return;
+    }
+    owned[owner].push_back((uint32_t)i);
+  }
+  P.sh_p2tab.assign(2 * nb, 0u);
+  std::unordered_multimap<uint64_t, std::pair<uint32_t, uint32_t>> seen;
+  std::vector<uint32_t> rec;
+  for (size_t b = 0; b < nb; ++b) {
+    std::vector<uint32_t> &m = owned[b];
+    auto k_of = [&](uint32_t i) { return P.s_off[i + 1] - P.s_off[i]; };
+    std::stable_sort(m.begin(), m.end(), [&](uint32_t x, uint32_t y) { return k_of(x) > k_of(y); });
+    const uint32_t base = P.sh_batch[b * kShBatchWords], ne = (uint32_t)m.size(), kmax = ne ? k_of(m[0]) : 0u;
+    auto pad = [](uint32_t x) { return (x + 63u) & ~63u; };
+    const uint32_t e0 = pad(ne);
+    rec.assign(kP2Header, 0u);
+    rec[0] = ne;
+    rec[1] = e0;
+    rec[2] = kmax;
+    rec.resize(kP2Header + 2 * (size_t)e0, 0u);
+    for (uint32_t e = 0; e < e0; ++e) rec[kP2Header + e] = e < ne ? P.sdofs[m[e]] - base : 0xffffffffu;
+    for (uint32_t e = 0; e < ne; ++e) rec[kP2Header + e0 + e] = k_of(m[e]);
+    for (uint32_t t = 0; t < kmax; ++t) {
+      uint32_t cnt = 0;
+      while (cnt < ne && k_of(m[cnt]) > t) ++cnt;
+      rec[3 + t] = (uint32_t)rec.size();
+      rec.resize(rec.size() + pad(cnt), 0u);
+      for (uint32_t e = 0; e < cnt; ++e) {
+        const uint32_t slot = P.s_idx[P.s_off[m[e]] + t], tb = slot / hs;
+        rec[rec[3 + t] + e] = ((tb - (uint32_t)b) << kP2SlotBits) | (slot - tb * hs);
+      }
+    }
+    const uint64_t h = hash_words(rec.data(), rec.size());
+    uint32_t off = 0xffffffffu;
+    const auto range = seen.equal_range(h);
+    for (auto it = range.first; it != range.second && off == 0xffffffffu; ++it)
+      if (it->second.second == rec.size() &&
+          !std::memcmp(P.sh_p2rec.data() + it->second.first, rec.data(), rec.size() * sizeof(uint32_t)))
+        off = it->second.first;
+    if (off == 0xffffffffu) {
+      off = (uint32_t)P.sh_p2rec.size();
+      P.sh_p2rec.insert(P.sh_p2rec.end(), rec.begin(), rec.end());
+      seen.emplace(h, std::make_pair(off, (uint32_t)rec.size()));
+    }
+    P.sh_p2tab[2 * b] = base;
+    P.sh_p2tab[2 * b + 1] = off;
+  }
+  const size_t shared = P.sh_p2rec.size() + P.sh_p2tab.size();
+  P.sh_p2_use = (double)shared <= kShareMaxFraction * (double)expanded;
 }
 
 int choose_kernel_and_plan(const mfgpu_desc &d, PlaneKernel &pk, BatchKernel &bk, Plan &plan) {
@@ -832,10 +947,19 @@
     case 14: v = &p->plan.pr_idx; break;
     case 15: v = &p->plan.pr_hn; break;
     case 16: v = &p->plan.pr_hn_slot; break;
+    case 17: v = &p->plan.sh_dofs; break;
+    case 18: v = &p->plan.sh_idx; break;
+    case 19: v = &p->plan.sh_batch; break;
+    case 20: v = &p->plan.sh_p2rec; break;
+    case 21: v = &p->plan.sh_p2tab; break;
     default: mfgpu::set_error("bad array id"); return MFGPU_EINVAL;
   }
   *ptr = v->data();
   return (int64_t)v->size();
+}
+
+int mfgpu_plan_shares_records(const mfgpu_plan *p) {
+  return p ? (p->plan.sh_use ? 1 : 0) | (p->plan.sh_p2_use ? 2 : 0) : 0;
 }
 
 int64_t mfgpu_plan_lmap(const mfgpu_plan *p, const uint16_t **ptr) {
diff --git a/dealii-cuda_amd/pymfgpu/__init__.py b/dealii-cuda_amd/pymfgpu/__init__.py
--- a/dealii-cuda_amd/pymfgpu/__init__.py
+++ b/dealii-cuda_amd/pymfgpu/__init__.py
@@ -10,7 +10,7 @@
 
 F64, F32 = 0, 1
 OK, EINVAL = 0, -1
-UNIFORM_J0, HANGING_NODES, COLORED_SCATTER = 1, 2, 1 << 8
+UNIFORM_J0, HANGING_NODES, COLORED_SCATTER, NO_SHARED_RECORDS = 1, 2, 1 << 8, 1 << 9
 KERNEL_AUTO, KERNEL_PENCILS, KERNEL_PENCILS_X, KERNEL_PLANES, KERNEL_PLANES_2W = 0, 1, 2, 3, 4
 
 
@@ -37,6 +37,7 @@
     "mfgpu_vec_sadd", "mfgpu_vec_equ", "mfgpu_vec_scale", "mfgpu_vec_divide", "mfgpu_vec_invert", "mfgpu_vec_mul",
     "mfgpu_vec_dot", "mfgpu_vec_l2_norm", "mfgpu_vec_add_and_dot", "mfgpu_vec_all_zero", "mfgpu_profile_enable", "mfgpu_profile_read", "mfgpu_profile_read_pass2",
     "mfgpu_plan_create", "mfgpu_plan_destroy", "mfgpu_plan_array_u32", "mfgpu_plan_lmap", "mfgpu_plan_bflags",
+    "mfgpu_plan_shares_records", "mfgpu_record_stats",
     "mfgpu_vec_alloc", "mfgpu_vec_free", "mfgpu_vec_fill", "mfgpu_vec_from_host", "mfgpu_vec_to_host",
     "mfgpu_device_synchronize", "mfgpu_device_memory_info", "mfgpu_mesh_create_uniform", "mfgpu_mesh_create_adaptive", "mfgpu_mesh_create_ball", "mfgpu_mesh_create_from_leaves",
     "mfgpu_mesh_cell_levels", "mfgpu_mesh_destroy",
@@ -104,6 +105,8 @@
         L.mfgpu_plan_lmap.restype = C.c_int64
         L.mfgpu_plan_bflags.argtypes = [C.c_void_p, C.POINTER(C.c_void_p)]
         L.mfgpu_plan_bflags.restype = C.c_int64
+        L.mfgpu_plan_shares_records.argtypes = [C.c_void_p]
+        L.mfgpu_record_stats.argtypes = [C.c_void_p, C.POINTER(C.c_uint64)]
         L.mfgpu_vec_alloc.argtypes = [C.POINTER(C.c_void_p), C.c_size_t, C.c_int]
         L.mfgpu_vec_free.argtypes = [C.c_void_p]
         L.mfgpu_vec_fill.argtypes = [C.c_void_p, C.c_size_t, C.c_int, C.c_double, C.c_void_p]
@@ -386,6 +389,13 @@
     pr_idx = property(lambda s: s._u32(14))
     pr_hn = property(lambda s: s._u32(15))
     pr_hn_slot = property(lambda s: s._u32(16))
+    sh_dofs = property(lambda s: s._u32(17))
+    sh_idx = property(lambda s: s._u32(18))
+    sh_batch = property(lambda s: s._u32(19).reshape(-1, 4))
+    shares_records = property(lambda s: bool(lib().mfgpu_plan_shares_records(s._h) & 1))
+    sh_p2rec = property(lambda s: s._u32(20))
+    sh_p2tab = property(lambda s: s._u32(21).reshape(-1, 2))
+    shares_pass2_records = property(lambda s: bool(lib().mfgpu_plan_shares_records(s._h) & 2))
 
     @property
     def lmap(self):
@@ -514,7 +524,13 @@
         _check(lib().mfgpu_plan_stats(self._h, s))
         keys = ["n_batches", "n_launches", "batch_dofs", "max_batch_dofs", "max_batch_cells", "n_orphans",
                 "first_touch_or_shared_dofs", "rmw_adds_or_halo_slots"]
-        return dict(zip(keys, [int(v) for v in s]))
+        out = dict(zip(keys, [int(v) for v in s]))
+        r = (C.c_uint64 * 4)()
+        _check(lib().mfgpu_record_stats(self._h, r))
+        out.update(index_records="shared" if r[0] & 1 else "expanded",
+                   pass2_records="shared" if r[0] & 2 else "expanded", distinct_dof_records=int(r[1]),
+                   distinct_index_records=int(r[2]), index_record_bytes=int(r[3]))
+        return out
 
     def kernel_name(self):
         return lib().mfgpu_kernel_name(self._h).decode()
diff --git a/include/mfgpu.h b/include/mfgpu.h
--- a/include/mfgpu.h
+++ b/include/mfgpu.h
@@ -21,6 +21,8 @@
 #define MFGPU_HANGING_NODES (1u << 1)
 
 #define MFGPU_COLORED_SCATTER (1u << 8)
+
+#define MFGPU_NO_SHARED_RECORDS (1u << 9)
 
 typedef struct mfgpu_handle mfgpu_handle;
 
@@ -72,6 +74,8 @@
 
 int mfgpu_plan_stats(const mfgpu_handle *h, uint64_t stats[8]);
 
+int mfgpu_record_stats(const mfgpu_handle *h, uint64_t stats[4]);
+
 const char *mfgpu_kernel_name(const mfgpu_handle *h);
 
 int mfgpu_profile_enable(mfgpu_handle *h, int on);
@@ -82,6 +86,7 @@
 int mfgpu_plan_create(const mfgpu_desc *desc, mfgpu_plan **out);
 void mfgpu_plan_destroy(mfgpu_plan *p);
 int64_t mfgpu_plan_array_u32(const mfgpu_plan *p, int what, const uint32_t **ptr);
+int mfgpu_plan_shares_records(const mfgpu_plan *p);
 int64_t mfgpu_plan_lmap(const mfgpu_plan *p, const uint16_t **ptr);
 int64_t mfgpu_plan_bflags(const mfgpu_plan *p, const uint8_t **ptr);
 
```

After: 80.30 billion DoFs/s (median of 6 runs). 9.9% higher.
